# facebookresearch/vggsfm

Measured on NVIDIA H100. Metric: BA iterations/sec, higher is better.
Workload: dtype f64

## Files before the change

include/vggsfm_b200.h:

```cpp
#ifndef VGGSFM_B200_H
#define VGGSFM_B200_H

#include <stddef.h>
#include <stdint.h>

#ifdef __cplusplus
extern "C" {
#endif

#define VGG_OK 0
#define VGG_EINVAL (-1)
#define VGG_ECUDA (-2)
#define VGG_EWORKSPACE (-3)
#define VGG_ESOLVER (-4)

#define VGG_SIMPLE_PINHOLE 0
#define VGG_SIMPLE_RADIAL 1

#define VGG_INTR_CONST 0
#define VGG_INTR_PER_FRAME 1
#define VGG_INTR_SHARED 2

const char* vgg_last_error(void);
int vgg_version(void);


typedef struct vgg_ba_problem {
  int32_t S, N;
  int32_t camera_model;
  int32_t intr_mode;
  const float* uv;
  const uint8_t* mask;
  const uint8_t* param_const;
  const uint8_t* point_const;
  double* poses;
  double* intr;
  double* points;
} vgg_ba_problem;

typedef struct vgg_ba_options {
  int32_t max_num_iterations;
  int32_t max_num_consecutive_invalid_steps;
  int32_t jacobi_scaling;
  int32_t reserved;
  double function_tolerance, gradient_tolerance, parameter_tolerance;
  double initial_trust_region_radius, max_trust_region_radius, min_trust_region_radius;
  double min_relative_decrease, min_lm_diagonal, max_lm_diagonal;
} vgg_ba_options;

typedef struct vgg_ba_summary {
  int32_t iterations, successful, termination, reserved;
  double initial_cost, final_cost, final_radius;
  double device_ms;
  int64_t kernel_launches;
} vgg_ba_summary;

#define VGG_BA_NO_CONVERGENCE 0
#define VGG_BA_CONVERGENCE_GRADIENT 1
#define VGG_BA_CONVERGENCE_FUNCTION 2
#define VGG_BA_CONVERGENCE_PARAMETER 3
#define VGG_BA_MIN_TRUST_REGION 4
#define VGG_BA_FAILURE 5

typedef int (*vgg_allreduce_fn)(void* user, double* buf, size_t count, int op, void* stream);

typedef struct vgg_ba_fabric {
  double* ar_local;
  double* ar_multicast;
  size_t ar_doubles;
  int32_t world, rank;
  double* peer_base[8];
  size_t total_doubles;
} vgg_ba_fabric;

void vgg_ba_default_options(vgg_ba_options* opt);
int vgg_ba_dims(int camera_model, int intr_mode, int* dc, int* ns);
int vgg_ba_workspace_bytes(int S, int N, int camera_model, int intr_mode, size_t* bytes);

int vgg_ba_camrec_len(int camera_model, int intr_mode);
int vgg_ba_build_blocks(const vgg_ba_problem* prob, double* cost, double* camrec, double* g_p,
                        double* H_pp, double* W, double* shared, int tracks_per_warp, void* stream);

int vgg_ba_schur(const vgg_ba_problem* prob, const double* camrec, const double* g_p,
                 const double* H_pp, const double* W, const double* shared, const double* scale_p,
                 double radius, double min_diag, double max_diag, void* workspace, size_t ws_bytes,
                 double* Sraw, double* rhs, int* Dpad_out, void* stream);

int vgg_cholesky_lower(int n, int lda, double* A, void* workspace, size_t ws_bytes, int* info_host, void* stream);

int vgg_syrk_ozaki_workspace_bytes(int Kpad, int Dpad, int slices, size_t* bytes);
int vgg_syrk_ozaki(int Kpad, int Dpad, const double* Zt, double* Cmat, int slices, void* workspace, size_t ws_bytes,
                   void* stream);
int vgg_ba_solve(const vgg_ba_problem* prob, const vgg_ba_options* opt, void* workspace,
                 size_t ws_bytes, vgg_allreduce_fn allreduce, void* allreduce_user,
                 vgg_ba_summary* summary, double* trace, void* stream);
int vgg_ba_reduced_system_doubles(int S, int camera_model, int intr_mode, size_t* doubles);
int vgg_ba_fabric_doubles(int S, int camera_model, int intr_mode, size_t* doubles);
int vgg_ba_solve_fabric(const vgg_ba_problem* prob, const vgg_ba_options* opt, void* workspace,
                        size_t ws_bytes, vgg_allreduce_fn allreduce, void* allreduce_user,
                        const vgg_ba_fabric* fabric, vgg_ba_summary* summary, double* trace, void* stream);


typedef struct vgg_pose_options {
  int32_t max_num_iterations;
  int32_t max_num_consecutive_invalid_steps;
  int32_t min_inliers;
  int32_t reserved;
  double function_tolerance, gradient_tolerance, parameter_tolerance;
  double initial_trust_region_radius, max_trust_region_radius, min_trust_region_radius;
  double min_relative_decrease, min_lm_diagonal, max_lm_diagonal;
  double loss_function_scale;
  double max_reproj_error;
} vgg_pose_options;

#define VGG_POSE_SKIPPED 6
#define VGG_POSE_FEW_INLIERS 7

void vgg_pose_default_options(vgg_pose_options* opt);

int vgg_pose_refinement(int S, int P, int camera_model, const float* uv, const uint8_t* inlier,
                        const uint8_t* frame_flags, const double* points, double* poses, double* intr,
                        const vgg_pose_options* opt, uint8_t* inlier_used, double* summary_d, int32_t* summary_i,
                        void* stream);


int vgg_tri_workspace_bytes(int S, int N, int H0, int lo_num, size_t* bytes);
int vgg_triangulate_tracks(int S, int N, const double* extrinsics, const double* tracks_normalized,
                           const float* track_vis, const float* track_score, const int32_t* pairs, int H0,
                           int lo_num, double max_angular_error_deg, double min_tri_angle_deg, double* out_points,
                           int64_t* out_inlier_num, uint8_t* out_inlier_mask, void* workspace, size_t ws_bytes,
                           void* stream);

int vgg_triangulate_by_pair(int S, int N, const double* extrinsics, const double* tracks_normalized,
                            double* out_points, uint8_t* out_cheirality, double* out_angle_deg, void* workspace,
                            size_t ws_bytes, void* stream);

int vgg_filter_points3d(int S, int P, const double* points3d, const void* points2d, int points2d_is_f64,
                        const double* extrinsics, const double* intrinsics9, const double* extra_params,
                        double max_reproj_error, double min_tri_angle_deg, int check_triangle, double hard_max,
                        uint8_t* out_valid, uint8_t* out_detail, void* workspace, size_t ws_bytes, void* stream);

int vgg_project_points(int S, int P, const double* points3d, const double* extrinsics, const double* intrinsics9,
                       const double* extra_params, double* out_points2d, double* out_points_cam, void* stream);

int vgg_normalize_tracks(int S, int N, const void* tracks, const void* focal2, const void* pp2, int is_f64, void* out,
                         void* stream);

int vgg_undistort_simple_radial(int S, int N, const double* tracks_normalized, const double* extra_params,
                                int max_iterations, double max_step_norm, double rel_step_size, double* out,
                                int* iterations_run, void* workspace, size_t ws_bytes, void* stream);

int vgg_pnp_workspace_bytes(int S, int estimate_focal_length, size_t* bytes);
int vgg_absolute_pose_estimation(int S, int P, int camera_model, const float* uv, const uint8_t* mask,
                                 const uint8_t* frame_flags, const double* points, const double* intr,
                                 const double* u_samples, int num_trials, int estimate_focal_length, double max_error,
                                 double* pose_out, double* focal_out, int* num_inliers_out, uint8_t* inlier_out,
                                 void* workspace, size_t ws_bytes, void* stream);


int vgg_twoview_workspace_bytes(int B, int N, int T, int lo_num, size_t* bytes);
int vgg_estimate_fundamental(int B, int N, const void* points1, const void* points2, int points_are_f64,
                             const uint8_t* valid_mask, const int32_t* samples, int T, int lo_num, double threshold,
                             int squared, int second_refine, double* fmat_out, int32_t* inlier_num_out,
                             uint8_t* inlier_mask_out, double* residuals_out, void* workspace, size_t ws_bytes,
                             void* stream);

int vgg_fundamental_inliers(int B, int N, const void* points1, const void* points2, int points_are_f64,
                            const double* fmat, double threshold, int squared, uint8_t* inlier_mask_out, void* stream);

int vgg_relative_pose_from_fundamental(int B, int N, const void* points1, const void* points2, int points_are_f64,
                                       const double* fmat, double width, double height, double* R_out, double* t_out,
                                       double* E_out, void* stream);

int vgg_msac_fundamental_workspace_bytes(int B, int N, int max_iterations, int min_iterations, size_t* bytes);
int vgg_estimate_fundamental_msac(int B, int N, const void* points1, const void* points2, int points_are_f64,
                                  const uint8_t* valid_mask, double max_error, int max_iterations, int min_iterations,
                                  unsigned long long seed, double* fmat_out, int32_t* inlier_num_out,
                                  uint8_t* inlier_mask_out, int32_t* iterations_out, void* workspace, size_t ws_bytes,
                                  void* stream);


int vgg_corr_pyramid_bytes(int BS, int C, int H, int W, int num_levels, int elem_size, size_t* pyramid_bytes,
                           size_t* scratch_bytes);
int vgg_corr_build_pyramid(int BS, int C, int H, int W, int num_levels, const float* fmaps_nchw, int elem_size,
                           void* pyramid, void* scratch, void* stream);

int vgg_corr_sample(int BS, int N, int C, int H, int W, int num_levels, int radius, const void* pyramid, int elem_size,
                    const float* targets, const float* coords, int border_padding, float* out, void* stream);

int vgg_corr_tc_supported(int C, int H, int W, int num_levels, int radius);
int vgg_corr_tc_bytes(int BS, int C, int H, int W, int num_levels, int N, size_t* tile_bytes, size_t* target_bytes);
int vgg_corr_tc_build(int BS, int C, int H, int W, int num_levels, const void* pyramid_half, void* tiles, void* stream);
int vgg_corr_tc_sample(int BS, int N, int C, int H, int W, int num_levels, int radius, const void* tiles, const float* targets,
                       const float* coords, void* target_tiles, float* out, void* stream);

int vgg_sample_features4d(int B, int C, int H, int W, int R, const float* input_nchw, const float* coords, float* out,
                          void* stream);



int vgg_depth_sparse_samples(int n_total, const int32_t* uvd_frame, const double* uvd, double depth_min,
                             double depth_max, const int64_t* map_offsets, const int32_t* map_hw, const float* disp,
                             float* x_out, double* y_out, uint8_t* keep_out, void* stream);

int vgg_depth_median(int F, const int32_t* offsets, const double* y, double divisor, double* median_out,
                     void* stream);

int vgg_depth_ransac_workspace_bytes(int F, size_t* bytes);
int vgg_depth_ransac_max_chunk(void);
int vgg_depth_ransac_begin(int F, int max_trials, void* workspace, size_t ws_bytes, void* stream);
int vgg_depth_ransac_chunk(int F, const int32_t* offsets, const float* x, const double* y, const double* threshold,
                           int R, const int32_t* frames, int T, const int32_t* samples, uint8_t* running_out,
                           void* workspace, size_t ws_bytes, void* stream);
int vgg_depth_ransac_finish(int F, const int32_t* offsets, const float* x, const double* y, const double* threshold,
                            float* scale_out, float* shift_out, int32_t* n_trials_out, int32_t* n_inliers_out,
                            uint8_t* inlier_mask_out, void* workspace, size_t ws_bytes, void* stream);

int vgg_depth_tile_pixels(void);
int vgg_depth_apply(int F, int64_t n_tiles, const int64_t* map_offsets, const int64_t* tile_offsets,
                    const float* scale, const float* shift, float* disp, float* depth_out, int32_t* tile_counts,
                    void* stream);

int vgg_depth_unproject(int F, int64_t n_tiles, const int64_t* map_offsets, const int32_t* map_hw,
                        const int64_t* tile_offsets, const int64_t* tile_base, const float* depth, const uint8_t* rgb,
                        const int32_t* cam_model, const double* cam_params, const double* world_from_cam,
                        double* out, void* stream);

#ifdef __cplusplus
}
#endif
#endif
```

vggsfm_b200/_lib.py:

```python
from __future__ import annotations

import ctypes
import os

_HERE = os.path.dirname(os.path.abspath(__file__))
LIB_PATH = os.path.join(_HERE, "libvggsfm_b200.so")

EXPORTS = [
    "vgg_last_error", "vgg_version",
    "vgg_ba_default_options", "vgg_ba_dims", "vgg_ba_workspace_bytes", "vgg_ba_camrec_len",
    "vgg_ba_build_blocks", "vgg_ba_schur", "vgg_cholesky_lower", "vgg_ba_solve",
    "vgg_ba_reduced_system_doubles", "vgg_ba_fabric_doubles", "vgg_ba_solve_fabric",
    "vgg_pose_default_options", "vgg_pose_refinement", "vgg_pnp_workspace_bytes", "vgg_absolute_pose_estimation", "vgg_syrk_ozaki_workspace_bytes", "vgg_syrk_ozaki",
    "vgg_tri_workspace_bytes", "vgg_triangulate_tracks", "vgg_triangulate_by_pair", "vgg_filter_points3d",
    "vgg_project_points", "vgg_normalize_tracks", "vgg_undistort_simple_radial",
    "vgg_corr_pyramid_bytes", "vgg_corr_build_pyramid", "vgg_corr_sample", "vgg_sample_features4d",
    "vgg_corr_tc_supported", "vgg_corr_tc_bytes", "vgg_corr_tc_build", "vgg_corr_tc_sample",
    "vgg_twoview_workspace_bytes", "vgg_estimate_fundamental", "vgg_relative_pose_from_fundamental",
    "vgg_fundamental_inliers", "vgg_msac_fundamental_workspace_bytes", "vgg_estimate_fundamental_msac",
    "vgg_depth_sparse_samples", "vgg_depth_median", "vgg_depth_ransac_workspace_bytes", "vgg_depth_ransac_max_chunk",
    "vgg_depth_ransac_begin", "vgg_depth_ransac_chunk", "vgg_depth_ransac_finish", "vgg_depth_tile_pixels",
    "vgg_depth_apply", "vgg_depth_unproject",
]


DEV_EXPORTS = ["vgg_dev_blocks_timing", "vgg_dev_blocks_last_ms", "vgg_dev_chol128_probe", "vgg_dev_syrk_f64", "vgg_dev_syrk_f64_band", "vgg_dev_syrk_ozaki_band", "vgg_dev_trsv_probe", "vgg_dev_cholesky_band",
               "vgg_dev_last_band_hint", "vgg_dev_msac_trace", "vgg_dev_relative_pose_counts"]


class BAProblem(ctypes.Structure):
    _fields_ = [
        ("S", ctypes.c_int32), ("N", ctypes.c_int32),
        ("camera_model", ctypes.c_int32), ("intr_mode", ctypes.c_int32),
        ("uv", ctypes.c_void_p), ("mask", ctypes.c_void_p),
        ("param_const", ctypes.c_void_p), ("point_const", ctypes.c_void_p),
        ("poses", ctypes.c_void_p), ("intr", ctypes.c_void_p), ("points", ctypes.c_void_p),
    ]


class BAOptions(ctypes.Structure):
    _fields_ = [
        ("max_num_iterations", ctypes.c_int32),
        ("max_num_consecutive_invalid_steps", ctypes.c_int32),
        ("jacobi_scaling", ctypes.c_int32),
        ("reserved", ctypes.c_int32),
        ("function_tolerance", ctypes.c_double),
        ("gradient_tolerance", ctypes.c_double),
        ("parameter_tolerance", ctypes.c_double),
        ("initial_trust_region_radius", ctypes.c_double),
        ("max_trust_region_radius", ctypes.c_double),
        ("min_trust_region_radius", ctypes.c_double),
        ("min_relative_decrease", ctypes.c_double),
        ("min_lm_diagonal", ctypes.c_double),
        ("max_lm_diagonal", ctypes.c_double),
    ]


class BASummary(ctypes.Structure):
    _fields_ = [
        ("iterations", ctypes.c_int32), ("successful", ctypes.c_int32),
        ("termination", ctypes.c_int32), ("reserved", ctypes.c_int32),
        ("initial_cost", ctypes.c_double), ("final_cost", ctypes.c_double),
        ("final_radius", ctypes.c_double), ("device_ms", ctypes.c_double),
        ("kernel_launches", ctypes.c_int64),
    ]


class BAFabric(ctypes.Structure):
    _fields_ = [("ar_local", ctypes.c_void_p), ("ar_multicast", ctypes.c_void_p), ("ar_doubles", ctypes.c_size_t),
                ("world", ctypes.c_int32), ("rank", ctypes.c_int32), ("peer_base", ctypes.c_void_p * 8),
                ("total_doubles", ctypes.c_size_t)]


class PoseOptions(ctypes.Structure):
    _fields_ = [
        ("max_num_iterations", ctypes.c_int32),
        ("max_num_consecutive_invalid_steps", ctypes.c_int32),
        ("min_inliers", ctypes.c_int32),
        ("reserved", ctypes.c_int32),
        ("function_tolerance", ctypes.c_double),
        ("gradient_tolerance", ctypes.c_double),
        ("parameter_tolerance", ctypes.c_double),
        ("initial_trust_region_radius", ctypes.c_double),
        ("max_trust_region_radius", ctypes.c_double),
        ("min_trust_region_radius", ctypes.c_double),
        ("min_relative_decrease", ctypes.c_double),
        ("min_lm_diagonal", ctypes.c_double),
        ("max_lm_diagonal", ctypes.c_double),
        ("loss_function_scale", ctypes.c_double),
        ("max_reproj_error", ctypes.c_double),
    ]


ALLREDUCE_FN = ctypes.CFUNCTYPE(ctypes.c_int, ctypes.c_void_p, ctypes.c_void_p, ctypes.c_size_t,
                                ctypes.c_int, ctypes.c_void_p)

_lib = None


class NativeLibraryMissing(RuntimeError):
    pass


def lib() -> ctypes.CDLL:
    global _lib
    if _lib is not None:
        return _lib
    if not os.path.exists(LIB_PATH):
        raise NativeLibraryMissing(
            f"{LIB_PATH} not found: build it with `python -c 'import __graft_entry__ as g; g.build()'` "
            "or `make`. vggsfm_b200 has no CPU/PyTorch fallback.")
    L = ctypes.CDLL(LIB_PATH, mode=ctypes.RTLD_GLOBAL)
    L.vgg_last_error.restype = ctypes.c_char_p
    L.vgg_version.restype = ctypes.c_int
    L.vgg_ba_default_options.argtypes = [ctypes.POINTER(BAOptions)]
    L.vgg_ba_default_options.restype = None
    L.vgg_ba_dims.argtypes = [ctypes.c_int, ctypes.c_int, ctypes.POINTER(ctypes.c_int), ctypes.POINTER(ctypes.c_int)]
    L.vgg_ba_workspace_bytes.argtypes = [ctypes.c_int, ctypes.c_int, ctypes.c_int, ctypes.c_int,
                                         ctypes.POINTER(ctypes.c_size_t)]
    L.vgg_ba_camrec_len.argtypes = [ctypes.c_int, ctypes.c_int]
    L.vgg_ba_build_blocks.argtypes = [ctypes.POINTER(BAProblem)] + [ctypes.c_void_p] * 6 + [ctypes.c_int, ctypes.c_void_p]
    L.vgg_ba_schur.argtypes = ([ctypes.POINTER(BAProblem)] + [ctypes.c_void_p] * 6 +
                               [ctypes.c_double] * 3 + [ctypes.c_void_p, ctypes.c_size_t, ctypes.c_void_p,
                                                        ctypes.c_void_p, ctypes.POINTER(ctypes.c_int), ctypes.c_void_p])
    L.vgg_ba_solve.argtypes = [ctypes.POINTER(BAProblem), ctypes.POINTER(BAOptions), ctypes.c_void_p, ctypes.c_size_t,
                               ALLREDUCE_FN, ctypes.c_void_p, ctypes.POINTER(BASummary), ctypes.c_void_p,
                               ctypes.c_void_p]
    vp, ci, cd, cs = ctypes.c_void_p, ctypes.c_int, ctypes.c_double, ctypes.c_size_t
    L.vgg_ba_reduced_system_doubles.argtypes = [ci, ci, ci, ctypes.POINTER(cs)]
    L.vgg_ba_fabric_doubles.argtypes = [ci, ci, ci, ctypes.POINTER(cs)]
    L.vgg_ba_solve_fabric.argtypes = [ctypes.POINTER(BAProblem), ctypes.POINTER(BAOptions), vp, cs, ALLREDUCE_FN, vp,
                                      ctypes.POINTER(BAFabric), ctypes.POINTER(BASummary), vp, vp]
    L.vgg_pose_default_options.argtypes = [ctypes.POINTER(PoseOptions)]
    L.vgg_pose_default_options.restype = None
    L.vgg_pose_refinement.argtypes = [ci, ci, ci, vp, vp, vp, vp, vp, vp, ctypes.POINTER(PoseOptions), vp, vp, vp, vp]
    L.vgg_pnp_workspace_bytes.argtypes = [ci, ci, ctypes.POINTER(cs)]
    L.vgg_absolute_pose_estimation.argtypes = [ci, ci, ci, vp, vp, vp, vp, vp, vp, ci, ci, cd, vp, vp, vp, vp, vp, cs, vp]
    L.vgg_syrk_ozaki_workspace_bytes.argtypes = [ci, ci, ci, ctypes.POINTER(cs)]
    L.vgg_dev_blocks_timing.argtypes = [ci]
    L.vgg_dev_blocks_last_ms.argtypes = [ctypes.POINTER(cd)]
    L.vgg_dev_chol128_probe.argtypes = [ci, vp, vp, vp]
    L.vgg_dev_syrk_f64.argtypes = [ci, ci, vp, vp, vp]
    L.vgg_dev_syrk_f64_band.argtypes = L.vgg_dev_syrk_f64.argtypes + [vp, ci]
    L.vgg_dev_trsv_probe.argtypes = [ci, ci, vp, vp, cs, vp, vp]
    L.vgg_dev_last_band_hint.argtypes = [vp, vp, vp, vp, vp]
    L.vgg_syrk_ozaki.argtypes = [ci, ci, vp, vp, ci, vp, cs, vp]
    L.vgg_dev_syrk_ozaki_band.argtypes = L.vgg_syrk_ozaki.argtypes + [vp, ci]
    L.vgg_cholesky_lower.argtypes = [ci, ci, vp, vp, cs, ctypes.POINTER(ci), vp]
    L.vgg_dev_cholesky_band.argtypes = L.vgg_cholesky_lower.argtypes + [vp, ci, ci]
    L.vgg_tri_workspace_bytes.argtypes = [ci, ci, ci, ci, ctypes.POINTER(cs)]
    L.vgg_triangulate_tracks.argtypes = [ci, ci, vp, vp, vp, vp, vp, ci, ci, cd, cd, vp, vp, vp, vp, cs, vp]
    L.vgg_triangulate_by_pair.argtypes = [ci, ci, vp, vp, vp, vp, vp, vp, cs, vp]
    L.vgg_filter_points3d.argtypes = [ci, ci, vp, vp, ci, vp, vp, vp, cd, cd, ci, cd, vp, vp, vp, cs, vp]
    L.vgg_project_points.argtypes = [ci, ci, vp, vp, vp, vp, vp, vp, vp]
    L.vgg_normalize_tracks.argtypes = [ci, ci, vp, vp, vp, ci, vp, vp]
    L.vgg_undistort_simple_radial.argtypes = [ci, ci, vp, vp, ci, cd, cd, vp, ctypes.POINTER(ci), vp, cs, vp]
    L.vgg_corr_pyramid_bytes.argtypes = [ci, ci, ci, ci, ci, ci, ctypes.POINTER(cs), ctypes.POINTER(cs)]
    L.vgg_corr_build_pyramid.argtypes = [ci, ci, ci, ci, ci, vp, ci, vp, vp, vp]
    L.vgg_sample_features4d.argtypes = [ci, ci, ci, ci, ci, vp, vp, vp, vp]
    L.vgg_corr_sample.argtypes = [ci, ci, ci, ci, ci, ci, ci, vp, ci, vp, vp, ci, vp, vp]
    L.vgg_corr_tc_supported.argtypes = [ci, ci, ci, ci, ci]
    L.vgg_corr_tc_bytes.argtypes = [ci, ci, ci, ci, ci, ci, ctypes.POINTER(cs), ctypes.POINTER(cs)]
    L.vgg_corr_tc_build.argtypes = [ci, ci, ci, ci, ci, vp, vp, vp]
    L.vgg_corr_tc_sample.argtypes = [ci, ci, ci, ci, ci, ci, ci, vp, vp, vp, vp, vp, vp]
    L.vgg_twoview_workspace_bytes.argtypes = [ci, ci, ci, ci, ctypes.POINTER(cs)]
    L.vgg_estimate_fundamental.argtypes = [ci, ci, vp, vp, ci, vp, vp, ci, ci, cd, ci, ci, vp, vp, vp, vp, vp, cs, vp]
    L.vgg_fundamental_inliers.argtypes = [ci, ci, vp, vp, ci, vp, cd, ci, vp, vp]
    L.vgg_relative_pose_from_fundamental.argtypes = [ci, ci, vp, vp, ci, vp, cd, cd, vp, vp, vp, vp]
    L.vgg_dev_relative_pose_counts.argtypes = [ci, ci, vp, vp, ci, vp, cd, cd, vp, vp, vp, vp, vp]
    cu64 = ctypes.c_ulonglong
    L.vgg_msac_fundamental_workspace_bytes.argtypes = [ci, ci, ci, ci, ctypes.POINTER(cs)]
    L.vgg_estimate_fundamental_msac.argtypes = [ci, ci, vp, vp, ci, vp, cd, ci, ci, cu64, vp, vp, vp, vp, vp, cs, vp]
    L.vgg_dev_msac_trace.argtypes = [ci, ci, ci, ci, vp, ci, vp, vp, vp]
    i64 = ctypes.c_int64
    L.vgg_depth_sparse_samples.argtypes = [ci, vp, vp, cd, cd, vp, vp, vp, vp, vp, vp, vp]
    L.vgg_depth_median.argtypes = [ci, vp, vp, cd, vp, vp]
    L.vgg_depth_ransac_workspace_bytes.argtypes = [ci, ctypes.POINTER(cs)]
    L.vgg_depth_ransac_max_chunk.argtypes = []
    L.vgg_depth_ransac_begin.argtypes = [ci, ci, vp, cs, vp]
    L.vgg_depth_ransac_chunk.argtypes = [ci, vp, vp, vp, vp, ci, vp, ci, vp, vp, vp, cs, vp]
    L.vgg_depth_ransac_finish.argtypes = [ci, vp, vp, vp, vp, vp, vp, vp, vp, vp, vp, cs, vp]
    L.vgg_depth_tile_pixels.argtypes = []
    L.vgg_depth_apply.argtypes = [ci, i64, vp, vp, vp, vp, vp, vp, vp, vp]
    L.vgg_depth_unproject.argtypes = [ci, i64, vp, vp, vp, vp, vp, vp, vp, vp, vp, vp, vp]
    _lib = L
    return L


def check(rc: int, what: str) -> None:
    if rc != 0:
        raise RuntimeError(f"{what} failed (rc={rc}): {lib().vgg_last_error().decode(errors='replace')}")
```

vggsfm_b200/bundle_adjustment.py:

```python
from __future__ import annotations

import ctypes
import dataclasses
from typing import Optional

import torch

from . import _lib
from ._lib import BAOptions, BAProblem, BASummary

SIMPLE_PINHOLE = 0
SIMPLE_RADIAL = 1
INTR_CONST = 0
INTR_PER_FRAME = 1
INTR_SHARED = 2

TERMINATION = {0: "NO_CONVERGENCE", 1: "CONVERGENCE_GRADIENT", 2: "CONVERGENCE_FUNCTION",
               3: "CONVERGENCE_PARAMETER", 4: "MIN_TRUST_REGION_RADIUS", 5: "FAILURE_INVALID_STEPS"}


def camera_model_id(camera_type: str) -> int:
    if camera_type == "SIMPLE_PINHOLE":
        return SIMPLE_PINHOLE
    if camera_type == "SIMPLE_RADIAL":
        return SIMPLE_RADIAL
    raise ValueError(f"Camera type {camera_type} is not supported yet")


def dims(model: int, mode: int):
    dc, ns = ctypes.c_int(), ctypes.c_int()
    _lib.check(_lib.lib().vgg_ba_dims(model, mode, ctypes.byref(dc), ctypes.byref(ns)), "vgg_ba_dims")
    return dc.value, ns.value


def default_options() -> BAOptions:
    o = BAOptions()
    _lib.lib().vgg_ba_default_options(ctypes.byref(o))
    return o


def prepare_ba_options() -> BAOptions:
    o = default_options()
    o.function_tolerance *= 10
    o.gradient_tolerance *= 10
    o.parameter_tolerance *= 10
    o.max_num_iterations = 50
    return o


def default_param_const(S: int, model: int, mode: int, device, refine_focal_length=True, refine_extra_params=True,
                        gauge=True, const_pose: Optional[torch.Tensor] = None) -> torch.Tensor:
    dc, ns = dims(model, mode)
    c = torch.zeros(S * dc + ns, dtype=torch.uint8)
    if gauge:
        c[0:6] = 1
        if S > 1:
            c[dc + 3] = 1
    if const_pose is not None:
        for s in torch.nonzero(const_pose.cpu()).flatten().tolist():
            c[s * dc:s * dc + 6] = 1
    ni = 1 if model == SIMPLE_PINHOLE else 2
    for j, fl in enumerate([refine_focal_length, refine_extra_params][:ni]):
        if not fl:
            if mode == INTR_PER_FRAME:
                c[torch.arange(S) * dc + 6 + j] = 1
            elif mode == INTR_SHARED:
                c[S * dc + j] = 1
    return c.to(device)


_ws_cache: dict = {}


def workspace(S: int, N: int, model: int, mode: int, device) -> torch.Tensor:
    key = (S, N, model, mode, str(device))
    ws = _ws_cache.get(key)
    if ws is None:
        nbytes = ctypes.c_size_t()
        with torch.cuda.device(device):
            _lib.check(_lib.lib().vgg_ba_workspace_bytes(S, N, model, mode, ctypes.byref(nbytes)),
                       "vgg_ba_workspace_bytes")
        if len(_ws_cache) > 4:
            _ws_cache.clear()
        ws = torch.empty(nbytes.value, dtype=torch.uint8, device=device)
        _ws_cache[key] = ws
    return ws


def _problem(uv, mask, poses, intr, points, model, mode, param_const, point_const):
    S, N = mask.shape
    assert uv.dtype == torch.float32 and uv.is_contiguous() and uv.shape == (S, N, 2)
    assert mask.dtype == torch.uint8 and mask.is_contiguous()
    for t in (poses, intr, points):
        assert t.dtype == torch.float64 and t.is_contiguous() and t.is_cuda
    assert poses.shape == (S, 3, 4) and intr.shape == (S, 4) and points.shape == (N, 3)
    p = BAProblem()
    p.S, p.N, p.camera_model, p.intr_mode = S, N, model, mode
    p.uv, p.mask = uv.data_ptr(), mask.data_ptr()
    p.param_const = param_const.data_ptr() if param_const is not None else None
    p.point_const = point_const.data_ptr() if point_const is not None else None
    p.poses, p.intr, p.points = poses.data_ptr(), intr.data_ptr(), points.data_ptr()
    return p


def build_blocks(uv, mask, poses, intr, points, model, mode, point_const=None, tracks_per_warp=0):
    L = _lib.lib()
    S, N = mask.shape
    dc, ns = dims(model, mode)
    KR = L.vgg_ba_camrec_len(model, mode)
    dev = uv.device
    al = lambda n: (n + 31) // 32 * 32
    offs, tot = {}, 0
    for name, n in (("cost", 8), ("shared", 8), ("camrec", S * KR), ("g_p", N * 3), ("H_pp", N * 6)):
        offs[name] = (tot, n)
        tot += al(n)
    flat = torch.empty(tot, dtype=torch.float64, device=dev)
    view = lambda name, shape: flat[offs[name][0]:offs[name][0] + offs[name][1]].view(*shape)
    out = {
        "cost": view("cost", (8,))[:1],
        "camrec": view("camrec", (S, KR)),
        "g_p": view("g_p", (N, 3)),
        "H_pp": view("H_pp", (N, 6)),
        "W": torch.empty(N, (S * dc + ns + 1) // 2 * 2, 3, dtype=torch.float64, device=dev),
        "shared": view("shared", (8,)),
    }
    p = _problem(uv, mask, poses, intr, points, model, mode, None, point_const)
    with torch.cuda.device(dev):
        st = torch.cuda.current_stream().cuda_stream
        _lib.check(L.vgg_ba_build_blocks(ctypes.byref(p), out["cost"].data_ptr(), out["camrec"].data_ptr(),
                                         out["g_p"].data_ptr(), out["H_pp"].data_ptr(), out["W"].data_ptr(),
                                         out["shared"].data_ptr(), tracks_per_warp, st), "vgg_ba_build_blocks")
    return out


def schur(uv, mask, poses, intr, points, model, mode, blocks, scale_p, radius, min_diag=1e-6, max_diag=1e32,
          point_const=None):
    L = _lib.lib()
    S, N = mask.shape
    dc, ns = dims(model, mode)
    D = S * dc + ns
    Dpad = (D + 2 + 127) // 128 * 128
    dev = uv.device
    ws = workspace(S, N, model, mode, dev)
    Sraw = torch.empty(D, Dpad, dtype=torch.float64, device=dev)
    rhs = torch.empty(Dpad, dtype=torch.float64, device=dev)
    p = _problem(uv, mask, poses, intr, points, model, mode, None, point_const)
    dpad = ctypes.c_int()
    with torch.cuda.device(dev):
        st = torch.cuda.current_stream().cuda_stream
        _lib.check(L.vgg_ba_schur(ctypes.byref(p), blocks["camrec"].data_ptr(), blocks["g_p"].data_ptr(),
                                  blocks["H_pp"].data_ptr(), blocks["W"].data_ptr(), blocks["shared"].data_ptr(),
                                  scale_p.data_ptr(), radius, min_diag, max_diag, ws.data_ptr(), ws.numel(),
                                  Sraw.data_ptr(), rhs.data_ptr(), ctypes.byref(dpad), st), "vgg_ba_schur")
    assert dpad.value == Dpad
    return Sraw, rhs[:D]


@dataclasses.dataclass
class Summary:
    iterations: int
    successful: int
    termination: str
    initial_cost: float
    final_cost: float
    final_radius: float
    device_ms: float
    kernel_launches: int
    trace: Optional[torch.Tensor] = None
    alive: Optional[torch.Tensor] = None
    mask: Optional[torch.Tensor] = None


def lm_solve(uv, mask, poses, intr, points, model, mode, param_const=None, point_const=None,
             options: Optional[BAOptions] = None, allreduce=None, want_trace=False) -> Summary:
    L = _lib.lib()
    S, N = mask.shape
    dev = uv.device
    if param_const is None:
        param_const = default_param_const(S, model, mode, dev)
    opt = options or default_options()
    ws = workspace(S, N, model, mode, dev)
    p = _problem(uv, mask, poses, intr, points, model, mode, param_const, point_const)
    summ = BASummary()
    trace = torch.zeros(max(1, opt.max_num_iterations), 8, dtype=torch.float64) if want_trace else None
    cb = allreduce.bind(ws) if allreduce is not None else _lib.ALLREDUCE_FN()
    fabric = getattr(allreduce, "fabric", None)
    with torch.cuda.device(dev):
        st = torch.cuda.current_stream().cuda_stream
        if fabric is not None:
            fs = fabric.struct()
            rc = L.vgg_ba_solve_fabric(ctypes.byref(p), ctypes.byref(opt), ws.data_ptr(), ws.numel(), cb, None,
                                       ctypes.byref(fs), ctypes.byref(summ),
                                       trace.data_ptr() if trace is not None else None, st)
        else:
            rc = L.vgg_ba_solve(ctypes.byref(p), ctypes.byref(opt), ws.data_ptr(), ws.numel(), cb, None,
                                ctypes.byref(summ), trace.data_ptr() if trace is not None else None, st)
    _lib.check(rc, "vgg_ba_solve")
    return Summary(summ.iterations, summ.successful, TERMINATION.get(summ.termination, "?"), summ.initial_cost,
                   summ.final_cost, summ.final_radius, summ.device_ms, summ.kernel_launches,
                   trace[:summ.iterations] if trace is not None else None)



def filter_negative_depth(poses, points, mask):
    eps = torch.finfo(torch.float64).eps
    depth = torch.einsum("sj,nj->sn", poses[:, 2, :3], points) + poses[:, 2, 3][:, None]
    bad = mask & ~(depth >= eps)
    length = mask.sum(dim=0)
    nbad = bad.sum(dim=0)
    alive = (nbad == 0) | ((length - nbad) >= 2)
    mask = mask & ~bad & alive[None]
    return mask, alive


def normalize(poses, points, extent=10.0, p0=0.1, p1=0.9, alive=None):
    S = poses.shape[0]
    if S < 2:
        return poses, points
    R = poses[:, :, :3]
    t = poses[:, :, 3]
    centers = -torch.einsum("sji,sj->si", R, t)
    c32 = torch.sort(centers.to(torch.float32), dim=0).values
    P0 = int(p0 * (S - 1)) if S > 3 else 0
    P1 = int(p1 * (S - 1)) if S > 3 else S - 1
    bmin = c32[P0].double()
    bmax = c32[P1].double()
    mean = c32[P0:P1 + 1].double().sum(dim=0) / (P1 - P0 + 1)
    old_extent = torch.linalg.norm(bmax - bmin)
    scale = torch.where(old_extent < torch.finfo(torch.float64).eps, torch.ones_like(old_extent), extent / old_extent)
    tr = -scale * mean
    new_points = scale * points + tr
    if alive is not None:
        new_points = torch.where(alive[:, None], new_points, points)
    new_poses = poses.clone()
    new_poses[:, :, 3] = scale * t - torch.einsum("sij,j->si", R, tr)
    return new_poses, new_points


def pad_tracks(n: int, multiple: int = 16) -> int:
    return (n + multiple - 1) // multiple * multiple


def bundle_adjustment(points3d, extrinsics, intrinsics, extra_params, tracks, masks, shared_camera=False,
                      camera_type="SIMPLE_PINHOLE", options: Optional[BAOptions] = None, max_points3D_val=3000.0,
                      allreduce=None, want_trace=False, refine_focal_length=True, refine_extra_params=True,
                      const_pose=None, const_points=None, gauge=True, do_normalize=True, filter_reconstruction=True,
                      drop_negative_depth=True):
    model = camera_model_id(camera_type)
    dev = tracks.device
    if not tracks.is_cuda:
        raise RuntimeError("vggsfm_b200.bundle_adjustment needs CUDA tensors (no CPU fallback)")
    masks = masks.bool()
    valid_idx = torch.nonzero(masks.sum(dim=0) >= 2).flatten()
    pts = points3d.double()[valid_idx].contiguous()
    P = pts.shape[0]
    m = masks[:, valid_idx]
    m = m & (pts < max_points3D_val).all(dim=1)[None]
    poses = extrinsics.double().contiguous().clone()
    S = poses.shape[0]
    intr = torch.zeros(S, 4, dtype=torch.float64, device=dev)
    intr[:, 0] = intrinsics[:, 0, 0]
    intr[:, 1] = intrinsics[:, 0, 2]
    intr[:, 2] = intrinsics[:, 1, 2]
    if model == SIMPLE_RADIAL:
        intr[:, 3] = extra_params[:, 0]
    if shared_camera:
        mode = INTR_SHARED
        intr[:] = intr[0].clone()
    else:
        mode = INTR_PER_FRAME
    if not (refine_focal_length or refine_extra_params):
        mode = INTR_CONST
    if drop_negative_depth:
        m, alive = filter_negative_depth(poses, pts, m)
    else:
        alive = torch.ones(P, dtype=torch.bool, device=dev)
    point_const = ~m.any(dim=0)
    if const_points is not None:
        point_const = point_const | const_points[valid_idx]
    Pp = pad_tracks(max(P, 1))
    uv = torch.zeros(S, Pp, 2, dtype=torch.float32, device=dev)
    uv[:, :P] = tracks[:, valid_idx].float()
    mk = torch.zeros(S, Pp, dtype=torch.uint8, device=dev)
    mk[:, :P] = m.to(torch.uint8)
    X = torch.zeros(Pp, 3, dtype=torch.float64, device=dev)
    X[:P] = pts
    X[P:, 2] = 1.0
    pc = torch.ones(Pp, dtype=torch.uint8, device=dev)
    pc[:P] = point_const.to(torch.uint8)
    param_const = default_param_const(S, model, mode, dev, refine_focal_length, refine_extra_params, gauge, const_pose)
    summary = lm_solve(uv, mk, poses, intr, X, model, mode, param_const, pc, options, allreduce, want_trace)
    pts = X[:P]
    if do_normalize:
        poses, pts = normalize(poses, pts, 10.0, 0.1, 0.9, alive)
        if filter_reconstruction:
            poses, pts = normalize(poses, pts, 5.0, 0.1, 0.9, alive)
    pts = torch.where(alive[:, None], pts, torch.zeros_like(pts))
    summary.alive, summary.mask = alive, m
    K = torch.zeros(S, 3, 3, dtype=torch.float64, device=dev)
    K[:, 0, 0] = intr[:, 0]
    K[:, 1, 1] = intr[:, 0]
    K[:, 0, 2] = intr[:, 1]
    K[:, 1, 2] = intr[:, 2]
    K[:, 2, 2] = 1.0
    extra_out = intr[:, 3:4].clone() if model == SIMPLE_RADIAL else None
    return pts, poses, K, extra_out, valid_idx, summary


run_ba = bundle_adjustment



from .reconstruction import Reconstruction


def _reconstruction(pts, extr, K, extra, tracks, masks, image_size, camera_type, shared_camera, summary, alive=None):
    return Reconstruction.from_batch_matrix(pts, extr, K, tracks, masks, image_size, shared_camera=shared_camera,
                                            camera_type=camera_type, extra_params=extra, summary=summary, alive=alive)


def _revert_negative_focal(extr_new, K_new, extra_new, extr_old, K_old, extra_old):
    bad = K_new[:, 0, 0] < 0
    if bad.any():
        extr_new[bad] = extr_old[bad].to(extr_new.dtype)
        K_new[bad] = K_old[bad].to(K_new.dtype)
        if extra_new is not None:
            extra_new[bad] = extra_old[bad].to(extra_new.dtype)
    return extr_new, K_new, extra_new


def global_BA(triangulated_points, valid_tracks, pred_tracks, inlier_mask, extrinsics, intrinsics, extra_params,
              image_size, shared_camera=False, camera_type="SIMPLE_PINHOLE", allreduce=None):
    BA_points = triangulated_points[valid_tracks]
    BA_tracks = pred_tracks[:, valid_tracks]
    BA_inlier_masks = inlier_mask[valid_tracks].transpose(0, 1)
    pts, extr, K, extra, valid_idx, summary = bundle_adjustment(
        BA_points, extrinsics, intrinsics, extra_params, BA_tracks, BA_inlier_masks, shared_camera=shared_camera,
        camera_type=camera_type, options=prepare_ba_options(), allreduce=allreduce)
    extr, K, extra = _revert_negative_focal(extr, K, extra, extrinsics, intrinsics, extra_params)
    rec = _reconstruction(pts, extr, K, extra, BA_tracks[:, valid_idx], summary.mask, image_size, camera_type,
                          shared_camera, summary, summary.alive)
    return pts, extr, K, extra, rec


def init_BA(extrinsics, intrinsics, extra_params, tracks, points_3d_pair, inlier, image_size, shared_camera=False,
            init_max_reproj_error=0.5, camera_type="SIMPLE_PINHOLE"):
    from . import triangulation as tri
    init_idx = int(torch.argmax(inlier.sum(dim=-1)).item())
    init_indices = [0, init_idx + 1]
    toBA_extrinsics = extrinsics[init_indices]
    toBA_intrinsics = intrinsics[init_indices]
    toBA_extra = extra_params[init_indices] if extra_params is not None else None
    toBA_masks = inlier[init_idx].unsqueeze(0)
    toBA_masks = torch.cat([torch.ones_like(toBA_masks), toBA_masks], dim=0)
    valid_track = toBA_masks.sum(dim=0) >= 2
    toBA_masks = toBA_masks[:, valid_track]
    toBA_points = points_3d_pair[init_idx][valid_track]
    toBA_tracks = tracks[init_indices][:, valid_track]
    pts, extr, K, extra, valid_idx, summary = bundle_adjustment(
        toBA_points, toBA_extrinsics, toBA_intrinsics, toBA_extra, toBA_tracks, toBA_masks, shared_camera=shared_camera,
        camera_type=camera_type, options=prepare_ba_options(), filter_reconstruction=False)
    rec = _reconstruction(pts, extr, K, extra, toBA_tracks[:, valid_idx], summary.mask, image_size, camera_type,
                          shared_camera, summary, summary.alive)
    ok, _ = tri.filter_all_points3D(pts, toBA_tracks, extr, K, extra, check_triangle=False,
                                    max_reproj_error=init_max_reproj_error)
    points3D_opt = pts[ok]
    filtered = valid_track.clone()
    filtered[valid_track] = ok
    extrinsics[init_indices] = extr.to(extrinsics.dtype)
    intrinsics[init_indices] = K.to(intrinsics.dtype)
    if extra_params is not None:
        extra_params[init_indices] = extra.to(extra_params.dtype)
    return points3D_opt, extrinsics, intrinsics, extra_params, filtered, rec, init_idx


def get_valid_frame_mask(intrinsics, extrinsics, extra_params, scale):
    valid = (intrinsics[:, 0, 0] >= 0.1 * scale) & (intrinsics[:, 0, 0] <= 30 * scale)
    if extra_params is not None:
        if extra_params.dim() == 1:
            extra_params = extra_params[:, None]
        valid = valid & (extra_params.abs() <= 1.0).all(dim=-1)
    return valid & (extrinsics[:, :, 3].abs() <= 30).all(-1)


def iterative_global_BA(pred_tracks, intrinsics, extrinsics, pred_vis, pred_score, valid_tracks, points3D_opt,
                        image_size, shared_camera=False, min_valid_track_length=2, max_reproj_error=1,
                        ba_options=None, lastBA=False, camera_type="SIMPLE_PINHOLE", extra_params=None,
                        allreduce=None):
    from . import triangulation as tri
    tn = tri.cam_from_img(pred_tracks, intrinsics, extra_params)
    best_points, best_num, best_mask = tri.triangulate_tracks(extrinsics, tn, track_vis=pred_vis, track_score=pred_score,
                                                             max_ransac_iters=128)
    best_points[valid_tracks] = points3D_opt.to(best_points.dtype)
    _, filtered = tri.filter_all_points3D(best_points, pred_tracks, extrinsics, intrinsics, extra_params=extra_params,
                                          max_reproj_error=max_reproj_error, return_detail=True)
    valid_tracks = filtered.sum(dim=0) >= min_valid_track_length
    BA_points = best_points[valid_tracks]
    BA_tracks = pred_tracks[:, valid_tracks]
    BA_inlier_masks = filtered[:, valid_tracks]
    pts, extr, K, extra, valid_idx, summary = bundle_adjustment(
        BA_points, extrinsics, intrinsics, extra_params, BA_tracks, BA_inlier_masks, shared_camera=shared_camera,
        camera_type=camera_type, options=ba_options or default_options(), allreduce=allreduce)
    rec = _reconstruction(pts, extr, K, extra, BA_tracks[:, valid_idx], summary.mask, image_size, camera_type,
                          shared_camera, summary, summary.alive)
    if valid_idx.numel() != BA_points.shape[0]:
        full = torch.zeros(BA_points.shape[0], 3, dtype=pts.dtype, device=pts.device)
        full[valid_idx] = pts
        pts = full
    extr, K, extra = _revert_negative_focal(extr, K, extra, extrinsics, intrinsics, extra_params)
    _, filtered = tri.filter_all_points3D(pts, pred_tracks[:, valid_tracks], extr, K, extra_params=extra,
                                          max_reproj_error=max_reproj_error, return_detail=True)
    valid_after = filtered.sum(dim=0) >= min_valid_track_length
    valid_tmp = valid_tracks.clone()
    valid_tmp[valid_tracks] = valid_after
    valid_tracks = valid_tmp
    pts = pts[valid_after]
    BA_inlier_masks = filtered[:, valid_after]
    if lastBA:
        e2, p2 = normalize(extr, pts, 5.0, 0.1, 0.9)
        rec = _reconstruction(p2, e2, K, extra, pred_tracks[:, valid_tracks], BA_inlier_masks, image_size, camera_type,
                              shared_camera, summary)
    return pts, extr, K, extra, valid_tracks, BA_inlier_masks, rec
```

vggsfm_b200/csrc/ba_blocks.cu:

```cuda
#include <stdlib.h>
#include <utility>
#include "common.cuh"
#include "dev_probes.h"

namespace vgg {

static bool g_blocks_timing = false;
static cudaEvent_t g_blocks_ev[2] = {nullptr, nullptr};

constexpr int BW = 4;
constexpr int BT = BW * 32;
constexpr int TB = 4;
constexpr int XT = 32;
constexpr int PVS = 33;

template <int MODEL, int MODE>
struct BlkCfg {
  static constexpr int NI = (MODEL == VGG_SIMPLE_PINHOLE) ? 1 : 2;
  static constexpr int DC = (MODE == VGG_INTR_PER_FRAME) ? 6 + NI : 6;
  static constexpr int NS = (MODE == VGG_INTR_SHARED) ? NI : 0;
  static constexpr int NPACK = DC * (DC + 1) / 2;
  static constexpr int KR = DC + NPACK + 6 * NS;
  static constexpr int NP = 9 + 3 * NS;
};

__host__ __device__ constexpr int pack_row(int dc, int p) {
  int i = 0;
  while (p >= dc - i) { p -= dc - i; ++i; }
  return i;
}
__host__ __device__ constexpr int pack_col(int dc, int p) {
  int i = 0;
  while (p >= dc - i) { p -= dc - i; ++i; }
  return i + p;
}

template <int DC, int NS, int K, int KR>
__device__ __forceinline__ void cam_accumulate_one(double (&acc)[KR], const double* jc0, const double* jc1, double rx,
                                                   double ry) {
  constexpr int NPACK = DC * (DC + 1) / 2;
  if constexpr (K < DC) {
    acc[K] = fma(jc0[K], rx, fma(jc1[K], ry, acc[K]));
  } else if constexpr (K < DC + NPACK) {
    constexpr int i = pack_row(DC, K - DC), j = pack_col(DC, K - DC);
    acc[K] = fma(jc0[i], jc0[j], fma(jc1[i], jc1[j], acc[K]));
  } else {
    constexpr int q = K - DC - NPACK;
    constexpr int i = q / (NS > 0 ? NS : 1), j = q % (NS > 0 ? NS : 1);
    acc[K] = fma(jc0[i], jc0[6 + j], fma(jc1[i], jc1[6 + j], acc[K]));
  }
}
template <int DC, int NS, int KR, int... K>
__device__ __forceinline__ void cam_accumulate(double (&acc)[KR], const double* jc0, const double* jc1, double rx,
                                               double ry, std::integer_sequence<int, K...>) {
  (cam_accumulate_one<DC, NS, K, KR>(acc, jc0, jc1, rx, ry), ...);
}

template <int MODEL>
__device__ __forceinline__ void obs_math(const double* pw, int lane, const double* xt, float ox, float oy, bool valid,
                                         double* jc0, double* jc1, double* jx0, double* jx1, double& rx, double& ry) {
  const double2 xa = *reinterpret_cast<const double2*>(xt);
  const double2 xb = *reinterpret_cast<const double2*>(xt + 2);
  const double X0 = xa.x, X1 = xa.y, X2 = xb.x;
  const double m = valid ? 1.0 : 0.0;
  const double mp = (xb.y != 0.0) ? 0.0 : m;
  const double R00 = pw[0 * 32 + lane], R01 = pw[1 * 32 + lane], R02 = pw[2 * 32 + lane], t0_ = pw[3 * 32 + lane];
  const double R10 = pw[4 * 32 + lane], R11 = pw[5 * 32 + lane], R12 = pw[6 * 32 + lane], t1_ = pw[7 * 32 + lane];
  const double R20 = pw[8 * 32 + lane], R21 = pw[9 * 32 + lane], R22 = pw[10 * 32 + lane], t2_ = pw[11 * 32 + lane];
  const double fo = pw[12 * 32 + lane], cx = pw[13 * 32 + lane], cy = pw[14 * 32 + lane];
  const double kk = (MODEL == VGG_SIMPLE_RADIAL) ? pw[15 * 32 + lane] : 0.0;
  const double a1 = R00 * X0 + R01 * X1 + R02 * X2;
  const double a2 = R10 * X0 + R11 * X1 + R12 * X2;
  const double a3 = R20 * X0 + R21 * X1 + R22 * X2;
  const double px = a1 + t0_, py = a2 + t1_;
  const double pz = valid ? (a3 + t2_) : 1.0;
  const double iz = 1.0 / pz;
  const double u = px * iz, w_ = py * iz;
  const double r2 = u * u + w_ * w_;
  const double d = 1.0 + kk * r2;
  rx = valid ? (fo * d * u + cx - (double)ox) : 0.0;
  ry = valid ? (fo * d * w_ + cy - (double)oy) : 0.0;
  double a00, a01, a11;
  if (MODEL == VGG_SIMPLE_RADIAL) {
    a00 = fo * (d + 2.0 * kk * u * u);
    a01 = fo * (2.0 * kk * u * w_);
    a11 = fo * (d + 2.0 * kk * w_ * w_);
  } else {
    a00 = fo; a01 = 0.0; a11 = fo;
  }
  const double izm = iz * m;
  const double j00 = a00 * izm, j01 = a01 * izm, j02 = -(a00 * u + a01 * w_) * izm;
  const double j10 = a01 * izm, j11 = a11 * izm, j12 = -(a01 * u + a11 * w_) * izm;
  const double b1 = 2.0 * a1, b2 = 2.0 * a2, b3 = 2.0 * a3;
  jc0[0] = b2 * j02 - b3 * j01;  jc1[0] = b2 * j12 - b3 * j11;
  jc0[1] = b3 * j00 - b1 * j02;  jc1[1] = b3 * j10 - b1 * j12;
  jc0[2] = b1 * j01 - b2 * j00;  jc1[2] = b1 * j11 - b2 * j10;
  jc0[3] = j00; jc0[4] = j01; jc0[5] = j02;
  jc1[3] = j10; jc1[4] = j11; jc1[5] = j12;
  jc0[6] = m * d * u;            jc1[6] = m * d * w_;
  jc0[7] = m * fo * u * r2;      jc1[7] = m * fo * w_ * r2;
  const double mq = (xb.y != 0.0) ? 0.0 : 1.0;
  jx0[0] = mq * (j00 * R00 + j01 * R10 + j02 * R20);
  jx0[1] = mq * (j00 * R01 + j01 * R11 + j02 * R21);
  jx0[2] = mq * (j00 * R02 + j01 * R12 + j02 * R22);
  jx1[0] = mq * (j10 * R00 + j11 * R10 + j12 * R20);
  jx1[1] = mq * (j10 * R01 + j11 * R11 + j12 * R21);
  jx1[2] = mq * (j10 * R02 + j11 * R12 + j12 * R22);
  (void)mp;
}

template <int DC, int NS, int WB>
__device__ __forceinline__ void emit_blocks(double* wt, double* pvw, int lane, const double* jc0, const double* jc1,
                                            const double* jx0, const double* jx1, double rx, double ry) {
  double wb[WB];
#pragma unroll
  for (int i = 0; i < DC; ++i)
#pragma unroll
    for (int c = 0; c < 3; ++c) wb[i * 3 + c] = jc0[i] * jx0[c] + jc1[i] * jx1[c];
  if ((WB & 1) == 0) {
#pragma unroll
    for (int e = 0; e < WB; e += 2) *reinterpret_cast<double2*>(wt + e) = make_double2(wb[e], wb[e + 1]);
  } else {
#pragma unroll
    for (int e = 0; e < WB; ++e) wt[e] = wb[e];
  }
  pvw[0 * PVS + lane] = jx0[0] * rx + jx1[0] * ry;
  pvw[1 * PVS + lane] = jx0[1] * rx + jx1[1] * ry;
  pvw[2 * PVS + lane] = jx0[2] * rx + jx1[2] * ry;
  pvw[3 * PVS + lane] = jx0[0] * jx0[0] + jx1[0] * jx1[0];
  pvw[4 * PVS + lane] = jx0[0] * jx0[1] + jx1[0] * jx1[1];
  pvw[5 * PVS + lane] = jx0[0] * jx0[2] + jx1[0] * jx1[2];
  pvw[6 * PVS + lane] = jx0[1] * jx0[1] + jx1[1] * jx1[1];
  pvw[7 * PVS + lane] = jx0[1] * jx0[2] + jx1[1] * jx1[2];
  pvw[8 * PVS + lane] = jx0[2] * jx0[2] + jx1[2] * jx1[2];
#pragma unroll
  for (int j = 0; j < NS; ++j)
#pragma unroll
    for (int c = 0; c < 3; ++c) pvw[(9 + j * 3 + c) * PVS + lane] = jc0[6 + j] * jx0[c] + jc1[6 + j] * jx1[c];
}

__host__ __device__ inline size_t w_pitch(int D) { return (size_t)(D + (D & 1)); }

template <int MODEL, int MODE, bool USE_TMA>
__global__ void __launch_bounds__(BT, USE_TMA ? 2 : 3) ba_blocks_kernel(
    int S, int N, int tracks_per_warp, const float* __restrict__ uv, const uint8_t* __restrict__ mask,
    const double* __restrict__ poses, const double* __restrict__ intr, const double* __restrict__ points,
    const uint8_t* __restrict__ point_const, double* __restrict__ cost, double* __restrict__ camrec,
    double* __restrict__ g_p, double* __restrict__ H_pp, double* __restrict__ W, double* __restrict__ shared_out,
    const int* __restrict__ fg_tracks) {
  using C = BlkCfg<MODEL, MODE>;
  constexpr int DC = C::DC, NS = C::NS, KR = C::KR, NP = C::NP;
  constexpr int WB = DC * 3;
  extern __shared__ __align__(128) unsigned char smem_raw[];
  double* sm_pose = reinterpret_cast<double*>(smem_raw);
  double* sm_x = sm_pose + BW * 16 * 32;
  double* sm_pv = sm_x + BW * XT * 4;
  double* sm_w = sm_pv + BW * 32 * PVS;
  float* sm_obs = reinterpret_cast<float*>(sm_w + (size_t)BW * 2 * 32 * WB);
  const int tid = threadIdx.x, lane = tid & 31, warp = tid >> 5;
  const int D = S * DC + NS;
  const size_t pitch = w_pitch(D);
  const int ngroups = (S + 31) / 32;
  const int wid = blockIdx.x * BW + warp;
  const int g = wid % ngroups;
  const int chunk = wid / ngroups;
  const int t_begin = (int)min((long long)N, (long long)chunk * tracks_per_warp);
  const int t_end = min(N, t_begin + tracks_per_warp);
  if (fg_tracks && (t_end <= fg_tracks[2 * g] || t_begin >= fg_tracks[2 * g + 1])) return;
  const int s = g * 32 + lane;
  const bool frame_ok = s < S;
  const int nf = min(32, S - g * 32);
  double* pw = sm_pose + warp * 16 * 32;
  double* xw = sm_x + warp * XT * 4;
  double* pvw = sm_pv + warp * 32 * PVS;
  float* ow = sm_obs + (size_t)warp * 2 * 32 * 12 + lane * 12;
  double* wbuf = sm_w + (size_t)warp * 2 * 32 * WB;

#pragma unroll
  for (int i = 0; i < 12; ++i) pw[i * 32 + lane] = frame_ok ? poses[(size_t)s * 12 + i] : 0.0;
#pragma unroll
  for (int i = 0; i < 4; ++i) pw[(12 + i) * 32 + lane] = frame_ok ? intr[(size_t)s * 4 + i] : 0.0;
  __syncwarp();

  double acc[KR];
#pragma unroll
  for (int i = 0; i < KR; ++i) acc[i] = 0.0;
  double cost_acc = 0.0, gs0 = 0.0, gs1 = 0.0, hss0 = 0.0, hss1 = 0.0, hss2 = 0.0;

  const bool vec_ok = (N & 3) == 0;
  auto fetch = [&](int t0, int stage) {
    float* slot = ow + stage * 32 * 12;
    if (frame_ok && t0 < t_end) {
      const size_t o = (size_t)s * N + t0;
      if (vec_ok && t0 + TB <= t_end) {
        cp_async16(slot, uv + o * 2);
        cp_async16(slot + 4, uv + o * 2 + 4);
        cp_async4(slot + 8, mask + o);
      } else {
        uint32_t m = 0;
        for (int k = 0; k < TB; ++k) {
          const bool in = t0 + k < t_end;
          slot[2 * k] = in ? uv[(o + k) * 2] : 0.f;
          slot[2 * k + 1] = in ? uv[(o + k) * 2 + 1] : 0.f;
          if (in) m |= (uint32_t)(mask[o + k] != 0) << (8 * k);
        }
        reinterpret_cast<uint32_t*>(slot)[8] = m;
      }
    } else {
      *reinterpret_cast<float4*>(slot) = make_float4(0.f, 0.f, 0.f, 0.f);
      *reinterpret_cast<float4*>(slot + 4) = make_float4(0.f, 0.f, 0.f, 0.f);
      reinterpret_cast<uint32_t*>(slot)[8] = 0u;
    }
    cp_async_commit();
  };
  fetch(t_begin, 0);
  int batch = 0;
  for (int t0 = t_begin; t0 < t_end; t0 += TB) {
    if (((t0 - t_begin) & (XT - 1)) == 0) {
      __syncwarp();
      const int nn = t0 + lane;
      double x0 = 0.0, x1 = 0.0, x2 = 1.0, cf = 1.0;
      if (nn < t_end) {
        x0 = points[(size_t)nn * 3]; x1 = points[(size_t)nn * 3 + 1]; x2 = points[(size_t)nn * 3 + 2];
        cf = (point_const && point_const[nn] != 0) ? 1.0 : 0.0;
      }
      *reinterpret_cast<double2*>(xw + lane * 4) = make_double2(x0, x1);
      *reinterpret_cast<double2*>(xw + lane * 4 + 2) = make_double2(x2, cf);
      __syncwarp();
    }
    fetch(t0 + TB, (batch + 1) & 1);
    cp_async_wait<1>();
    const float* cur = ow + (batch & 1) * 32 * 12;
    const float4 ca = *reinterpret_cast<const float4*>(cur);
    const float4 cb = *reinterpret_cast<const float4*>(cur + 4);
    const uint32_t cm = reinterpret_cast<const uint32_t*>(cur)[8];
    ++batch;
#pragma unroll 1
    for (int k = 0; k < TB; k += 2) {
      const int nA = t0 + k;
      if (nA >= t_end) break;
      const bool hasB = nA + 1 < t_end;
      double jcA0[8], jcA1[8], jxA0[3], jxA1[3], rxA, ryA;
      double jcB0[8], jcB1[8], jxB0[3], jxB1[3], rxB, ryB;
      {
        const float ox = k == 0 ? ca.x : cb.x, oy = k == 0 ? ca.y : cb.y;
        const bool valid = frame_ok && ((cm >> (8 * k)) & 0xffu) != 0;
        obs_math<MODEL>(pw, lane, xw + ((nA - t_begin) & (XT - 1)) * 4, ox, oy, valid, jcA0, jcA1, jxA0, jxA1, rxA, ryA);
      }
      {
        const float ox = k == 0 ? ca.z : cb.z, oy = k == 0 ? ca.w : cb.w;
        const bool valid = hasB && frame_ok && ((cm >> (8 * (k + 1))) & 0xffu) != 0;
        obs_math<MODEL>(pw, lane, xw + ((nA + 1 - t_begin) & (XT - 1)) * 4, ox, oy, valid, jcB0, jcB1, jxB0, jxB1, rxB, ryB);
      }
      cost_acc += 0.5 * (rxA * rxA + ryA * ryA) + 0.5 * (rxB * rxB + ryB * ryB);
      if (USE_TMA) {
        if (lane == 0) tma_store_wait_read<0>();
        __syncwarp();
      }
      double* wA = wbuf + lane * WB;
      double* wB = wbuf + 32 * WB + lane * WB;
      emit_blocks<DC, NS, WB>(wA, pvw, lane, jcA0, jcA1, jxA0, jxA1, rxA, ryA);
      emit_blocks<DC, NS, WB>(wB, pvw + 16 * PVS, lane, jcB0, jcB1, jxB0, jxB1, rxB, ryB);
      double* dstA = W + ((size_t)nA * pitch + (size_t)g * 32 * DC) * 3;
      double* dstB = dstA + pitch * 3;
      const uint32_t bytes = (uint32_t)nf * WB * 8u;
      if (USE_TMA && (bytes & 15u) == 0) {
        fence_proxy_async();
        __syncwarp();
        if (lane == 0) {
          tma_store_1d(dstA, wbuf, bytes);
          if (hasB) tma_store_1d(dstB, wbuf + 32 * WB, bytes);
          tma_store_commit();
        }
      } else {
        __syncwarp();
        for (int e = lane; e < nf * WB; e += 32) dstA[e] = wbuf[e];
        if (hasB)
          for (int e = lane; e < nf * WB; e += 32) dstB[e] = wbuf[32 * WB + e];
        __syncwarp();
      }
      cam_accumulate<DC, NS, KR>(acc, jcA0, jcA1, rxA, ryA, std::make_integer_sequence<int, KR>{});
      cam_accumulate<DC, NS, KR>(acc, jcB0, jcB1, rxB, ryB, std::make_integer_sequence<int, KR>{});
      if (NS > 0) {
        gs0 += jcA0[6] * rxA + jcA1[6] * ryA + jcB0[6] * rxB + jcB1[6] * ryB;
        hss0 += jcA0[6] * jcA0[6] + jcA1[6] * jcA1[6] + jcB0[6] * jcB0[6] + jcB1[6] * jcB1[6];
        if (NS > 1) {
          gs1 += jcA0[7] * rxA + jcA1[7] * ryA + jcB0[7] * rxB + jcB1[7] * ryB;
          hss1 += jcA0[6] * jcA0[7] + jcA1[6] * jcA1[7] + jcB0[6] * jcB0[7] + jcB1[6] * jcB1[7];
          hss2 += jcA0[7] * jcA0[7] + jcA1[7] * jcA1[7] + jcB0[7] * jcB0[7] + jcB1[7] * jcB1[7];
        }
      }
      {
        const int v = lane & 15;
        const int nT = nA + (lane >> 4);
        double r = 0.0;
        if (v < NP) {
          const double* row = pvw + ((lane >> 4) * 16 + v) * PVS;
          double r0 = 0.0, r1 = 0.0, r2s = 0.0, r3 = 0.0;
#pragma unroll
          for (int j = 0; j < 32; j += 4) { r0 += row[j]; r1 += row[j + 1]; r2s += row[j + 2]; r3 += row[j + 3]; }
          r = (r0 + r1) + (r2s + r3);
        }
        if (r != 0.0 && nT < t_end) {
          if (v < 3) atomicAdd(&g_p[(size_t)nT * 3 + v], r);
          else if (v < 9) atomicAdd(&H_pp[(size_t)nT * 6 + (v - 3)], r);
          else if (v < NP) atomicAdd(&W[((size_t)nT * pitch + (size_t)S * DC + (v - 9) / 3) * 3 + (v - 9) % 3], r);
        }
      }
      __syncwarp();
    }
  }
  if (USE_TMA && lane == 0) tma_store_wait_all<0>();

  if (frame_ok && t_begin < t_end) {
#pragma unroll
    for (int i = 0; i < KR; ++i)
      if (acc[i] != 0.0) atomicAdd(&camrec[(size_t)s * KR + i], acc[i]);
  }
  {
    double a[8] = {cost_acc, gs0, gs1, hss0, hss1, hss2, 0.0, 0.0};
    const double r = warp_reduce_scatter<8>(a, lane);
    if (lane == 0 && r != 0.0) atomicAdd(cost, r);
    else if (NS > 0 && lane >= 1 && lane < 6 && r != 0.0) atomicAdd(&shared_out[lane - 1], r);
  }
}

template <int MODEL, int MODE>
static int launch_blocks(const vgg_ba_problem* p, double* cost, double* camrec, double* g_p, double* H_pp,
                         double* W, double* shared_out, int tracks_per_warp, const int* fg_tracks, cudaStream_t stream,
                         bool outputs_zeroed) {
  using C = BlkCfg<MODEL, MODE>;
  const int S = p->S, N = p->N;
  const int D = S * C::DC + C::NS;
  const size_t pitch = w_pitch(D);
  const size_t smem = sizeof(double) * (BW * 16 * 32 + BW * XT * 4 + BW * 32 * PVS + (size_t)BW * 2 * 32 * C::DC * 3) +
                      sizeof(float) * BW * 2 * 32 * 12;
  const bool tma_ok = ((reinterpret_cast<uintptr_t>(W) & 15) == 0);
  const int ngroups = (S + 31) / 32;
  const auto kern = tma_ok ? ba_blocks_kernel<MODEL, MODE, true> : ba_blocks_kernel<MODEL, MODE, false>;
  if (tracks_per_warp <= 0 && fg_tracks) {
    tracks_per_warp = 64;
  }
  if (tracks_per_warp <= 0) {
    static int slots = 0;
    if (slots == 0) {
      int dev = 0, sms = 132, per_sm = 2;
      cudaGetDevice(&dev);
      cudaDeviceGetAttribute(&sms, cudaDevAttrMultiProcessorCount, dev);
      cudaFuncSetAttribute(ba_blocks_kernel<MODEL, MODE, true>, cudaFuncAttributeMaxDynamicSharedMemorySize, (int)smem);
      cudaOccupancyMaxActiveBlocksPerMultiprocessor(&per_sm, ba_blocks_kernel<MODEL, MODE, true>, BT, smem);
      if (per_sm < 1) per_sm = 1;
      slots = sms * per_sm;
    }
    const long wave_warps = (long)slots * BW;
    long best_tpw = N;
    for (int waves = 1; waves <= 4; ++waves) {
      long chunks = waves * wave_warps / ngroups;
      if (chunks < 1) chunks = 1;
      long tpw = (N + chunks - 1) / chunks;
      tpw = (tpw + TB - 1) / TB * TB;
      if (tpw < 32 && waves > 1) break;
      best_tpw = tpw;
      if (tpw <= 512) break;
    }
    tracks_per_warp = (int)best_tpw;
  }
  const int chunks = (N + tracks_per_warp - 1) / tracks_per_warp;
  const long nwarps = (long)chunks * ngroups;
  const unsigned grid = (unsigned)((nwarps + BW - 1) / BW);
  if (!outputs_zeroed) {
    const char* lo = reinterpret_cast<const char*>(cost);
    const char* hi = reinterpret_cast<const char*>(H_pp + (size_t)N * 6);
    const size_t payload = sizeof(double) * (1 + 8 + (size_t)S * C::KR + (size_t)N * 9);
    const bool packed = lo < reinterpret_cast<const char*>(shared_out) && shared_out < camrec && camrec < g_p && g_p < H_pp &&
                        hi > lo && (size_t)(hi - lo) <= payload + 5 * 256;
    if (packed) {
      VGG_CUDA_CHECK(cudaMemsetAsync(cost, 0, (size_t)(hi - lo), stream));
    } else {
      VGG_CUDA_CHECK(cudaMemsetAsync(cost, 0, sizeof(double), stream));
      VGG_CUDA_CHECK(cudaMemsetAsync(camrec, 0, sizeof(double) * (size_t)S * C::KR, stream));
      VGG_CUDA_CHECK(cudaMemsetAsync(g_p, 0, sizeof(double) * (size_t)N * 3, stream));
      VGG_CUDA_CHECK(cudaMemsetAsync(H_pp, 0, sizeof(double) * (size_t)N * 6, stream));
      VGG_CUDA_CHECK(cudaMemsetAsync(shared_out, 0, sizeof(double) * 8, stream));
    }
  }
  if (pitch > (size_t)S * C::DC) {
    const size_t tail = pitch - (size_t)S * C::DC;
    VGG_CUDA_CHECK(cudaMemset2DAsync(W + (size_t)S * C::DC * 3, pitch * 24, 0, tail * 24, (size_t)N, stream));
  }
  if (g_blocks_timing) VGG_CUDA_CHECK(cudaEventRecord(g_blocks_ev[0], stream));
  VGG_CUDA_CHECK(cudaFuncSetAttribute(kern, cudaFuncAttributeMaxDynamicSharedMemorySize, (int)smem));
  kern<<<grid, BT, smem, stream>>>(S, N, tracks_per_warp, p->uv, p->mask, p->poses, p->intr, p->points, p->point_const,
                                   cost, camrec, g_p, H_pp, W, shared_out, fg_tracks);
  VGG_LAUNCH_CHECK();
  if (g_blocks_timing) VGG_CUDA_CHECK(cudaEventRecord(g_blocks_ev[1], stream));
  return VGG_OK;
}

int ba_build_blocks(const vgg_ba_problem* p, double* cost, double* camrec, double* g_p, double* H_pp, double* W,
                    double* shared_out, int tracks_per_warp, const int* fg_tracks, cudaStream_t stream,
                    bool outputs_zeroed) {
  const int key = p->camera_model * 3 + p->intr_mode;
  switch (key) {
    case 0: return launch_blocks<0, 0>(p, cost, camrec, g_p, H_pp, W, shared_out, tracks_per_warp, fg_tracks, stream, outputs_zeroed);
    case 1: return launch_blocks<0, 1>(p, cost, camrec, g_p, H_pp, W, shared_out, tracks_per_warp, fg_tracks, stream, outputs_zeroed);
    case 2: return launch_blocks<0, 2>(p, cost, camrec, g_p, H_pp, W, shared_out, tracks_per_warp, fg_tracks, stream, outputs_zeroed);
    case 3: return launch_blocks<1, 0>(p, cost, camrec, g_p, H_pp, W, shared_out, tracks_per_warp, fg_tracks, stream, outputs_zeroed);
    case 4: return launch_blocks<1, 1>(p, cost, camrec, g_p, H_pp, W, shared_out, tracks_per_warp, fg_tracks, stream, outputs_zeroed);
    case 5: return launch_blocks<1, 2>(p, cost, camrec, g_p, H_pp, W, shared_out, tracks_per_warp, fg_tracks, stream, outputs_zeroed);
  }
  set_error("bad camera_model/intr_mode %d/%d", p->camera_model, p->intr_mode);
  return VGG_EINVAL;
}

}

extern "C" int vgg_dev_blocks_timing(int enable) {
  using namespace vgg;
  if (enable && !g_blocks_ev[0]) {
    VGG_CUDA_CHECK(cudaEventCreate(&g_blocks_ev[0]));
    VGG_CUDA_CHECK(cudaEventCreate(&g_blocks_ev[1]));
  }
  g_blocks_timing = enable != 0;
  return VGG_OK;
}

extern "C" int vgg_dev_blocks_last_ms(double* ms) {
  using namespace vgg;
  VGG_REQUIRE(g_blocks_ev[0] && ms, "blocks timing was never enabled");
  VGG_CUDA_CHECK(cudaEventSynchronize(g_blocks_ev[1]));
  float f = 0.f;
  VGG_CUDA_CHECK(cudaEventElapsedTime(&f, g_blocks_ev[0], g_blocks_ev[1]));
  *ms = (double)f;
  return VGG_OK;
}
```

vggsfm_b200/csrc/ba_schur.cu:

```cuda
#include <stddef.h>
#include <algorithm>
#include <vector>
#include "common.cuh"
#include "dev_probes.h"
#include "syrk_work.h"

namespace vgg {

__device__ __forceinline__ void ar_add(double* local, double* mc, double v) {
  if (mc) asm volatile("multimem.red.relaxed.sys.global.add.f64 [%0], %1;" ::"l"(mc), "d"(v) : "memory");
  else atomicAdd(local, v);
}
__device__ __forceinline__ void ar_put(double* local, double* mc, double v) {
  if (mc) asm volatile("multimem.red.relaxed.sys.global.add.f64 [%0], %1;" ::"l"(mc), "d"(v) : "memory");
  else *local = v;
}

__global__ void jacobi_scale_points_kernel(int N, const double* __restrict__ H_pp, double* __restrict__ sc_p, int enable) {
  const int n = blockIdx.x * blockDim.x + threadIdx.x;
  if (n >= N) return;
  const double* h = H_pp + (size_t)n * 6;
  sc_p[n * 3 + 0] = enable ? 1.0 / (1.0 + sqrt(h[0])) : 1.0;
  sc_p[n * 3 + 1] = enable ? 1.0 / (1.0 + sqrt(h[3])) : 1.0;
  sc_p[n * 3 + 2] = enable ? 1.0 / (1.0 + sqrt(h[5])) : 1.0;
}

__global__ void jacobi_scale_cams_kernel(int D, const double* __restrict__ hdiag, double* __restrict__ sc_c, int enable) {
  const int i = blockIdx.x * blockDim.x + threadIdx.x;
  if (i >= D) return;
  sc_c[i] = enable ? 1.0 / (1.0 + sqrt(hdiag[i])) : 1.0;
}

__global__ void point_prep_kernel(int N, const double* __restrict__ H_pp, const double* __restrict__ g_p,
                                  const double* __restrict__ sc_p, const uint8_t* __restrict__ point_const,
                                  double radius, double min_diag, double max_diag, double* __restrict__ M,
                                  double* __restrict__ q, double* __restrict__ dpp, double* __restrict__ scal) {
  const int n = blockIdx.x * blockDim.x + threadIdx.x;
  if (n >= N) return;
  double* Mo = M + (size_t)n * 9;
  if (point_const && point_const[n]) {
#pragma unroll
    for (int i = 0; i < 9; ++i) Mo[i] = 0.0;
    q[n * 3] = q[n * 3 + 1] = q[n * 3 + 2] = 0.0;
    dpp[n * 3] = dpp[n * 3 + 1] = dpp[n * 3 + 2] = 0.0;
    return;
  }
  const double* h = H_pp + (size_t)n * 6;
  const double s0 = sc_p[n * 3], s1 = sc_p[n * 3 + 1], s2 = sc_p[n * 3 + 2];
  double v00 = h[0] * s0 * s0, v01 = h[1] * s0 * s1, v02 = h[2] * s0 * s2;
  double v11 = h[3] * s1 * s1, v12 = h[4] * s1 * s2, v22 = h[5] * s2 * s2;
  const double d0 = fmin(fmax(v00, min_diag), max_diag);
  const double d1 = fmin(fmax(v11, min_diag), max_diag);
  const double d2 = fmin(fmax(v22, min_diag), max_diag);
  dpp[n * 3] = d0; dpp[n * 3 + 1] = d1; dpp[n * 3 + 2] = d2;
  v00 += d0 / radius; v11 += d1 / radius; v22 += d2 / radius;
  bool bad = !(v00 > 0.0);
  const double l00 = sqrt(v00);
  const double l10 = v01 / l00, l20 = v02 / l00;
  const double t11 = v11 - l10 * l10;
  bad = bad || !(t11 > 0.0);
  const double l11 = sqrt(t11);
  const double l21 = (v12 - l20 * l10) / l11;
  const double t22 = v22 - l20 * l20 - l21 * l21;
  bad = bad || !(t22 > 0.0);
  const double l22 = sqrt(t22);
  if (bad) {
    atomicAdd(&scal[6], 1.0);
#pragma unroll
    for (int i = 0; i < 9; ++i) Mo[i] = 0.0;
    q[n * 3] = q[n * 3 + 1] = q[n * 3 + 2] = 0.0;
    return;
  }
  const double i00 = 1.0 / l00, i11 = 1.0 / l11, i22 = 1.0 / l22;
  const double i10 = -l10 * i00 * i11;
  const double i21 = -l21 * i11 * i22;
  const double i20 = -(l20 * i00 + l21 * i10) * i22;
  const double m00 = s0 * i00, m01 = s0 * i10, m02 = s0 * i20;
  const double m11 = s1 * i11, m12 = s1 * i21;
  const double m22 = s2 * i22;
  Mo[0] = m00; Mo[1] = m01; Mo[2] = m02;
  Mo[3] = 0.0; Mo[4] = m11; Mo[5] = m12;
  Mo[6] = 0.0; Mo[7] = 0.0; Mo[8] = m22;
  const double g0 = g_p[n * 3], g1 = g_p[n * 3 + 1], g2 = g_p[n * 3 + 2];
  q[n * 3 + 0] = m00 * g0;
  q[n * 3 + 1] = m01 * g0 + m11 * g1;
  q[n * 3 + 2] = m02 * g0 + m12 * g1 + m22 * g2;
}

__global__ void assemble_hc_kernel(int S, int dc, int ns, int KR, int Dpad, const double* __restrict__ camrec,
                                   const double* __restrict__ shared_in, double* __restrict__ Sraw,
                                   double* __restrict__ rhs, double* __restrict__ hdiag, double* __restrict__ gvec,
                                   ptrdiff_t mc_off) {
  const int s = blockIdx.x;
  const int tid = threadIdx.x;
#define VGG_PUT(ptr, val) ar_put((ptr), mc_off ? (ptr) + mc_off : nullptr, (val))
  if (s < S) {
    const double* rec = camrec + (size_t)s * KR;
    const int base = s * dc;
    if (tid < dc) {
      VGG_PUT(&gvec[base + tid], rec[tid]);
      VGG_PUT(&rhs[base + tid], -rec[tid]);
    }
    if (tid < dc * dc) {
      const int i = tid / dc, j = tid % dc;
      const int a = i < j ? i : j, b = i < j ? j : i;
      const int idx = dc + a * dc - a * (a - 1) / 2 + (b - a);
      const double val = rec[idx];
      VGG_PUT(&Sraw[(size_t)(base + i) * Dpad + base + j], val);
      if (i == j) VGG_PUT(&hdiag[base + i], val);
    }
    if (tid < 6 * ns) {
      const int i = tid / ns, j = tid % ns;
      const double val = rec[dc + dc * (dc + 1) / 2 + tid];
      VGG_PUT(&Sraw[(size_t)(S * dc + j) * Dpad + base + i], val);
      VGG_PUT(&Sraw[(size_t)(base + i) * Dpad + S * dc + j], val);
    }
  } else if (ns > 0) {
    const int base = S * dc;
    if (tid < ns) {
      VGG_PUT(&gvec[base + tid], shared_in[tid]);
      VGG_PUT(&rhs[base + tid], -shared_in[tid]);
    }
    if (tid < ns * ns) {
      const int i = tid / ns, j = tid % ns;
      const int a = i < j ? i : j, b = i < j ? j : i;
      const double val = shared_in[2 + (a == 0 ? b : 2)];
      VGG_PUT(&Sraw[(size_t)(base + i) * Dpad + base + j], val);
      if (i == j) VGG_PUT(&hdiag[base + i], val);
    }
  }
#undef VGG_PUT
}

constexpr int ZB_NT = 32;
__global__ void __launch_bounds__(128) z_build_kernel(int D, int N, int Dpad, size_t pitch, const double* __restrict__ W,
                                                      const double* __restrict__ M, const double* __restrict__ q,
                                                      double* __restrict__ Zt, double* __restrict__ rhs,
                                                      ptrdiff_t mc_off, const int* __restrict__ rb_range) {
  __shared__ double sm[ZB_NT][12];
  const int row = blockIdx.x * 128 + threadIdx.x;
  const int n0 = blockIdx.y * ZB_NT;
  const int nt = min(ZB_NT, N - n0);
  if (rb_range) {
    const int kb_first = (3 * n0) >> 6, kb_last = (3 * (n0 + nt - 1) + 2) >> 6;
    if (kb_last < rb_range[2 * blockIdx.x] || kb_first >= rb_range[2 * blockIdx.x + 1]) return;
  }
  for (int e = threadIdx.x; e < nt * 12; e += 128) {
    const int t = e / 12, k = e % 12;
    sm[t][k] = k < 9 ? M[(size_t)(n0 + t) * 9 + k] : q[(size_t)(n0 + t) * 3 + (k - 9)];
  }
  __syncthreads();
  if (row >= D) return;
  double zq = 0.0;
  const double* wp = W + ((size_t)n0 * pitch + row) * 3;
#pragma unroll 4
  for (int t = 0; t < nt; ++t, wp += pitch * 3) {
    const double w0 = wp[0], w1 = wp[1], w2 = wp[2];
    const double* m = sm[t];
    const double z0 = w0 * m[0];
    const double z1 = w0 * m[1] + w1 * m[4];
    const double z2 = w0 * m[2] + w1 * m[5] + w2 * m[8];
    double* zo = Zt + (size_t)(3 * (n0 + t)) * Dpad + row;
    zo[0] = z0;
    zo[Dpad] = z1;
    zo[2 * (size_t)Dpad] = z2;
    zq += z0 * m[9] + z1 * m[10] + z2 * m[11];
  }
  if (zq != 0.0) ar_add(&rhs[row], mc_off ? &rhs[row] + mc_off : nullptr, zq);
}

constexpr int SF_BM = 128, SF_BK = 16, SF_LDS = 132, SF_STAGES = 4, SF_MMA_WARPS = 8;
constexpr int SF_THREADS = 128 + SF_MMA_WARPS * 32;
constexpr int SF_STAGE_DOUBLES = 2 * SF_BK * SF_LDS;
constexpr size_t SF_SMEM_BYTES = sizeof(double) * SF_STAGES * SF_STAGE_DOUBLES + sizeof(uint64_t) * 2 * SF_STAGES;

struct SyrkWork {
  int bi, bj, kb0, kb1;
};

__global__ void __launch_bounds__(SF_THREADS, 1)
    syrk_f64_kernel(const SyrkWork* __restrict__ work, int nwork, int Kpad, int Dpad, const double* __restrict__ Zt,
                    double* __restrict__ Cmat, ptrdiff_t mc_off, const __grid_constant__ FabricDev fd) {
  extern __shared__ __align__(16) double sf_smem[];
  uint64_t* full = reinterpret_cast<uint64_t*>(sf_smem + SF_STAGES * SF_STAGE_DOUBLES);
  uint64_t* empty = full + SF_STAGES;
  const int warp = threadIdx.x >> 5, lane = threadIdx.x & 31;
  if (threadIdx.x == 0) {
    for (int s = 0; s < SF_STAGES; ++s) {
      mbar_init(&full[s], 1);
      mbar_init(&empty[s], SF_MMA_WARPS);
    }
    mbar_fence_init();
  }
  __syncthreads();

  int stage = 0, phase = 0;
  if (warp < 4) {
    asm volatile("setmaxnreg.dec.sync.aligned.u32 40;");
    if (warp > 0) return;
    const int row = lane & (SF_BK - 1), opnd = lane / SF_BK;
    for (int w = blockIdx.x; w < nwork; w += gridDim.x) {
      const SyrkWork wk = work[w];
      const bool diag = wk.bi == wk.bj;
      const int k1 = min(Kpad, wk.kb1 * 64);
      for (int k = wk.kb0 * 64; k < k1; k += SF_BK) {
        mbar_wait(&empty[stage], phase ^ 1);
        if (lane == 0) mbar_expect_tx(&full[stage], (diag ? 1u : 2u) * SF_BK * SF_BM * (uint32_t)sizeof(double));
        __syncwarp();
        if (opnd == 0 || !diag)
          tma_load_1d(sf_smem + stage * SF_STAGE_DOUBLES + (opnd * SF_BK + row) * SF_LDS,
                      Zt + (size_t)(k + row) * Dpad + (opnd ? wk.bj : wk.bi) * SF_BM, SF_BM * sizeof(double), &full[stage]);
        if (++stage == SF_STAGES) {
          stage = 0;
          phase ^= 1;
        }
      }
    }
    return;
  }

  asm volatile("setmaxnreg.inc.sync.aligned.u32 232;");
  const int wm = (warp - 4) >> 2, wn = warp & 3;
  const int g = lane >> 2, t = lane & 3;
  for (int w = blockIdx.x; w < nwork; w += gridDim.x) {
    const SyrkWork wk = work[w];
    const bool diag = wk.bi == wk.bj;
    const int k1 = min(Kpad, wk.kb1 * 64);
    double acc[4][4][4];
#pragma unroll
    for (int mt = 0; mt < 4; ++mt)
#pragma unroll
      for (int nt = 0; nt < 4; ++nt)
#pragma unroll
        for (int h = 0; h < 4; ++h) acc[mt][nt][h] = 0.0;
    for (int k = wk.kb0 * 64; k < k1; k += SF_BK) {
      mbar_wait(&full[stage], phase);
      const double* as = sf_smem + stage * SF_STAGE_DOUBLES + t * SF_LDS + wm * 64 + g;
      const double* bs = sf_smem + stage * SF_STAGE_DOUBLES + (diag ? 0 : SF_BK * SF_LDS) + t * SF_LDS + wn * 32 + g;
      double b[4][4];
#pragma unroll
      for (int nt = 0; nt < 4; ++nt)
#pragma unroll
        for (int j = 0; j < 4; ++j) b[nt][j] = bs[4 * j * SF_LDS + nt * 8];
#pragma unroll
      for (int mt = 0; mt < 4; ++mt) {
        double a[8];
#pragma unroll
        for (int i = 0; i < 8; ++i) a[i] = as[4 * (i >> 1) * SF_LDS + mt * 16 + 8 * (i & 1)];
#pragma unroll
        for (int nt = 0; nt < 4; ++nt) dmma_m16n8k16(acc[mt][nt], a, b[nt]);
      }
      __syncwarp();
      if (lane == 0) mbar_arrive(&empty[stage]);
      if (++stage == SF_STAGES) {
        stage = 0;
        phase ^= 1;
      }
    }
#pragma unroll
    for (int mt = 0; mt < 4; ++mt)
#pragma unroll
      for (int nt = 0; nt < 4; ++nt)
#pragma unroll
        for (int h = 0; h < 4; ++h) {
          const int r = wk.bi * SF_BM + wm * 64 + mt * 16 + g + 8 * (h >> 1);
          const int col = wk.bj * SF_BM + wn * 32 + nt * 8 + 2 * t + (h & 1);
          syrk_red_upper(Cmat, Dpad, r, col, wk.bj, diag, acc[mt][nt][h], mc_off, fd);
        }
  }
}

__global__ void scale_damp_kernel(int D, int Dpad, double* __restrict__ A, const double* __restrict__ rhs,
                                  const double* __restrict__ hdiag, const double* __restrict__ sc,
                                  const uint8_t* __restrict__ pconst, double radius, double min_diag, double max_diag,
                                  double* __restrict__ bvec) {
  const int j = blockIdx.x * blockDim.x + threadIdx.x;
  const int i = blockIdx.y;
  if (j >= D || j > i) return;
  const bool ci = pconst[i] != 0, cj = pconst[j] != 0;
  double v;
  if (ci || cj) {
    v = (i == j) ? 1.0 : 0.0;
  } else {
    v = A[(size_t)i * Dpad + j] * sc[i] * sc[j];
    if (i == j) v += fmin(fmax(hdiag[i] * sc[i] * sc[i], min_diag), max_diag) / radius;
  }
  A[(size_t)i * Dpad + j] = v;
  if (i == j) {
    const double b = ci ? 0.0 : rhs[i] * sc[i];
    bvec[i] = b;
    A[(size_t)D * Dpad + i] = b;
    if (i == 0) A[(size_t)D * Dpad + D] = 1e300;
  }
}

__global__ void cam_step_kernel(int D, const double* __restrict__ dcs, size_t dcs_stride, const double* __restrict__ sc,
                                const double* __restrict__ hdiag, const double* __restrict__ gvec,
                                const uint8_t* __restrict__ pconst, double radius, double min_diag, double max_diag,
                                double* __restrict__ d_c, double* __restrict__ scal) {
  const int i = blockIdx.x * blockDim.x + threadIdx.x;
  double a = 0, b = 0, bad = 0;
  if (i < D) {
    const double x = pconst[i] ? 0.0 : dcs[(size_t)i * dcs_stride];
    const double dc = x * sc[i];
    d_c[i] = dc;
    if (!isfinite(x)) bad = 1.0;
    const double dcc = fmin(fmax(hdiag[i] * sc[i] * sc[i], min_diag), max_diag);
    a = pconst[i] ? 0.0 : (x * x * dcc / radius - dc * gvec[i]);
    b = dc * dc;
  }
  a = warp_sum(a); b = warp_sum(b); bad = warp_sum(bad);
  if ((threadIdx.x & 31) == 0) {
    atomicAdd(&scal[0], a);
    atomicAdd(&scal[1], b);
    if (bad > 0) atomicAdd(&scal[7], bad);
  }
}

__global__ void __launch_bounds__(256) backsub_kernel(int D, int N, size_t pitch, const double* __restrict__ W,
                                                      const double* __restrict__ d_c, double* __restrict__ wacc,
                                                      const int* __restrict__ kb_rows, int arrow_row) {
  const int lane = threadIdx.x & 31;
  const int n = blockIdx.x * 8 + (threadIdx.x >> 5);
  if (n >= N) return;
  const double* wp = W + (size_t)n * pitch * 3;
  double w0 = 0, w1 = 0, w2 = 0;
  auto span = [&](int r0, int r1) {
#pragma unroll 4
    for (int r = r0 + lane; r < r1; r += 32) {
      const double d = __ldg(d_c + r);
      w0 = fma(wp[(size_t)r * 3], d, w0);
      w1 = fma(wp[(size_t)r * 3 + 1], d, w1);
      w2 = fma(wp[(size_t)r * 3 + 2], d, w2);
    }
  };
  if (kb_rows) {
    const int ka = (3 * n) >> 6, kb = (3 * n + 2) >> 6;
    const int lo = min(kb_rows[2 * ka], kb_rows[2 * kb]), hi = min(max(kb_rows[2 * ka + 1], kb_rows[2 * kb + 1]), arrow_row);
    if (lo < hi) span(lo, hi);
    span(min(arrow_row, D), D);
  } else {
    span(0, D);
  }
  w0 = warp_sum(w0); w1 = warp_sum(w1); w2 = warp_sum(w2);
  if (lane == 0) {
    wacc[(size_t)n * 3] = w0;
    wacc[(size_t)n * 3 + 1] = w1;
    wacc[(size_t)n * 3 + 2] = w2;
  }
}

__global__ void point_step_kernel(int N, const double* __restrict__ M, const double* __restrict__ g_p,
                                  const double* __restrict__ wacc, const double* __restrict__ sc_p,
                                  const double* __restrict__ dpp, const double* __restrict__ X, double radius,
                                  double* __restrict__ Xc, double* __restrict__ scal) {
  const int n = blockIdx.x * blockDim.x + threadIdx.x;
  double a = 0, b = 0;
  if (n < N) {
    const double* m = M + (size_t)n * 9;
    const double g0 = g_p[n * 3], g1 = g_p[n * 3 + 1], g2 = g_p[n * 3 + 2];
    const double y0 = -(g0 + wacc[n * 3]), y1 = -(g1 + wacc[n * 3 + 1]), y2 = -(g2 + wacc[n * 3 + 2]);
    const double t0 = m[0] * y0;
    const double t1 = m[1] * y0 + m[4] * y1;
    const double t2 = m[2] * y0 + m[5] * y1 + m[8] * y2;
    const double d0 = m[0] * t0 + m[1] * t1 + m[2] * t2;
    const double d1 = m[4] * t1 + m[5] * t2;
    const double d2 = m[8] * t2;
    Xc[n * 3] = X[n * 3] + d0;
    Xc[n * 3 + 1] = X[n * 3 + 1] + d1;
    Xc[n * 3 + 2] = X[n * 3 + 2] + d2;
    const double s0 = sc_p[n * 3], s1 = sc_p[n * 3 + 1], s2 = sc_p[n * 3 + 2];
    const double e0 = d0 / s0, e1 = d1 / s1, e2 = d2 / s2;
    a = (e0 * e0 * dpp[n * 3] + e1 * e1 * dpp[n * 3 + 1] + e2 * e2 * dpp[n * 3 + 2]) / radius -
        (d0 * g0 + d1 * g1 + d2 * g2);
    b = d0 * d0 + d1 * d1 + d2 * d2;
  }
  a = warp_sum(a); b = warp_sum(b);
  if ((threadIdx.x & 31) == 0) {
    atomicAdd(&scal[2], a);
    atomicAdd(&scal[3], b);
  }
}

__global__ void cam_update_kernel(int S, int dc, int ns, int model, const double* __restrict__ d_c,
                                  const double* __restrict__ poses, const double* __restrict__ intr,
                                  double* __restrict__ poses_c, double* __restrict__ intr_c) {
  const int s = blockIdx.x * blockDim.x + threadIdx.x;
  if (s >= S) return;
  const double* d = d_c + (size_t)s * dc;
  const double p0 = 2.0 * d[0], p1 = 2.0 * d[1], p2 = 2.0 * d[2];
  const double th2 = p0 * p0 + p1 * p1 + p2 * p2;
  const double th = sqrt(th2);
  double a, b;
  if (th < 1e-12) {
    a = 1.0 - th2 / 6.0;
    b = 0.5 - th2 / 24.0;
  } else {
    a = sin(th) / th;
    b = (1.0 - cos(th)) / th2;
  }
  double E[9];
  E[0] = 1.0 + b * (-(p1 * p1 + p2 * p2)); E[1] = -a * p2 + b * p0 * p1;           E[2] = a * p1 + b * p0 * p2;
  E[3] = a * p2 + b * p0 * p1;             E[4] = 1.0 + b * (-(p0 * p0 + p2 * p2)); E[5] = -a * p0 + b * p1 * p2;
  E[6] = -a * p1 + b * p0 * p2;            E[7] = a * p0 + b * p1 * p2;            E[8] = 1.0 + b * (-(p0 * p0 + p1 * p1));
  const double* P = poses + (size_t)s * 12;
  double* Q = poses_c + (size_t)s * 12;
#pragma unroll
  for (int i = 0; i < 3; ++i)
#pragma unroll
    for (int j = 0; j < 3; ++j) Q[i * 4 + j] = E[i * 3] * P[j] + E[i * 3 + 1] * P[4 + j] + E[i * 3 + 2] * P[8 + j];
  Q[3] = P[3] + d[3];
  Q[7] = P[7] + d[4];
  Q[11] = P[11] + d[5];
  const int ni = (model == VGG_SIMPLE_PINHOLE) ? 1 : 2;
  double f = intr[s * 4], k = intr[s * 4 + 3];
  if (dc > 6) {
    f += d[6];
    if (ni > 1) k += d[7];
  } else if (ns > 0) {
    const double* dsh = d_c + (size_t)S * dc;
    f += dsh[0];
    if (ni > 1) k += dsh[1];
  }
  intr_c[s * 4] = f;
  intr_c[s * 4 + 1] = intr[s * 4 + 1];
  intr_c[s * 4 + 2] = intr[s * 4 + 2];
  intr_c[s * 4 + 3] = k;
}

__global__ void extract_gvec_kernel(int S, int dc, int ns, int KR, const double* __restrict__ camrec,
                                    const double* __restrict__ shared_in, double* __restrict__ gvec) {
  const int i = blockIdx.x * blockDim.x + threadIdx.x;
  const int D = S * dc + ns;
  if (i >= D) return;
  gvec[i] = (i < S * dc) ? camrec[(size_t)(i / dc) * KR + (i % dc)] : shared_in[i - S * dc];
}

__global__ void gradmax_kernel(int D, int N, const double* __restrict__ gvec, const uint8_t* __restrict__ pconst,
                               const double* __restrict__ g_p, const uint8_t* __restrict__ point_const,
                               double* __restrict__ scal) {
  const int i = blockIdx.x * blockDim.x + threadIdx.x;
  unsigned long long mc = 0, mp = 0;
  if (i < D && !pconst[i]) mc = (unsigned long long)__double_as_longlong(fabs(gvec[i]));
  if (i < N * 3 && !(point_const && point_const[i / 3])) mp = (unsigned long long)__double_as_longlong(fabs(g_p[i]));
#pragma unroll
  for (int off = 16; off >= 1; off >>= 1) {
    mc = max(mc, __shfl_xor_sync(0xffffffffu, mc, off));
    mp = max(mp, __shfl_xor_sync(0xffffffffu, mp, off));
  }
  if ((threadIdx.x & 31) == 0) {
    atomicMax(reinterpret_cast<unsigned long long*>(&scal[4]), mc);
    atomicMax(reinterpret_cast<unsigned long long*>(&scal[5]), mp);
  }
}

int launch_jacobi_scale_points(int N, const double* H_pp, double* sc_p, int enable, cudaStream_t st) {
  jacobi_scale_points_kernel<<<(N + 255) / 256, 256, 0, st>>>(N, H_pp, sc_p, enable);
  VGG_LAUNCH_CHECK();
  return VGG_OK;
}
int launch_jacobi_scale_cams(int D, const double* hdiag, double* sc_c, int enable, cudaStream_t st) {
  jacobi_scale_cams_kernel<<<(D + 255) / 256, 256, 0, st>>>(D, hdiag, sc_c, enable);
  VGG_LAUNCH_CHECK();
  return VGG_OK;
}
int launch_point_prep(int N, const double* H_pp, const double* g_p, const double* sc_p, const uint8_t* point_const,
                      double radius, double min_diag, double max_diag, double* M, double* q, double* dpp,
                      double* scal, cudaStream_t st) {
  point_prep_kernel<<<(N + 127) / 128, 128, 0, st>>>(N, H_pp, g_p, sc_p, point_const, radius, min_diag, max_diag, M, q,
                                                     dpp, scal);
  VGG_LAUNCH_CHECK();
  return VGG_OK;
}
int launch_assemble_hc(int S, int dc, int ns, int KR, int Dpad, const double* camrec, const double* shared_in,
                       double* Sraw, double* rhs, double* hdiag, double* gvec, ptrdiff_t mc_off, cudaStream_t st) {
  assemble_hc_kernel<<<S + (ns > 0 ? 1 : 0), 64, 0, st>>>(S, dc, ns, KR, Dpad, camrec, shared_in, Sraw, rhs, hdiag, gvec,
                                                          mc_off);
  VGG_LAUNCH_CHECK();
  return VGG_OK;
}
int launch_z_transpose(int D, int N, int Dpad, const double* W, const double* M, const double* q, double* Zt,
                       double* rhs, ptrdiff_t mc_off, const int* rb_range, cudaStream_t st) {
  const size_t pitch = (size_t)(D + (D & 1));
  dim3 grid((D + 127) / 128, (N + ZB_NT - 1) / ZB_NT);
  z_build_kernel<<<grid, 128, 0, st>>>(D, N, Dpad, pitch, W, M, q, Zt, rhs, mc_off, rb_range);
  VGG_LAUNCH_CHECK();
  return VGG_OK;
}

struct SyrkF64State {
  int dev = -1, Kpad = -1, Dpad = -1, sms = 0, nwork = 0;
  std::vector<int> ranges;
  SyrkWork* work_dev = nullptr;
  size_t work_cap = 0;
};
thread_local SyrkF64State g_sf;

int launch_syrk(int Kpad, int Dpad, const double* Zt, double* Cmat, ptrdiff_t mc_off, const std::vector<int>& kb_ranges,
                const FabricDev& fd, cudaStream_t st) {
  VGG_REQUIRE(Dpad % SF_BM == 0 && Kpad % SF_BK == 0, "syrk: Dpad must be a multiple of 128 and Kpad of 16");
  const int nb = Dpad / SF_BM, KB = (Kpad + 63) / 64;
  SyrkF64State& hs = g_sf;
  const std::vector<int> ranges = (int)kb_ranges.size() == 2 * nb ? kb_ranges : std::vector<int>();
  int dev = 0;
  VGG_CUDA_CHECK(cudaGetDevice(&dev));
  if (hs.dev != dev || hs.Kpad != Kpad || hs.Dpad != Dpad || hs.ranges != ranges) {
    VGG_CUDA_CHECK(cudaDeviceGetAttribute(&hs.sms, cudaDevAttrMultiProcessorCount, dev));
    VGG_CUDA_CHECK(cudaFuncSetAttribute(syrk_f64_kernel, cudaFuncAttributeMaxDynamicSharedMemorySize, (int)SF_SMEM_BYTES));
    std::vector<SyrkWork> work;
    build_work_list<SyrkWork>({1}, syrk_tile_jobs(nb, ranges), KB, hs.sms, KB, 1,
                              [](const SyrkTileJob& j, int, int k0, int k1) { return SyrkWork{j.bi, j.bj, k0, k1}; }, &work);
    VGG_CUDA_CHECK(cudaDeviceSynchronize());
    if (hs.dev != dev || work.size() > hs.work_cap) {
      if (hs.work_dev) cudaFree(hs.work_dev);
      hs.work_dev = nullptr;
      hs.work_cap = std::max<size_t>(work.size(), 1);
      VGG_CUDA_CHECK(cudaMalloc(reinterpret_cast<void**>(&hs.work_dev), sizeof(SyrkWork) * hs.work_cap));
    }
    if (!work.empty())
      VGG_CUDA_CHECK(cudaMemcpy(hs.work_dev, work.data(), sizeof(SyrkWork) * work.size(), cudaMemcpyHostToDevice));
    hs.nwork = (int)work.size();
    hs.dev = dev;
    hs.Kpad = Kpad;
    hs.Dpad = Dpad;
    hs.ranges = ranges;
  }
  if (hs.nwork == 0) return VGG_OK;
  syrk_f64_kernel<<<std::min(hs.sms, hs.nwork), SF_THREADS, SF_SMEM_BYTES, st>>>(hs.work_dev, hs.nwork, Kpad, Dpad, Zt, Cmat,
                                                                               mc_off, fd);
  VGG_LAUNCH_CHECK();
  return VGG_OK;
}
int launch_scale_damp(int D, int Dpad, double* A, const double* rhs, const double* hdiag, const double* sc,
                      const uint8_t* pconst, double radius, double min_diag, double max_diag, double* bvec,
                      cudaStream_t st) {
  dim3 grid((D + 255) / 256, D);
  scale_damp_kernel<<<grid, 256, 0, st>>>(D, Dpad, A, rhs, hdiag, sc, pconst, radius, min_diag, max_diag, bvec);
  VGG_LAUNCH_CHECK();
  return VGG_OK;
}
int launch_cam_step(int D, const double* dcs, size_t dcs_stride, const double* sc, const double* hdiag, const double* gvec,
                    const uint8_t* pconst, double radius, double min_diag, double max_diag, double* d_c, double* scal,
                    cudaStream_t st) {
  cam_step_kernel<<<(D + 255) / 256, 256, 0, st>>>(D, dcs, dcs_stride, sc, hdiag, gvec, pconst, radius, min_diag, max_diag, d_c, scal);
  VGG_LAUNCH_CHECK();
  return VGG_OK;
}
int launch_backsub(int D, int N, const double* W, const double* d_c, double* wacc, const int* kb_rows, int arrow_row,
                   cudaStream_t st) {
  const size_t pitch = (size_t)(D + (D & 1));
  backsub_kernel<<<(N + 7) / 8, 256, 0, st>>>(D, N, pitch, W, d_c, wacc, kb_rows, arrow_row);
  VGG_LAUNCH_CHECK();
  return VGG_OK;
}
int launch_point_step(int N, const double* M, const double* g_p, const double* wacc, const double* sc_p,
                      const double* dpp, const double* X, double radius, double* Xc, double* scal, cudaStream_t st) {
  point_step_kernel<<<(N + 127) / 128, 128, 0, st>>>(N, M, g_p, wacc, sc_p, dpp, X, radius, Xc, scal);
  VGG_LAUNCH_CHECK();
  return VGG_OK;
}
int launch_cam_update(int S, int dc, int ns, int model, const double* d_c, const double* poses, const double* intr,
                      double* poses_c, double* intr_c, cudaStream_t st) {
  cam_update_kernel<<<(S + 127) / 128, 128, 0, st>>>(S, dc, ns, model, d_c, poses, intr, poses_c, intr_c);
  VGG_LAUNCH_CHECK();
  return VGG_OK;
}
int launch_extract_gvec(int S, int dc, int ns, int KR, const double* camrec, const double* shared_in, double* gvec,
                        cudaStream_t st) {
  const int D = S * dc + ns;
  extract_gvec_kernel<<<(D + 255) / 256, 256, 0, st>>>(S, dc, ns, KR, camrec, shared_in, gvec);
  VGG_LAUNCH_CHECK();
  return VGG_OK;
}
int launch_gradmax(int D, int N, const double* gvec, const uint8_t* pconst, const double* g_p,
                   const uint8_t* point_const, double* scal, cudaStream_t st) {
  const int n = D > N * 3 ? D : N * 3;
  gradmax_kernel<<<(n + 255) / 256, 256, 0, st>>>(D, N, gvec, pconst, g_p, point_const, scal);
  VGG_LAUNCH_CHECK();
  return VGG_OK;
}

}

extern "C" {

int vgg_dev_syrk_f64(int Kpad, int Dpad, const double* Zt, double* Cmat, void* stream) {
  return vgg_dev_syrk_f64_band(Kpad, Dpad, Zt, Cmat, stream, nullptr, 0);
}

int vgg_dev_syrk_f64_band(int Kpad, int Dpad, const double* Zt, double* Cmat, void* stream, const int* ranges, int count) {
  using namespace vgg;
  g_launch_count = 0;
  VGG_REQUIRE(Zt && Cmat && Kpad > 0 && Dpad > 0 && (ranges || count <= 0), "bad argument");
  return launch_syrk(Kpad, Dpad, Zt, Cmat, 0, std::vector<int>(ranges, ranges + std::max(count, 0)), FabricDev{},
                     static_cast<cudaStream_t>(stream));
}

}
```

vggsfm_b200/csrc/ba_solve.cu:

```cuda
#include <cublas_v2.h>
#include <math.h>
#include <stdlib.h>
#include <string.h>
#include <map>
#include <vector>
#include "common.cuh"
#include "dev_probes.h"

namespace vgg {

static thread_local char g_err[512] = "";
thread_local long long g_launch_count = 0;
void set_error(const char* fmt, ...) {
  va_list ap;
  va_start(ap, fmt);
  vsnprintf(g_err, sizeof(g_err), fmt, ap);
  va_end(ap);
}

int ba_build_blocks(const vgg_ba_problem* p, double* cost, double* camrec, double* g_p, double* H_pp, double* W,
                    double* shared_out, int tracks_per_warp, const int* fg_tracks, cudaStream_t stream,
                    bool outputs_zeroed = false);
int launch_jacobi_scale_points(int N, const double* H_pp, double* sc_p, int enable, cudaStream_t st);
int launch_jacobi_scale_cams(int D, const double* hdiag, double* sc_c, int enable, cudaStream_t st);
int launch_point_prep(int N, const double* H_pp, const double* g_p, const double* sc_p, const uint8_t* point_const,
                      double radius, double min_diag, double max_diag, double* M, double* q, double* dpp,
                      double* scal, cudaStream_t st);
int launch_assemble_hc(int S, int dc, int ns, int KR, int Dpad, const double* camrec, const double* shared_in,
                       double* Sraw, double* rhs, double* hdiag, double* gvec, ptrdiff_t mc_off, cudaStream_t st);
int launch_z_transpose(int D, int N, int Dpad, const double* W, const double* M, const double* q, double* Zt,
                       double* rhs, ptrdiff_t mc_off, const int* rb_range, cudaStream_t st);
int launch_syrk(int Kpad, int Dpad, const double* Zt, double* Cmat, ptrdiff_t mc_off, const std::vector<int>& kb_ranges,
                const FabricDev& fd, cudaStream_t st);
int launch_scale_damp(int D, int Dpad, double* A, const double* rhs, const double* hdiag, const double* sc,
                      const uint8_t* pconst, double radius, double min_diag, double max_diag, double* bvec,
                      cudaStream_t st);
int launch_cam_step(int D, const double* dcs, size_t dcs_stride, const double* sc, const double* hdiag, const double* gvec,
                    const uint8_t* pconst, double radius, double min_diag, double max_diag, double* d_c, double* scal,
                    cudaStream_t st);
int launch_backsub(int D, int N, const double* W, const double* d_c, double* wacc, const int* kb_rows, int arrow_row,
                   cudaStream_t st);
int launch_point_step(int N, const double* M, const double* g_p, const double* wacc, const double* sc_p,
                      const double* dpp, const double* X, double radius, double* Xc, double* scal, cudaStream_t st);
int launch_cam_update(int S, int dc, int ns, int model, const double* d_c, const double* poses, const double* intr,
                      double* poses_c, double* intr_c, cudaStream_t st);
int launch_extract_gvec(int S, int dc, int ns, int KR, const double* camrec, const double* shared_in, double* gvec,
                        cudaStream_t st);
int launch_gradmax(int D, int N, const double* gvec, const uint8_t* pconst, const double* g_p,
                   const uint8_t* point_const, double* scal, cudaStream_t st);

int launch_trsv_upper(int n, int lda, const double* A, const double* y, size_t y_stride, double* x, long long* stamps,
                      cudaStream_t st);
size_t chol_workspace_doubles(int n);
int chol_lower_inplace(int n, int lda, double* A, double* Ldiag, int* info, const std::vector<int>& end_blk,
                       int arrow_blk, cudaStream_t st);
int launch_fabric_barrier(const FabricDev& fd, size_t flags_off, unsigned long long epoch, int* err, cudaStream_t st);
int launch_fabric_gather(const FabricDev& fd, int nrows, int nmat, int ncols_vec, int lda, cudaStream_t st);
int launch_fabric_allreduce(const FabricDev& fd, size_t flags_off, size_t mail_off, int mail_len, int parity,
                            unsigned long long epoch, double* vec, int count, int max_slot, int* err, cudaStream_t st);

__global__ void pack_scalars_kernel(const double* __restrict__ scal, const double* __restrict__ small,
                                    const int* __restrict__ info, double* __restrict__ out) {
  const int i = threadIdx.x;
  if (i < 8) out[i] = scal[i];
  else if (i < 16) out[i] = small[i - 8];
  else if (i < 18) out[i] = (double)info[i - 16];
  else if (i == 18) out[i] = scal[8];
  else if (i == 19) out[i] = (double)info[2];
}

__global__ void xnorm_kernel(int S, int N, int dc, int ns, int model, const uint8_t* __restrict__ pconst,
                             const uint8_t* __restrict__ point_const, const double* __restrict__ poses,
                             const double* __restrict__ intr, const double* __restrict__ pts, double* __restrict__ out) {
  double acc = 0.0;
  const int np = model == VGG_SIMPLE_RADIAL ? 4 : 3;
  for (int s = threadIdx.x; s < S; s += blockDim.x) {
    const uint8_t* c = pconst + (size_t)s * dc;
    if (!(c[0] && c[1] && c[2])) acc += 1.0;
    if (!(c[3] && c[4] && c[5])) {
      const double* P = poses + (size_t)s * 12;
      acc += P[3] * P[3] + P[7] * P[7] + P[11] * P[11];
    }
    if (dc > 6) {
      bool all_const = true;
      for (int i = 6; i < dc; ++i) all_const = all_const && c[i];
      if (!all_const)
        for (int i = 0; i < np; ++i) acc += intr[(size_t)s * 4 + i] * intr[(size_t)s * 4 + i];
    }
  }
  if (threadIdx.x == 0 && ns > 0) {
    bool all_const = true;
    for (int i = 0; i < ns; ++i) all_const = all_const && pconst[(size_t)S * dc + i];
    if (!all_const)
      for (int i = 0; i < np; ++i) acc += intr[i] * intr[i];
  }
  for (int n = threadIdx.x; n < N; n += blockDim.x) {
    if (point_const && point_const[n]) continue;
    acc += pts[3 * (size_t)n] * pts[3 * (size_t)n] + pts[3 * (size_t)n + 1] * pts[3 * (size_t)n + 1] +
           pts[3 * (size_t)n + 2] * pts[3 * (size_t)n + 2];
  }
  __shared__ double red[32];
  acc = warp_sum(acc);
  if ((threadIdx.x & 31) == 0) red[threadIdx.x >> 5] = acc;
  __syncthreads();
  if (threadIdx.x < 32) {
    double v = threadIdx.x < (blockDim.x >> 5) ? red[threadIdx.x] : 0.0;
    v = warp_sum(v);
    if (threadIdx.x == 0) out[0] = v;
  }
}

struct EventPair {
  cudaEvent_t a = nullptr, b = nullptr;
  ~EventPair() {
    if (a) cudaEventDestroy(a);
    if (b) cudaEventDestroy(b);
  }
};

static double grad_max_norm(double gc, double gp) { return isnan(gc) || isnan(gp) ? NAN : fmax(gc, gp); }

static double* pinned_scalars() {
  static thread_local double* h = nullptr;
  if (!h) {
    if (cudaHostAlloc(reinterpret_cast<void**>(&h), sizeof(double) * 32, cudaHostAllocDefault) != cudaSuccess) h = nullptr;
  }
  return h;
}

static int dims_of(int model, int mode, int* dc, int* ns, int* KR) {
  if (model != VGG_SIMPLE_PINHOLE && model != VGG_SIMPLE_RADIAL) return VGG_EINVAL;
  const int ni = model == VGG_SIMPLE_PINHOLE ? 1 : 2;
  int d, n;
  if (mode == VGG_INTR_CONST) { d = 6; n = 0; }
  else if (mode == VGG_INTR_PER_FRAME) { d = 6 + ni; n = 0; }
  else if (mode == VGG_INTR_SHARED) { d = 6; n = ni; }
  else return VGG_EINVAL;
  if (dc) *dc = d;
  if (ns) *ns = n;
  if (KR) *KR = d + d * (d + 1) / 2 + 6 * n;
  return VGG_OK;
}

struct BlockSet {
  double *cost, *camrec, *g_p, *H_pp, *W, *shared;
};
struct Layout {
  int S, N, dc, ns, KR, D, Dpad, Kpad;
  BlockSet blk[2];
  double *poses[2], *intr[2], *points[2];
  double *sc_c, *sc_p, *M, *q, *dpp, *wacc, *d_c, *bvec, *Zt;
  double *AR;
  double *small;
  double *scal;
  double *packed;
  double *chol_diag;
  int *dev_info;
  size_t bytes;
};

static int make_layout(int S, int N, int model, int mode, void* base, size_t cap, Layout* L) {
  int dc, ns, KR;
  if (dims_of(model, mode, &dc, &ns, &KR) != VGG_OK) {
    set_error("bad camera_model/intr_mode");
    return VGG_EINVAL;
  }
  L->S = S; L->N = N; L->dc = dc; L->ns = ns; L->KR = KR;
  L->D = S * dc + ns;
  L->Dpad = (int)align_up((size_t)L->D + 2, 128);
  L->Kpad = (int)align_up((size_t)3 * N, 16);
  Carver c(base, cap);
  for (int b = 0; b < 2; ++b) {
    L->blk[b].cost = c.take<double>(8);
    L->blk[b].shared = c.take<double>(8);
    L->blk[b].camrec = c.take<double>((size_t)S * KR);
    L->blk[b].g_p = c.take<double>((size_t)N * 3);
    L->blk[b].H_pp = c.take<double>((size_t)N * 6);
    L->blk[b].W = c.take<double>((size_t)(L->D + (L->D & 1)) * N * 3);
    L->poses[b] = c.take<double>((size_t)S * 12);
    L->intr[b] = c.take<double>((size_t)S * 4);
    L->points[b] = c.take<double>((size_t)N * 3);
  }
  L->sc_c = c.take<double>(L->Dpad);
  L->sc_p = c.take<double>((size_t)N * 3);
  L->M = c.take<double>((size_t)N * 9);
  L->q = c.take<double>((size_t)N * 3);
  L->dpp = c.take<double>((size_t)N * 3);
  L->wacc = c.take<double>((size_t)N * 3);
  L->d_c = c.take<double>(L->Dpad);
  L->bvec = c.take<double>(L->Dpad);
  L->Zt = c.take<double>((size_t)L->Kpad * L->Dpad);
  L->AR = c.take<double>((size_t)L->D * L->Dpad + 3 * (size_t)L->Dpad);
  L->small = c.take<double>(8 + (size_t)L->Dpad);
  L->scal = c.take<double>(16);
  L->packed = c.take<double>(32);
  L->chol_diag = c.take<double>(chol_workspace_doubles(L->D + 1));
  L->dev_info = c.take<int>(4);
  L->bytes = align_up(c.off, 256);
  if (base && c.off > cap) {
    set_error("workspace too small: need %zu bytes, have %zu", c.off, cap);
    return VGG_EWORKSPACE;
  }
  return VGG_OK;
}

static cublasHandle_t get_cublas() {
  static thread_local cublasHandle_t h = nullptr;
  if (!h) {
    if (cublasCreate(&h) != CUBLAS_STATUS_SUCCESS) h = nullptr;
  }
  return h;
}

struct FabricLayout {
  size_t arc, mail_off, flags_off, total;
  int mail_len;
};
static FabricLayout fabric_layout(int D, int Dpad) {
  FabricLayout f;
  f.arc = align_up((size_t)D * Dpad + 3 * (size_t)Dpad, 256);
  f.mail_len = Dpad + 64;
  f.mail_off = 2 * f.arc;
  f.flags_off = align_up(f.mail_off + (size_t)2 * 8 * f.mail_len, 32);
  f.total = f.flags_off + 64;
  return f;
}

struct Fabric {
  bool on = false;
  FabricDev base{};
  FabricLayout lay{};
  unsigned long long* epoch = nullptr;
  int small_parity = 0;
  int* err = nullptr;
  FabricDev at(size_t off) const {
    FabricDev f = base;
    for (int r = 0; r < f.world; ++r) f.peer[r] += off;
    return f;
  }
  int barrier(cudaStream_t st) { return launch_fabric_barrier(base, lay.flags_off, ++*epoch, err, st); }
  int allreduce(double* vec, int count, int max_slot, cudaStream_t st) {
    small_parity ^= 1;
    return launch_fabric_allreduce(base, lay.flags_off, lay.mail_off, lay.mail_len, small_parity, ++*epoch, vec, count,
                                   max_slot, err, st);
  }
};

struct BandPlan {
  int nb = 0, KB = 0, ngroups = 0, arrow_blk = 0;
  std::vector<int> kb_ranges, end_blk, kb_rows, fg_tracks;
  BandDev dev{nullptr, nullptr, nullptr, 0};
};
static thread_local BandPlan g_band_last;

__global__ void __launch_bounds__(256) frame_point_range_kernel(int S, int N, const uint8_t* __restrict__ mask,
                                                                int* __restrict__ out) {
  __shared__ int s_lo[256], s_hi[256];
  const int s = blockIdx.x;
  int lo = N, hi = -1;
  for (int n = threadIdx.x; n < N; n += 256)
    if (mask[(size_t)s * N + n]) {
      lo = min(lo, n);
      hi = max(hi, n);
    }
  s_lo[threadIdx.x] = lo;
  s_hi[threadIdx.x] = hi;
  __syncthreads();
  for (int w = 128; w > 0; w >>= 1) {
    if ((int)threadIdx.x < w) {
      s_lo[threadIdx.x] = min(s_lo[threadIdx.x], s_lo[threadIdx.x + w]);
      s_hi[threadIdx.x] = max(s_hi[threadIdx.x], s_hi[threadIdx.x + w]);
    }
    __syncthreads();
  }
  if (threadIdx.x == 0) {
    out[2 * s] = s_lo[0];
    out[2 * s + 1] = s_hi[0];
  }
}

static int compute_band_hint(const vgg_ba_problem* prob, int dc, int D, int Dpad, int Kpad, bool multi_rank, cudaStream_t st,
                             BandPlan* plan) {
  const char* env = getenv("VGG_BAND");
  const bool off = env && env[0] == '0';
  const int S = prob->S, N = prob->N, nb = Dpad / 128, KB = (Kpad + 63) / 64;
  plan->nb = nb;
  plan->KB = KB;
  plan->ngroups = (S + 31) / 32;
  if (off || nb < 6 || N < 1024) return VGG_OK;
  static thread_local int* dev = nullptr;
  static thread_local int cap = 0;
  if (cap < 2 * S) {
    if (dev) cudaFree(dev);
    VGG_CUDA_CHECK(cudaMalloc(reinterpret_cast<void**>(&dev), sizeof(int) * 2 * (size_t)S));
    cap = 2 * S;
  }
  frame_point_range_kernel<<<S, 256, 0, st>>>(S, N, prob->mask, dev);
  VGG_LAUNCH_CHECK();
  std::vector<int> fr(2 * (size_t)S);
  VGG_CUDA_CHECK(cudaMemcpyAsync(fr.data(), dev, sizeof(int) * fr.size(), cudaMemcpyDeviceToHost, st));
  VGG_CUDA_CHECK(cudaStreamSynchronize(st));
  std::vector<int> rg(2 * (size_t)nb);
  for (int rb = 0; rb < nb; ++rb) {
    const int d0 = rb * 128, d1 = std::min(D, d0 + 128) - 1;
    int lo = KB, hi = 0;
    if (d1 >= d0) {
      if (d1 >= S * dc) {
        lo = 0;
        hi = KB;
      } else {
        for (int f = d0 / dc; f <= d1 / dc; ++f) {
          if (fr[2 * f + 1] < 0) continue;
          lo = std::min(lo, 3 * fr[2 * f] / 64);
          hi = std::max(hi, (3 * fr[2 * f + 1] + 2) / 64 + 1);
        }
      }
    }
    if (hi <= lo) lo = hi = 0;
    rg[2 * rb] = lo;
    rg[2 * rb + 1] = std::min(hi, KB);
  }
  double kept = 0.0, all = 0.0;
  for (int bi = 0; bi < nb; ++bi)
    for (int bj = 0; bj <= bi; ++bj) {
      all += KB;
      kept += std::max(0, std::min(rg[2 * bi + 1], rg[2 * bj + 1]) - std::max(rg[2 * bi], rg[2 * bj]));
    }
  if (kept < 0.7 * all) {
    plan->kb_ranges = rg;
    const int arrow = (S * dc) / 128;
    if (arrow >= 4 && !multi_rank) {
      std::vector<int> end(nb);
      int prev = 0;
      for (int b = 0; b < nb; ++b) {
        int e = b;
        if (b < arrow) {
          for (int i = b + 1; i < arrow; ++i)
            if (std::min(rg[2 * i + 1], rg[2 * b + 1]) > std::max(rg[2 * i], rg[2 * b])) e = i;
          e = std::max(e + 1, std::min(b + 2, arrow));
          e = std::max(e, prev);
          e = std::min(e, arrow);
        } else {
          e = nb;
        }
        end[b] = e;
        prev = e;
      }
      plan->end_blk = end;
      plan->arrow_blk = arrow;
      const int ngroups = (S + 31) / 32;
      std::vector<int> tab(2 * (size_t)(nb + KB + ngroups), 0);
      int* t_rb = tab.data();
      int* t_kb = t_rb + 2 * nb;
      int* t_fg = t_kb + 2 * KB;
      for (int i = 0; i < 2 * nb; ++i) t_rb[i] = rg[i];
      for (int kb = 0; kb < KB; ++kb) {
        int first = -1, last = -1;
        for (int rb = 0; rb < arrow; ++rb)
          if (rg[2 * rb] <= kb && kb < rg[2 * rb + 1]) {
            if (first < 0) first = rb;
            last = rb;
          }
        t_kb[2 * kb] = first < 0 ? 0 : first * 128;
        t_kb[2 * kb + 1] = first < 0 ? 0 : (last + 1) * 128;
      }
      for (int g = 0; g < ngroups; ++g) {
        int lo = N, hi = 0;
        for (int f = 32 * g; f < std::min(S, 32 * g + 32); ++f) {
          if (fr[2 * f + 1] < 0) continue;
          lo = std::min(lo, fr[2 * f]);
          hi = std::max(hi, fr[2 * f + 1] + 1);
        }
        t_fg[2 * g] = hi > lo ? lo : 0;
        t_fg[2 * g + 1] = hi > lo ? hi : 0;
      }
      static thread_local int* tdev = nullptr;
      static thread_local size_t tcap = 0;
      if (tcap < tab.size()) {
        if (tdev) cudaFree(tdev);
        VGG_CUDA_CHECK(cudaMalloc(reinterpret_cast<void**>(&tdev), sizeof(int) * tab.size()));
        tcap = tab.size();
      }
      VGG_CUDA_CHECK(cudaMemcpyAsync(tdev, tab.data(), sizeof(int) * tab.size(), cudaMemcpyHostToDevice, st));
      VGG_CUDA_CHECK(cudaStreamSynchronize(st));
      plan->dev = BandDev{tdev, tdev + 2 * nb, tdev + 2 * (nb + KB), arrow * 128};
      plan->kb_rows.assign(t_kb, t_kb + 2 * KB);
      plan->fg_tracks.assign(t_fg, t_fg + 2 * ngroups);
    }
  }
  return VGG_OK;
}

static int schur_build(const Layout& L, const BlockSet& b, const BandPlan& band, const FabricDev& fd,
                       const uint8_t* point_const, double radius, double min_diag, double max_diag, cudaStream_t st,
                       ptrdiff_t mc_off = 0, Fabric* fab = nullptr) {
  int rc;
  double* Sraw = L.AR;
  double* rhs = L.AR + (size_t)L.D * L.Dpad;
  double* hdiag = rhs + L.Dpad;
  double* gvec = hdiag + L.Dpad;
  if ((rc = launch_point_prep(L.N, b.H_pp, b.g_p, L.sc_p, point_const, radius, min_diag, max_diag, L.M, L.q, L.dpp,
                              L.scal, st)))
    return rc;
  VGG_CUDA_CHECK(cudaMemsetAsync(L.AR, 0, sizeof(double) * ((size_t)L.D * L.Dpad + 3 * (size_t)L.Dpad), st));
  if (fab && (rc = fab->barrier(st))) return rc;
  if ((rc = launch_assemble_hc(L.S, L.dc, L.ns, L.KR, L.Dpad, b.camrec, b.shared, Sraw, rhs, hdiag, gvec, mc_off, st))) return rc;
  if ((rc = launch_z_transpose(L.D, L.N, L.Dpad, b.W, L.M, L.q, L.Zt, rhs, mc_off, band.dev.rb_range, st))) return rc;
  if ((rc = launch_syrk(L.Kpad, L.Dpad, L.Zt, Sraw, mc_off, band.kb_ranges, fd, st))) return rc;
  if (fab && (rc = fab->barrier(st))) return rc;
  return VGG_OK;
}

}

using namespace vgg;

extern "C" {

const char* vgg_last_error(void) { return g_err; }
int vgg_version(void) { return 100; }

void vgg_ba_default_options(vgg_ba_options* o) {
  memset(o, 0, sizeof(*o));
  o->max_num_iterations = 100;
  o->max_num_consecutive_invalid_steps = 10;
  o->jacobi_scaling = 1;
  o->function_tolerance = 0.0;
  o->gradient_tolerance = 1e-4;
  o->parameter_tolerance = 0.0;
  o->initial_trust_region_radius = 1e4;
  o->max_trust_region_radius = 1e16;
  o->min_trust_region_radius = 1e-32;
  o->min_relative_decrease = 1e-3;
  o->min_lm_diagonal = 1e-6;
  o->max_lm_diagonal = 1e32;
}

int vgg_ba_dims(int camera_model, int intr_mode, int* dc, int* ns) {
  return dims_of(camera_model, intr_mode, dc, ns, nullptr);
}

int vgg_ba_camrec_len(int camera_model, int intr_mode) {
  int KR = 0;
  if (dims_of(camera_model, intr_mode, nullptr, nullptr, &KR) != VGG_OK) return VGG_EINVAL;
  return KR;
}

int vgg_ba_workspace_bytes(int S, int N, int camera_model, int intr_mode, size_t* bytes) {
  VGG_REQUIRE(S > 0 && N > 0 && bytes, "S, N must be positive");
  Layout L;
  const int rc = make_layout(S, N, camera_model, intr_mode, nullptr, 0, &L);
  if (rc) return rc;
  *bytes = L.bytes;
  return VGG_OK;
}

int vgg_ba_build_blocks(const vgg_ba_problem* prob, double* cost, double* camrec, double* g_p, double* H_pp, double* W,
                        double* shared_out, int tracks_per_warp, void* stream) {
  VGG_REQUIRE(prob && cost && camrec && g_p && H_pp && W && shared_out, "null pointer");
  VGG_REQUIRE(tracks_per_warp >= 0 && tracks_per_warp % 4 == 0, "tracks_per_warp must be 0 (choose) or a multiple of 4");
  g_launch_count = 0;
  return ba_build_blocks(prob, cost, camrec, g_p, H_pp, W, shared_out, tracks_per_warp, nullptr, (cudaStream_t)stream);
}

int vgg_ba_schur(const vgg_ba_problem* prob, const double* camrec, const double* g_p, const double* H_pp,
                 const double* W, const double* shared_in, const double* scale_p, double radius, double min_diag,
                 double max_diag, void* workspace, size_t ws_bytes, double* Sraw, double* rhs, int* Dpad_out,
                 void* stream) {
  VGG_REQUIRE(prob && workspace && Sraw && rhs, "null pointer");
  cudaStream_t st = (cudaStream_t)stream;
  g_launch_count = 0;
  Layout L;
  int rc = make_layout(prob->S, prob->N, prob->camera_model, prob->intr_mode, workspace, ws_bytes, &L);
  if (rc) return rc;
  BlockSet b;
  b.cost = nullptr;
  b.camrec = const_cast<double*>(camrec);
  b.g_p = const_cast<double*>(g_p);
  b.H_pp = const_cast<double*>(H_pp);
  b.W = const_cast<double*>(W);
  b.shared = const_cast<double*>(shared_in);
  VGG_CUDA_CHECK(cudaMemcpyAsync(L.sc_p, scale_p, sizeof(double) * (size_t)L.N * 3, cudaMemcpyDeviceToDevice, st));
  VGG_CUDA_CHECK(cudaMemsetAsync(L.Zt, 0, sizeof(double) * (size_t)L.Kpad * L.Dpad, st));
  VGG_CUDA_CHECK(cudaMemsetAsync(L.scal, 0, sizeof(double) * 16, st));
  rc = schur_build(L, b, BandPlan{}, FabricDev{}, prob->point_const, radius, min_diag, max_diag, st);
  if (rc) return rc;
  VGG_CUDA_CHECK(cudaMemcpyAsync(Sraw, L.AR, sizeof(double) * (size_t)L.D * L.Dpad, cudaMemcpyDeviceToDevice, st));
  VGG_CUDA_CHECK(cudaMemcpyAsync(rhs, L.AR + (size_t)L.D * L.Dpad, sizeof(double) * L.Dpad, cudaMemcpyDeviceToDevice, st));
  if (Dpad_out) *Dpad_out = L.Dpad;
  return VGG_OK;
}

int vgg_cholesky_lower(int n, int lda, double* A, void* workspace, size_t ws_bytes, int* info_host, void* stream) {
  return vgg_dev_cholesky_band(n, lda, A, workspace, ws_bytes, info_host, stream, nullptr, 0, 0);
}

int vgg_dev_cholesky_band(int n, int lda, double* A, void* workspace, size_t ws_bytes, int* info_host, void* stream,
                          const int* end_blk, int count, int arrow_blk) {
  VGG_REQUIRE(A && workspace && n > 0 && lda >= n && (end_blk || count <= 0), "bad arguments");
  cudaStream_t st = (cudaStream_t)stream;
  g_launch_count = 0;
  const size_t need = sizeof(double) * chol_workspace_doubles(n) + 256;
  if (ws_bytes < need) {
    set_error("cholesky workspace too small: need %zu bytes", need);
    return VGG_EWORKSPACE;
  }
  int* info = reinterpret_cast<int*>(workspace);
  double* diag = reinterpret_cast<double*>(reinterpret_cast<char*>(workspace) + 256);
  int rc = chol_lower_inplace(n, lda, A, diag, info, std::vector<int>(end_blk, end_blk + std::max(count, 0)),
                              count > 0 ? arrow_blk : 0, st);
  if (rc) return rc;
  if (info_host) {
    VGG_CUDA_CHECK(cudaMemcpyAsync(info_host, info, sizeof(int), cudaMemcpyDeviceToHost, st));
    VGG_CUDA_CHECK(cudaStreamSynchronize(st));
  }
  return VGG_OK;
}

int vgg_ba_reduced_system_doubles(int S, int camera_model, int intr_mode, size_t* doubles) {
  int dc, ns;
  if (!doubles || dims_of(camera_model, intr_mode, &dc, &ns, nullptr) != VGG_OK) {
    set_error("bad camera_model/intr_mode");
    return VGG_EINVAL;
  }
  const size_t D = (size_t)S * dc + ns, Dpad = align_up(D + 2, 128);
  *doubles = D * Dpad + 3 * Dpad;
  return VGG_OK;
}

int vgg_ba_fabric_doubles(int S, int camera_model, int intr_mode, size_t* doubles) {
  int dc, ns;
  if (!doubles || dims_of(camera_model, intr_mode, &dc, &ns, nullptr) != VGG_OK) {
    set_error("bad camera_model/intr_mode");
    return VGG_EINVAL;
  }
  const int D = S * dc + ns;
  *doubles = fabric_layout(D, (int)align_up((size_t)D + 2, 128)).total;
  return VGG_OK;
}

int vgg_ba_solve(const vgg_ba_problem* prob, const vgg_ba_options* opt_in, void* workspace, size_t ws_bytes,
                 vgg_allreduce_fn allreduce, void* ar_user, vgg_ba_summary* summary, double* trace, void* stream) {
  return vgg_ba_solve_fabric(prob, opt_in, workspace, ws_bytes, allreduce, ar_user, nullptr, summary, trace, stream);
}

int vgg_ba_solve_fabric(const vgg_ba_problem* prob, const vgg_ba_options* opt_in, void* workspace, size_t ws_bytes,
                        vgg_allreduce_fn allreduce, void* ar_user, const vgg_ba_fabric* fabric, vgg_ba_summary* summary,
                        double* trace, void* stream) {
  VGG_REQUIRE(prob && workspace && summary, "null pointer");
  VGG_REQUIRE(prob->uv && prob->mask && prob->param_const && prob->poses && prob->intr && prob->points, "null problem array");
  cudaStream_t st = (cudaStream_t)stream;
  g_launch_count = 0;
  vgg_ba_options opt;
  if (opt_in) opt = *opt_in;
  else vgg_ba_default_options(&opt);
  const int S = prob->S, N = prob->N;
  int dc, ns;
  if (dims_of(prob->camera_model, prob->intr_mode, &dc, &ns, nullptr) != VGG_OK) {
    set_error("bad camera_model/intr_mode");
    return VGG_EINVAL;
  }
  const int D = S * dc + ns;
  Layout L;
  int rc = make_layout(S, N, prob->camera_model, prob->intr_mode, workspace, ws_bytes, &L);
  if (rc) return rc;
  const size_t ar_count = (size_t)D * L.Dpad + 3 * (size_t)L.Dpad;
  ptrdiff_t mc_off = 0;
  Fabric fab;
  static thread_local std::map<const double*, unsigned long long> fabric_epochs;
  if (fabric && fabric->ar_local && fabric->ar_multicast) {
    VGG_REQUIRE(fabric->ar_doubles >= ar_count, "fabric buffer too small (vgg_ba_reduced_system_doubles)");
    const FabricLayout lay = fabric_layout(D, L.Dpad);
    VGG_REQUIRE(fabric->world > 1 && fabric->world <= 8 && fabric->peer_base[0] && fabric->total_doubles >= lay.total,
                "fabric needs its peer table: world in 2..8, peer_base set, total_doubles >= vgg_ba_fabric_doubles");
    L.AR = fabric->ar_local;
    mc_off = fabric->ar_multicast - fabric->ar_local;
    fab.on = true;
    fab.lay = lay;
    fab.base.world = fabric->world;
    fab.base.rank = fabric->rank;
    for (int r = 0; r < fabric->world; ++r) fab.base.peer[r] = fabric->peer_base[r];
    fab.epoch = &fabric_epochs[fabric->peer_base[fabric->rank]];
    fab.err = L.dev_info + 2;
  }
  BandPlan band;
  if ((rc = compute_band_hint(prob, dc, D, L.Dpad, L.Kpad, allreduce != nullptr || fabric != nullptr, st, &band))) return rc;
  g_band_last = band;
  if (band.dev.fg_tracks) {
    const size_t w_doubles = (size_t)N * (size_t)(D + (D & 1)) * 3;
    VGG_CUDA_CHECK(cudaMemsetAsync(L.blk[0].W, 0, sizeof(double) * w_doubles, st));
    VGG_CUDA_CHECK(cudaMemsetAsync(L.blk[1].W, 0, sizeof(double) * w_doubles, st));
  }
  double* Sraw = L.AR;
  double* rhs = L.AR + (size_t)D * L.Dpad;
  double* hdiag = rhs + L.Dpad;
  double* gvec = hdiag + L.Dpad;
  auto reduce_small = [&](double* vec, size_t count, int op) -> int {
    if (fab.on) return fab.allreduce(vec, (int)count, op == 1 ? 0 : -1, st);
    if (allreduce) return allreduce(ar_user, vec, count, op, st);
    return VGG_OK;
  };

  EventPair evs;
  VGG_CUDA_CHECK(cudaEventCreate(&evs.a));
  VGG_CUDA_CHECK(cudaEventCreate(&evs.b));
  const cudaEvent_t ev0 = evs.a, ev1 = evs.b;
  VGG_CUDA_CHECK(cudaEventRecord(ev0, st));

  int cur = 0;
  VGG_CUDA_CHECK(cudaMemcpyAsync(L.poses[0], prob->poses, sizeof(double) * (size_t)S * 12, cudaMemcpyDeviceToDevice, st));
  VGG_CUDA_CHECK(cudaMemcpyAsync(L.intr[0], prob->intr, sizeof(double) * (size_t)S * 4, cudaMemcpyDeviceToDevice, st));
  VGG_CUDA_CHECK(cudaMemcpyAsync(L.points[0], prob->points, sizeof(double) * (size_t)N * 3, cudaMemcpyDeviceToDevice, st));
  VGG_CUDA_CHECK(cudaMemsetAsync(L.Zt, 0, sizeof(double) * (size_t)L.Kpad * L.Dpad, st));
  VGG_CUDA_CHECK(cudaMemsetAsync(L.d_c, 0, sizeof(double) * L.Dpad, st));

  auto eval = [&](int which) -> int {
    vgg_ba_problem p = *prob;
    p.poses = L.poses[which];
    p.intr = L.intr[which];
    p.points = L.points[which];
    const BlockSet& b = L.blk[which];
    const size_t acc_bytes = reinterpret_cast<char*>(b.H_pp + (size_t)N * 6) - reinterpret_cast<char*>(b.cost);
    VGG_CUDA_CHECK(cudaMemsetAsync(b.cost, 0, acc_bytes, st));
    return ba_build_blocks(&p, b.cost, b.camrec, b.g_p, b.H_pp, b.W, b.shared, 0, band.dev.fg_tracks, st, true);
  };
  double* h_scal = pinned_scalars();
  if (!h_scal) {
    set_error("cudaHostAlloc for the scalar read-back failed");
    return VGG_ECUDA;
  }
  VGG_CUDA_CHECK(cudaMemsetAsync(L.dev_info, 0, sizeof(int) * 4, st));
  auto read_scalars = [&]() -> int {
    pack_scalars_kernel<<<1, 32, 0, st>>>(L.scal, L.small, L.dev_info, L.packed);
    VGG_LAUNCH_CHECK();
    VGG_CUDA_CHECK(cudaMemcpyAsync(h_scal, L.packed, sizeof(double) * 24, cudaMemcpyDeviceToHost, st));
    VGG_CUDA_CHECK(cudaStreamSynchronize(st));
    return VGG_OK;
  };
  auto cost_and_gradient = [&](int which, double* cost_out, double* gmax_out) -> int {
    const BlockSet& b = L.blk[which];
    int r;
    VGG_CUDA_CHECK(cudaMemsetAsync(L.small, 0, sizeof(double) * (8 + (size_t)L.Dpad), st));
    VGG_CUDA_CHECK(cudaMemcpyAsync(L.small, b.cost, sizeof(double), cudaMemcpyDeviceToDevice, st));
    if ((r = launch_extract_gvec(S, dc, ns, L.KR, b.camrec, b.shared, L.small + 8, st))) return r;
    if ((r = reduce_small(L.small, 8 + (size_t)L.Dpad, 0))) return r;
    VGG_CUDA_CHECK(cudaMemsetAsync(L.scal + 4, 0, sizeof(double) * 2, st));
    if ((r = launch_gradmax(D, N, L.small + 8, prob->param_const, b.g_p, prob->point_const, L.scal, st))) return r;
    if ((r = reduce_small(L.scal + 5, 1, 1))) return r;
    if ((r = read_scalars())) return r;
    if (h_scal[19] != 0.0) {
      set_error("fabric barrier timed out: a peer rank did not arrive");
      return VGG_ECUDA;
    }
    *cost_out = h_scal[8];
    *gmax_out = grad_max_norm(h_scal[4], h_scal[5]);
    return VGG_OK;
  };

  if ((rc = eval(cur))) return rc;
  if ((rc = launch_jacobi_scale_points(N, L.blk[cur].H_pp, L.sc_p, opt.jacobi_scaling, st))) return rc;
  double cost = 0, gmax = 0;
  if ((rc = cost_and_gradient(cur, &cost, &gmax))) return rc;

  memset(summary, 0, sizeof(*summary));
  summary->initial_cost = cost;
  summary->termination = VGG_BA_NO_CONVERGENCE;
  double radius = opt.initial_trust_region_radius;
  double decrease_factor = 2.0;
  int it = 0, invalid_steps = 0;
  bool have_scale_c = false;
  bool done = gmax <= opt.gradient_tolerance;
  if (done) summary->termination = VGG_BA_CONVERGENCE_GRADIENT;

  while (!done) {
    if (it >= opt.max_num_iterations) break;
    if (radius < opt.min_trust_region_radius) {
      summary->termination = VGG_BA_MIN_TRUST_REGION;
      break;
    }
    ++it;
    const int cand = cur ^ 1;
    VGG_CUDA_CHECK(cudaMemsetAsync(L.scal, 0, sizeof(double) * 16, st));
    FabricDev fd{};
    if (fab.on) {
      const size_t off = (size_t)(it & 1) * fab.lay.arc;
      L.AR = fabric->ar_local + off;
      Sraw = L.AR;
      rhs = L.AR + (size_t)D * L.Dpad;
      hdiag = rhs + L.Dpad;
      gvec = hdiag + L.Dpad;
      fd = fab.at(off);
    }
    if ((rc = schur_build(L, L.blk[cur], band, fd, prob->point_const, radius, opt.min_lm_diagonal, opt.max_lm_diagonal, st,
                          mc_off, fab.on ? &fab : nullptr)))
      return rc;
    if (fab.on && (rc = launch_fabric_gather(fd, D + 3, D + 1, D, L.Dpad, st))) return rc;
    if (allreduce && !mc_off && (rc = allreduce(ar_user, L.AR, ar_count, 0, st))) return rc;
    if (!have_scale_c) {
      if ((rc = launch_jacobi_scale_cams(D, hdiag, L.sc_c, opt.jacobi_scaling, st))) return rc;
      have_scale_c = true;
    }
    if ((rc = launch_scale_damp(D, L.Dpad, Sraw, rhs, hdiag, L.sc_c, prob->param_const, radius, opt.min_lm_diagonal,
                                opt.max_lm_diagonal, L.bvec, st)))
      return rc;
    if ((rc = chol_lower_inplace(D + 1, L.Dpad, Sraw, L.chol_diag, L.dev_info, band.end_blk, band.arrow_blk, st))) return rc;
    const double* dcs = L.bvec;
    size_t dcs_stride = 1;
    {
      VGG_CUDA_CHECK(cudaMemsetAsync(L.dev_info + 1, 0, sizeof(int), st));
      if (D > 7000) {
        cublasHandle_t cb = get_cublas();
        if (!cb || cublasSetStream(cb, st) != CUBLAS_STATUS_SUCCESS) {
          set_error("cublasCreate / cublasSetStream failed");
          return VGG_ESOLVER;
        }
        if (cublasDtrsv(cb, CUBLAS_FILL_MODE_LOWER, CUBLAS_OP_T, CUBLAS_DIAG_NON_UNIT, D, Sraw, L.Dpad, Sraw + D, L.Dpad) !=
            CUBLAS_STATUS_SUCCESS) {
          set_error("cublasDtrsv failed to launch");
          return VGG_ESOLVER;
        }
        g_launch_count += 1;
        dcs = Sraw + D;
        dcs_stride = (size_t)L.Dpad;
      } else {
        if ((rc = launch_trsv_upper(D, L.Dpad, Sraw, Sraw + D, (size_t)L.Dpad, L.bvec, nullptr, st))) return rc;
      }
    }
    if ((rc = launch_cam_step(D, dcs, dcs_stride, L.sc_c, hdiag, gvec, prob->param_const, radius, opt.min_lm_diagonal,
                              opt.max_lm_diagonal, L.d_c, L.scal, st)))
      return rc;
    if ((rc = launch_backsub(D, N, L.blk[cur].W, L.d_c, L.wacc, band.dev.kb_rows, band.dev.arrow_row, st))) return rc;
    if ((rc = launch_point_step(N, L.M, L.blk[cur].g_p, L.wacc, L.sc_p, L.dpp, L.points[cur], radius, L.points[cand],
                                L.scal, st)))
      return rc;
    if ((rc = launch_cam_update(S, dc, ns, prob->camera_model, L.d_c, L.poses[cur], L.intr[cur], L.poses[cand],
                                L.intr[cand], st)))
      return rc;
    if ((rc = eval(cand))) return rc;
    VGG_CUDA_CHECK(cudaMemsetAsync(L.small, 0, sizeof(double) * (8 + (size_t)L.Dpad), st));
    VGG_CUDA_CHECK(cudaMemcpyAsync(L.small, L.blk[cand].cost, sizeof(double), cudaMemcpyDeviceToDevice, st));
    VGG_CUDA_CHECK(cudaMemcpyAsync(L.small + 1, L.scal + 2, sizeof(double) * 2, cudaMemcpyDeviceToDevice, st));
    VGG_CUDA_CHECK(cudaMemcpyAsync(L.small + 3, L.scal + 6, sizeof(double), cudaMemcpyDeviceToDevice, st));
    if ((rc = launch_extract_gvec(S, dc, ns, L.KR, L.blk[cand].camrec, L.blk[cand].shared, L.small + 8, st))) return rc;
    if (fab.on) {
      if ((rc = launch_gradmax(D, N, L.small + 8, prob->param_const, L.blk[cand].g_p, prob->point_const, L.scal, st))) return rc;
      VGG_CUDA_CHECK(cudaMemcpyAsync(L.small + 4, L.scal + 5, sizeof(double), cudaMemcpyDeviceToDevice, st));
      if ((rc = fab.allreduce(L.small, 8 + L.Dpad, 4, st))) return rc;
      VGG_CUDA_CHECK(cudaMemsetAsync(L.scal + 4, 0, sizeof(double) * 2, st));
      if ((rc = launch_gradmax(D, N, L.small + 8, prob->param_const, L.blk[cand].g_p, prob->point_const, L.scal, st))) return rc;
      VGG_CUDA_CHECK(cudaMemcpyAsync(L.scal + 5, L.small + 4, sizeof(double), cudaMemcpyDeviceToDevice, st));
    } else {
      if (allreduce && (rc = allreduce(ar_user, L.small, 8 + (size_t)L.Dpad, 0, st))) return rc;
      if ((rc = launch_gradmax(D, N, L.small + 8, prob->param_const, L.blk[cand].g_p, prob->point_const, L.scal, st))) return rc;
      if (allreduce && (rc = allreduce(ar_user, L.scal + 5, 1, 1, st))) return rc;
    }
    if (opt.parameter_tolerance > 0.0) {
      xnorm_kernel<<<1, 1024, 0, st>>>(S, N, dc, ns, prob->camera_model, prob->param_const, prob->point_const,
                                        L.poses[cur], L.intr[cur], L.points[cur], L.scal + 8);
      VGG_LAUNCH_CHECK();
    }
    if ((rc = read_scalars())) return rc;
    const int h_info[2] = {(int)h_scal[16], (int)h_scal[17]};

    const double c_cost = h_scal[8];
    const double quad = h_scal[0] + h_scal[9];
    const double step_norm = sqrt(h_scal[1] + h_scal[10]);
    const double model_change = 0.5 * quad;
    if (h_scal[19] != 0.0) {
      set_error("fabric barrier timed out: a peer rank did not arrive");
      return VGG_ECUDA;
    }
    const bool solver_bad = h_info[0] != 0 || h_info[1] != 0 || h_scal[7] > 0 || h_scal[11] > 0;
    double* tr = trace ? trace + (size_t)(it - 1) * 8 : nullptr;
    if (tr) {
      tr[0] = it; tr[1] = cost; tr[2] = c_cost; tr[3] = model_change; tr[4] = 0; tr[5] = radius; tr[6] = step_norm; tr[7] = 0;
    }
    if (solver_bad || !(model_change > 0.0) || !isfinite(c_cost)) {
      ++invalid_steps;
      if (tr) tr[7] = 2;
      if (invalid_steps >= opt.max_num_consecutive_invalid_steps) {
        summary->termination = VGG_BA_FAILURE;
        break;
      }
      radius *= 0.5;
      continue;
    }
    invalid_steps = 0;
    const double cost_change = cost - c_cost;
    const double rho = cost_change / model_change;
    if (tr) tr[4] = rho;
    const double x_norm = opt.parameter_tolerance > 0.0 ? sqrt(h_scal[18]) : 0.0;
    if (step_norm <= opt.parameter_tolerance * (x_norm + opt.parameter_tolerance)) {
      summary->termination = VGG_BA_CONVERGENCE_PARAMETER;
      break;
    }
    const bool success = rho > opt.min_relative_decrease;
    if (fabs(cost_change) <= opt.function_tolerance * cost) {
      summary->termination = VGG_BA_CONVERGENCE_FUNCTION;
      break;
    }
    if (success) {
      cur = cand;
      cost = c_cost;
      summary->successful++;
      if (tr) tr[7] = 1;
      radius = fmin(opt.max_trust_region_radius, radius / fmax(1.0 / 3.0, 1.0 - pow(2.0 * rho - 1.0, 3.0)));
      decrease_factor = 2.0;
      gmax = grad_max_norm(h_scal[4], h_scal[5]);
      if (gmax <= opt.gradient_tolerance) {
        summary->termination = VGG_BA_CONVERGENCE_GRADIENT;
        break;
      }
    } else {
      radius = radius / decrease_factor;
      decrease_factor *= 2.0;
    }
  }

  VGG_CUDA_CHECK(cudaMemcpyAsync(prob->poses, L.poses[cur], sizeof(double) * (size_t)S * 12, cudaMemcpyDeviceToDevice, st));
  VGG_CUDA_CHECK(cudaMemcpyAsync(prob->intr, L.intr[cur], sizeof(double) * (size_t)S * 4, cudaMemcpyDeviceToDevice, st));
  VGG_CUDA_CHECK(cudaMemcpyAsync(prob->points, L.points[cur], sizeof(double) * (size_t)N * 3, cudaMemcpyDeviceToDevice, st));
  VGG_CUDA_CHECK(cudaEventRecord(ev1, st));
  VGG_CUDA_CHECK(cudaEventSynchronize(ev1));
  float ms = 0;
  VGG_CUDA_CHECK(cudaEventElapsedTime(&ms, ev0, ev1));
  summary->iterations = it;
  summary->final_cost = cost;
  summary->final_radius = radius;
  summary->device_ms = ms;
  summary->kernel_launches = g_launch_count;
  return VGG_OK;
}

int vgg_dev_last_band_hint(int* meta, int* rb_range, int* end_blk, int* kb_rows, int* fg_tracks) {
  VGG_REQUIRE(meta, "null pointer");
  const BandPlan& r = g_band_last;
  const int m[8] = {!r.kb_ranges.empty(), !r.end_blk.empty(), !r.fg_tracks.empty(), r.nb, r.KB, r.ngroups, r.arrow_blk, 0};
  memcpy(meta, m, sizeof(m));
  auto put = [](int* dst, const std::vector<int>& v) {
    if (dst && !v.empty()) memcpy(dst, v.data(), sizeof(int) * v.size());
  };
  put(rb_range, r.kb_ranges);
  put(end_blk, r.end_blk);
  put(kb_rows, r.kb_rows);
  put(fg_tracks, r.fg_tracks);
  return VGG_OK;
}

}
```

vggsfm_b200/csrc/common.cuh:

```cuda
#pragma once
#include <cuda_runtime.h>
#include <stdint.h>
#include <stdio.h>
#include <stdarg.h>
#include "../../include/vggsfm_b200.h"

namespace vgg {

void set_error(const char* fmt, ...);
extern thread_local long long g_launch_count;

#define VGG_CUDA_CHECK(expr)                                                              \
  do {                                                                                    \
    cudaError_t _e = (expr);                                                              \
    if (_e != cudaSuccess) {                                                              \
      vgg::set_error("%s:%d: %s -> %s", __FILE__, __LINE__, #expr, cudaGetErrorString(_e)); \
      return VGG_ECUDA;                                                                   \
    }                                                                                     \
  } while (0)

#define VGG_LAUNCH_CHECK()                 \
  do {                                     \
    vgg::g_launch_count++;                 \
    VGG_CUDA_CHECK(cudaGetLastError());    \
  } while (0)

#define VGG_REQUIRE(cond, msg)                                   \
  do {                                                           \
    if (!(cond)) {                                               \
      vgg::set_error("%s:%d: %s", __FILE__, __LINE__, msg);      \
      return VGG_EINVAL;                                         \
    }                                                            \
  } while (0)

__host__ __device__ constexpr inline size_t align_up(size_t x, size_t a) { return (x + a - 1) / a * a; }

struct Carver {
  char* base;
  size_t off = 0, cap;
  Carver(void* p, size_t c) : base(static_cast<char*>(p)), cap(c) {}
  template <typename T>
  T* take(size_t n) {
    off = align_up(off, 256);
    T* r = reinterpret_cast<T*>(base + off);
    off += n * sizeof(T);
    return r;
  }
  bool ok() const { return base == nullptr || off <= cap; }
};

struct BandDev {
  const int* rb_range;
  const int* kb_rows;
  const int* fg_tracks;
  int arrow_row;
};

struct FabricDev {
  int world, rank;
  double* peer[8];
};

#ifdef __CUDACC__
__device__ __forceinline__ uint32_t smem_u32(const void* p) {
  return static_cast<uint32_t>(__cvta_generic_to_shared(p));
}
__device__ __forceinline__ void mbar_init(uint64_t* bar, uint32_t count) {
  asm volatile("mbarrier.init.shared::cta.b64 [%0], %1;" ::"r"(smem_u32(bar)), "r"(count));
}
__device__ __forceinline__ void mbar_fence_init() {
  asm volatile("fence.mbarrier_init.release.cluster;" ::: "memory");
}
__device__ __forceinline__ void mbar_expect_tx(uint64_t* bar, uint32_t bytes) {
  asm volatile("mbarrier.arrive.expect_tx.shared::cta.b64 _, [%0], %1;" ::"r"(smem_u32(bar)), "r"(bytes)
               : "memory");
}
__device__ __forceinline__ void mbar_arrive(uint64_t* bar) {
  asm volatile("mbarrier.arrive.shared::cta.b64 _, [%0];" ::"r"(smem_u32(bar)) : "memory");
}
__device__ __forceinline__ void mbar_wait(uint64_t* bar, uint32_t parity) {
  asm volatile(
      "{\n"
      ".reg .pred p;\n"
      "WAIT_LOOP:\n"
      "mbarrier.try_wait.parity.shared::cta.b64 p, [%0], %1;\n"
      "@p bra DONE;\n"
      "bra WAIT_LOOP;\n"
      "DONE:\n"
      "}\n" ::"r"(smem_u32(bar)),
      "r"(parity)
      : "memory");
}
__device__ __forceinline__ void tma_load_1d(void* smem_dst, const void* gmem_src, uint32_t bytes, uint64_t* bar) {
  asm volatile(
      "cp.async.bulk.shared::cluster.global.mbarrier::complete_tx::bytes [%0], [%1], %2, [%3];" ::"r"(
          smem_u32(smem_dst)),
      "l"(gmem_src), "r"(bytes), "r"(smem_u32(bar))
      : "memory");
}
__device__ __forceinline__ void tma_store_1d(void* gmem_dst, const void* smem_src, uint32_t bytes) {
  asm volatile("cp.async.bulk.global.shared::cta.bulk_group [%0], [%1], %2;" ::"l"(gmem_dst),
               "r"(smem_u32(smem_src)), "r"(bytes)
               : "memory");
}
__device__ __forceinline__ void tma_store_commit() { asm volatile("cp.async.bulk.commit_group;" ::: "memory"); }
template <int N>
__device__ __forceinline__ void tma_store_wait_read() {
  asm volatile("cp.async.bulk.wait_group.read %0;" ::"n"(N) : "memory");
}
template <int N>
__device__ __forceinline__ void tma_store_wait_all() {
  asm volatile("cp.async.bulk.wait_group %0;" ::"n"(N) : "memory");
}
__device__ __forceinline__ void fence_proxy_async() { asm volatile("fence.proxy.async.shared::cta;" ::: "memory"); }

__device__ __forceinline__ uint64_t wgmma_desc_sw64(uint32_t saddr) {
  return (uint64_t)((saddr >> 4) & 0x3FFF) | (1ull << 16) | ((uint64_t)(512 >> 4) << 32) | (2ull << 62);
}
__device__ __forceinline__ void wgmma_fence() { asm volatile("wgmma.fence.sync.aligned;" ::: "memory"); }
__device__ __forceinline__ void wgmma_commit() { asm volatile("wgmma.commit_group.sync.aligned;" ::: "memory"); }
__device__ __forceinline__ void wgmma_wait_all() { asm volatile("wgmma.wait_group.sync.aligned 0;" ::: "memory"); }

__device__ __forceinline__ void cp_async16(void* smem_dst, const void* gmem_src) {
  asm volatile("cp.async.cg.shared.global [%0], [%1], 16;" ::"r"(smem_u32(smem_dst)), "l"(gmem_src) : "memory");
}
__device__ __forceinline__ void cp_async4(void* smem_dst, const void* gmem_src) {
  asm volatile("cp.async.ca.shared.global [%0], [%1], 4;" ::"r"(smem_u32(smem_dst)), "l"(gmem_src) : "memory");
}
__device__ __forceinline__ void cp_async_commit() { asm volatile("cp.async.commit_group;" ::: "memory"); }
template <int N>
__device__ __forceinline__ void cp_async_wait() {
  asm volatile("cp.async.wait_group %0;" ::"n"(N) : "memory");
}

__device__ __forceinline__ void dmma_m16n8k16(double (&d)[4], const double (&a)[8], const double (&b)[4]) {
  asm volatile(
      "mma.sync.aligned.m16n8k16.row.col.f64.f64.f64.f64 {%0,%1,%2,%3}, {%4,%5,%6,%7,%8,%9,%10,%11}, {%12,%13,%14,%15}, "
      "{%0,%1,%2,%3};"
      : "+d"(d[0]), "+d"(d[1]), "+d"(d[2]), "+d"(d[3])
      : "d"(a[0]), "d"(a[1]), "d"(a[2]), "d"(a[3]), "d"(a[4]), "d"(a[5]), "d"(a[6]), "d"(a[7]), "d"(b[0]), "d"(b[1]),
        "d"(b[2]), "d"(b[3]));
}

template <int KP>
__device__ __forceinline__ double warp_reduce_scatter(double (&v)[KP], int lane) {
#pragma unroll
  for (int off = KP / 2; off >= 1; off >>= 1) {
    const bool up = (lane & off) != 0;
#pragma unroll
    for (int i = 0; i < off; ++i) {
      const double mine = up ? v[i + off] : v[i];
      const double send = up ? v[i] : v[i + off];
      v[i] = mine + __shfl_xor_sync(0xffffffffu, send, off);
    }
  }
  double r = v[0];
#pragma unroll
  for (int off = KP; off < 32; off <<= 1) r += __shfl_xor_sync(0xffffffffu, r, off);
  return r;
}

__device__ __forceinline__ double warp_sum(double r) {
#pragma unroll
  for (int off = 16; off >= 1; off >>= 1) r += __shfl_xor_sync(0xffffffffu, r, off);
  return r;
}
__device__ __forceinline__ double warp_max(double r) {
#pragma unroll
  for (int off = 16; off >= 1; off >>= 1) r = fmax(r, __shfl_xor_sync(0xffffffffu, r, off));
  return r;
}

__device__ __forceinline__ void syrk_red_upper(double* Cmat, int Dpad, int r, int col, int bj, bool diag, double v,
                                               ptrdiff_t mc_off, const FabricDev& fd) {
  if (v == 0.0 || (diag && col < r)) return;
  const size_t off = (size_t)col * Dpad + r;
  if (fd.world > 1) {
    asm volatile("red.relaxed.sys.global.add.f64 [%0], %1;" ::"l"(fd.peer[bj % fd.world] + off), "d"(-v) : "memory");
  } else if (mc_off) {
    asm volatile("multimem.red.relaxed.sys.global.add.f64 [%0], %1;" ::"l"(Cmat + off + mc_off), "d"(-v) : "memory");
  } else {
    atomicAdd(Cmat + off, -v);
  }
}
#endif

}
```

Measured before the change: 341.0.

## Recompute camera-point Jacobian blocks on the fly instead of materializing W

The block builder no longer writes the dense per-point W (camera-by-point cross Jacobian) buffer. The Z-transpose and back-substitution stages now recompute the needed Jacobian entries directly from poses, intrinsics, points and observations through a shared obs_math header. This removes a large global write and read of W each iteration, plus its memsets and workspace. In exchange, the projection and Jacobian math runs again in the Z build and back-substitution kernels.

```diff
diff --git a/include/vggsfm_b200.h b/include/vggsfm_b200.h
--- a/include/vggsfm_b200.h
+++ b/include/vggsfm_b200.h
@@ -82,7 +82,7 @@
                         double* H_pp, double* W, double* shared, int tracks_per_warp, void* stream);
 
 int vgg_ba_schur(const vgg_ba_problem* prob, const double* camrec, const double* g_p,
-                 const double* H_pp, const double* W, const double* shared, const double* scale_p,
+                 const double* H_pp, const double* shared, const double* scale_p,
                  double radius, double min_diag, double max_diag, void* workspace, size_t ws_bytes,
                  double* Sraw, double* rhs, int* Dpad_out, void* stream);
 
diff --git a/vggsfm_b200/_lib.py b/vggsfm_b200/_lib.py
--- a/vggsfm_b200/_lib.py
+++ b/vggsfm_b200/_lib.py
@@ -120,7 +120,7 @@
                                          ctypes.POINTER(ctypes.c_size_t)]
     L.vgg_ba_camrec_len.argtypes = [ctypes.c_int, ctypes.c_int]
     L.vgg_ba_build_blocks.argtypes = [ctypes.POINTER(BAProblem)] + [ctypes.c_void_p] * 6 + [ctypes.c_int, ctypes.c_void_p]
-    L.vgg_ba_schur.argtypes = ([ctypes.POINTER(BAProblem)] + [ctypes.c_void_p] * 6 +
+    L.vgg_ba_schur.argtypes = ([ctypes.POINTER(BAProblem)] + [ctypes.c_void_p] * 5 +
                                [ctypes.c_double] * 3 + [ctypes.c_void_p, ctypes.c_size_t, ctypes.c_void_p,
                                                         ctypes.c_void_p, ctypes.POINTER(ctypes.c_int), ctypes.c_void_p])
     L.vgg_ba_solve.argtypes = [ctypes.POINTER(BAProblem), ctypes.POINTER(BAOptions), ctypes.c_void_p, ctypes.c_size_t,
diff --git a/vggsfm_b200/bundle_adjustment.py b/vggsfm_b200/bundle_adjustment.py
--- a/vggsfm_b200/bundle_adjustment.py
+++ b/vggsfm_b200/bundle_adjustment.py
@@ -149,7 +149,7 @@
     with torch.cuda.device(dev):
         st = torch.cuda.current_stream().cuda_stream
         _lib.check(L.vgg_ba_schur(ctypes.byref(p), blocks["camrec"].data_ptr(), blocks["g_p"].data_ptr(),
-                                  blocks["H_pp"].data_ptr(), blocks["W"].data_ptr(), blocks["shared"].data_ptr(),
+                                  blocks["H_pp"].data_ptr(), blocks["shared"].data_ptr(),
                                   scale_p.data_ptr(), radius, min_diag, max_diag, ws.data_ptr(), ws.numel(),
                                   Sraw.data_ptr(), rhs.data_ptr(), ctypes.byref(dpad), st), "vgg_ba_schur")
     assert dpad.value == Dpad
diff --git a/vggsfm_b200/csrc/ba_blocks.cu b/vggsfm_b200/csrc/ba_blocks.cu
--- a/vggsfm_b200/csrc/ba_blocks.cu
+++ b/vggsfm_b200/csrc/ba_blocks.cu
@@ -1,5 +1,6 @@
 #include <stdlib.h>
 #include <utility>
+#include "ba_obs.h"
 #include "common.cuh"
 #include "dev_probes.h"
 
@@ -13,16 +14,6 @@
 constexpr int TB = 4;
 constexpr int XT = 32;
 constexpr int PVS = 33;
-
-template <int MODEL, int MODE>
-struct BlkCfg {
-  static constexpr int NI = (MODEL == VGG_SIMPLE_PINHOLE) ? 1 : 2;
-  static constexpr int DC = (MODE == VGG_INTR_PER_FRAME) ? 6 + NI : 6;
-  static constexpr int NS = (MODE == VGG_INTR_SHARED) ? NI : 0;
-  static constexpr int NPACK = DC * (DC + 1) / 2;
-  static constexpr int KR = DC + NPACK + 6 * NS;
-  static constexpr int NP = 9 + 3 * NS;
-};
 
 __host__ __device__ constexpr int pack_row(int dc, int p) {
   int i = 0;
@@ -56,73 +47,22 @@
   (cam_accumulate_one<DC, NS, K, KR>(acc, jc0, jc1, rx, ry), ...);
 }
 
-template <int MODEL>
-__device__ __forceinline__ void obs_math(const double* pw, int lane, const double* xt, float ox, float oy, bool valid,
-                                         double* jc0, double* jc1, double* jx0, double* jx1, double& rx, double& ry) {
-  const double2 xa = *reinterpret_cast<const double2*>(xt);
-  const double2 xb = *reinterpret_cast<const double2*>(xt + 2);
-  const double X0 = xa.x, X1 = xa.y, X2 = xb.x;
-  const double m = valid ? 1.0 : 0.0;
-  const double mp = (xb.y != 0.0) ? 0.0 : m;
-  const double R00 = pw[0 * 32 + lane], R01 = pw[1 * 32 + lane], R02 = pw[2 * 32 + lane], t0_ = pw[3 * 32 + lane];
-  const double R10 = pw[4 * 32 + lane], R11 = pw[5 * 32 + lane], R12 = pw[6 * 32 + lane], t1_ = pw[7 * 32 + lane];
-  const double R20 = pw[8 * 32 + lane], R21 = pw[9 * 32 + lane], R22 = pw[10 * 32 + lane], t2_ = pw[11 * 32 + lane];
-  const double fo = pw[12 * 32 + lane], cx = pw[13 * 32 + lane], cy = pw[14 * 32 + lane];
-  const double kk = (MODEL == VGG_SIMPLE_RADIAL) ? pw[15 * 32 + lane] : 0.0;
-  const double a1 = R00 * X0 + R01 * X1 + R02 * X2;
-  const double a2 = R10 * X0 + R11 * X1 + R12 * X2;
-  const double a3 = R20 * X0 + R21 * X1 + R22 * X2;
-  const double px = a1 + t0_, py = a2 + t1_;
-  const double pz = valid ? (a3 + t2_) : 1.0;
-  const double iz = 1.0 / pz;
-  const double u = px * iz, w_ = py * iz;
-  const double r2 = u * u + w_ * w_;
-  const double d = 1.0 + kk * r2;
-  rx = valid ? (fo * d * u + cx - (double)ox) : 0.0;
-  ry = valid ? (fo * d * w_ + cy - (double)oy) : 0.0;
-  double a00, a01, a11;
-  if (MODEL == VGG_SIMPLE_RADIAL) {
-    a00 = fo * (d + 2.0 * kk * u * u);
-    a01 = fo * (2.0 * kk * u * w_);
-    a11 = fo * (d + 2.0 * kk * w_ * w_);
-  } else {
-    a00 = fo; a01 = 0.0; a11 = fo;
-  }
-  const double izm = iz * m;
-  const double j00 = a00 * izm, j01 = a01 * izm, j02 = -(a00 * u + a01 * w_) * izm;
-  const double j10 = a01 * izm, j11 = a11 * izm, j12 = -(a01 * u + a11 * w_) * izm;
-  const double b1 = 2.0 * a1, b2 = 2.0 * a2, b3 = 2.0 * a3;
-  jc0[0] = b2 * j02 - b3 * j01;  jc1[0] = b2 * j12 - b3 * j11;
-  jc0[1] = b3 * j00 - b1 * j02;  jc1[1] = b3 * j10 - b1 * j12;
-  jc0[2] = b1 * j01 - b2 * j00;  jc1[2] = b1 * j11 - b2 * j10;
-  jc0[3] = j00; jc0[4] = j01; jc0[5] = j02;
-  jc1[3] = j10; jc1[4] = j11; jc1[5] = j12;
-  jc0[6] = m * d * u;            jc1[6] = m * d * w_;
-  jc0[7] = m * fo * u * r2;      jc1[7] = m * fo * w_ * r2;
-  const double mq = (xb.y != 0.0) ? 0.0 : 1.0;
-  jx0[0] = mq * (j00 * R00 + j01 * R10 + j02 * R20);
-  jx0[1] = mq * (j00 * R01 + j01 * R11 + j02 * R21);
-  jx0[2] = mq * (j00 * R02 + j01 * R12 + j02 * R22);
-  jx1[0] = mq * (j10 * R00 + j11 * R10 + j12 * R20);
-  jx1[1] = mq * (j10 * R01 + j11 * R11 + j12 * R21);
-  jx1[2] = mq * (j10 * R02 + j11 * R12 + j12 * R22);
-  (void)mp;
-}
-
-template <int DC, int NS, int WB>
+template <int DC, int NS, int WB, bool WRITE_W>
 __device__ __forceinline__ void emit_blocks(double* wt, double* pvw, int lane, const double* jc0, const double* jc1,
                                             const double* jx0, const double* jx1, double rx, double ry) {
-  double wb[WB];
-#pragma unroll
-  for (int i = 0; i < DC; ++i)
-#pragma unroll
-    for (int c = 0; c < 3; ++c) wb[i * 3 + c] = jc0[i] * jx0[c] + jc1[i] * jx1[c];
-  if ((WB & 1) == 0) {
-#pragma unroll
-    for (int e = 0; e < WB; e += 2) *reinterpret_cast<double2*>(wt + e) = make_double2(wb[e], wb[e + 1]);
-  } else {
-#pragma unroll
-    for (int e = 0; e < WB; ++e) wt[e] = wb[e];
+  if (WRITE_W) {
+    double wb[WB];
+#pragma unroll
+    for (int i = 0; i < DC; ++i)
+#pragma unroll
+      for (int c = 0; c < 3; ++c) wb[i * 3 + c] = w_entry(jc0, jc1, jx0, jx1, i, c);
+    if ((WB & 1) == 0) {
+#pragma unroll
+      for (int e = 0; e < WB; e += 2) *reinterpret_cast<double2*>(wt + e) = make_double2(wb[e], wb[e + 1]);
+    } else {
+#pragma unroll
+      for (int e = 0; e < WB; ++e) wt[e] = wb[e];
+    }
   }
   pvw[0 * PVS + lane] = jx0[0] * rx + jx1[0] * ry;
   pvw[1 * PVS + lane] = jx0[1] * rx + jx1[1] * ry;
@@ -133,30 +73,34 @@
   pvw[6 * PVS + lane] = jx0[1] * jx0[1] + jx1[1] * jx1[1];
   pvw[7 * PVS + lane] = jx0[1] * jx0[2] + jx1[1] * jx1[2];
   pvw[8 * PVS + lane] = jx0[2] * jx0[2] + jx1[2] * jx1[2];
-#pragma unroll
-  for (int j = 0; j < NS; ++j)
-#pragma unroll
-    for (int c = 0; c < 3; ++c) pvw[(9 + j * 3 + c) * PVS + lane] = jc0[6 + j] * jx0[c] + jc1[6 + j] * jx1[c];
+  if (WRITE_W) {
+#pragma unroll
+    for (int j = 0; j < NS; ++j)
+#pragma unroll
+      for (int c = 0; c < 3; ++c) pvw[(9 + j * 3 + c) * PVS + lane] = w_entry(jc0, jc1, jx0, jx1, 6 + j, c);
+  }
 }
 
 __host__ __device__ inline size_t w_pitch(int D) { return (size_t)(D + (D & 1)); }
 
-template <int MODEL, int MODE, bool USE_TMA>
-__global__ void __launch_bounds__(BT, USE_TMA ? 2 : 3) ba_blocks_kernel(
+constexpr int BLK_NOW_CTAS = 2;
+template <int MODEL, int MODE, bool WRITE_W, bool USE_TMA>
+__global__ void __launch_bounds__(BT, WRITE_W ? (USE_TMA ? 2 : 3) : BLK_NOW_CTAS) ba_blocks_kernel(
     int S, int N, int tracks_per_warp, const float* __restrict__ uv, const uint8_t* __restrict__ mask,
     const double* __restrict__ poses, const double* __restrict__ intr, const double* __restrict__ points,
     const uint8_t* __restrict__ point_const, double* __restrict__ cost, double* __restrict__ camrec,
     double* __restrict__ g_p, double* __restrict__ H_pp, double* __restrict__ W, double* __restrict__ shared_out,
     const int* __restrict__ fg_tracks) {
   using C = BlkCfg<MODEL, MODE>;
-  constexpr int DC = C::DC, NS = C::NS, KR = C::KR, NP = C::NP;
+  constexpr int DC = C::DC, NS = C::NS, KR = C::KR;
+  constexpr int NP = WRITE_W ? 9 + 3 * NS : 9;
   constexpr int WB = DC * 3;
   extern __shared__ __align__(128) unsigned char smem_raw[];
   double* sm_pose = reinterpret_cast<double*>(smem_raw);
   double* sm_x = sm_pose + BW * 16 * 32;
   double* sm_pv = sm_x + BW * XT * 4;
   double* sm_w = sm_pv + BW * 32 * PVS;
-  float* sm_obs = reinterpret_cast<float*>(sm_w + (size_t)BW * 2 * 32 * WB);
+  float* sm_obs = reinterpret_cast<float*>(sm_w + (WRITE_W ? (size_t)BW * 2 * 32 * WB : 0));
   const int tid = threadIdx.x, lane = tid & 31, warp = tid >> 5;
   const int D = S * DC + NS;
   const size_t pitch = w_pitch(D);
@@ -245,26 +189,32 @@
       {
         const float ox = k == 0 ? ca.x : cb.x, oy = k == 0 ? ca.y : cb.y;
         const bool valid = frame_ok && ((cm >> (8 * k)) & 0xffu) != 0;
-        obs_math<MODEL>(pw, lane, xw + ((nA - t_begin) & (XT - 1)) * 4, ox, oy, valid, jcA0, jcA1, jxA0, jxA1, rxA, ryA);
+        const double* xt = xw + ((nA - t_begin) & (XT - 1)) * 4;
+        const double2 xa = *reinterpret_cast<const double2*>(xt), xb = *reinterpret_cast<const double2*>(xt + 2);
+        obs_math<MODEL>(pw + lane, 32, xa.x, xa.y, xb.x, xb.y != 0.0, ox, oy, valid, jcA0, jcA1, jxA0, jxA1, rxA, ryA);
       }
       {
         const float ox = k == 0 ? ca.z : cb.z, oy = k == 0 ? ca.w : cb.w;
         const bool valid = hasB && frame_ok && ((cm >> (8 * (k + 1))) & 0xffu) != 0;
-        obs_math<MODEL>(pw, lane, xw + ((nA + 1 - t_begin) & (XT - 1)) * 4, ox, oy, valid, jcB0, jcB1, jxB0, jxB1, rxB, ryB);
+        const double* xt = xw + ((nA + 1 - t_begin) & (XT - 1)) * 4;
+        const double2 xa = *reinterpret_cast<const double2*>(xt), xb = *reinterpret_cast<const double2*>(xt + 2);
+        obs_math<MODEL>(pw + lane, 32, xa.x, xa.y, xb.x, xb.y != 0.0, ox, oy, valid, jcB0, jcB1, jxB0, jxB1, rxB, ryB);
       }
       cost_acc += 0.5 * (rxA * rxA + ryA * ryA) + 0.5 * (rxB * rxB + ryB * ryB);
-      if (USE_TMA) {
+      if (WRITE_W && USE_TMA) {
         if (lane == 0) tma_store_wait_read<0>();
         __syncwarp();
       }
       double* wA = wbuf + lane * WB;
       double* wB = wbuf + 32 * WB + lane * WB;
-      emit_blocks<DC, NS, WB>(wA, pvw, lane, jcA0, jcA1, jxA0, jxA1, rxA, ryA);
-      emit_blocks<DC, NS, WB>(wB, pvw + 16 * PVS, lane, jcB0, jcB1, jxB0, jxB1, rxB, ryB);
+      emit_blocks<DC, NS, WB, WRITE_W>(wA, pvw, lane, jcA0, jcA1, jxA0, jxA1, rxA, ryA);
+      emit_blocks<DC, NS, WB, WRITE_W>(wB, pvw + 16 * PVS, lane, jcB0, jcB1, jxB0, jxB1, rxB, ryB);
       double* dstA = W + ((size_t)nA * pitch + (size_t)g * 32 * DC) * 3;
       double* dstB = dstA + pitch * 3;
       const uint32_t bytes = (uint32_t)nf * WB * 8u;
-      if (USE_TMA && (bytes & 15u) == 0) {
+      if (!WRITE_W) {
+        __syncwarp();
+      } else if (USE_TMA && (bytes & 15u) == 0) {
         fence_proxy_async();
         __syncwarp();
         if (lane == 0) {
@@ -310,7 +260,7 @@
       __syncwarp();
     }
   }
-  if (USE_TMA && lane == 0) tma_store_wait_all<0>();
+  if (WRITE_W && USE_TMA && lane == 0) tma_store_wait_all<0>();
 
   if (frame_ok && t_begin < t_end) {
 #pragma unroll
@@ -333,22 +283,28 @@
   const int S = p->S, N = p->N;
   const int D = S * C::DC + C::NS;
   const size_t pitch = w_pitch(D);
-  const size_t smem = sizeof(double) * (BW * 16 * 32 + BW * XT * 4 + BW * 32 * PVS + (size_t)BW * 2 * 32 * C::DC * 3) +
+  const bool write_w = W != nullptr;
+  const size_t smem = sizeof(double) * (BW * 16 * 32 + BW * XT * 4 + BW * 32 * PVS +
+                                        (write_w ? (size_t)BW * 2 * 32 * C::DC * 3 : 0)) +
                       sizeof(float) * BW * 2 * 32 * 12;
   const bool tma_ok = ((reinterpret_cast<uintptr_t>(W) & 15) == 0);
   const int ngroups = (S + 31) / 32;
-  const auto kern = tma_ok ? ba_blocks_kernel<MODEL, MODE, true> : ba_blocks_kernel<MODEL, MODE, false>;
+  const auto kern = !write_w ? ba_blocks_kernel<MODEL, MODE, false, false>
+                    : tma_ok ? ba_blocks_kernel<MODEL, MODE, true, true>
+                             : ba_blocks_kernel<MODEL, MODE, true, false>;
   if (tracks_per_warp <= 0 && fg_tracks) {
     tracks_per_warp = 64;
   }
   if (tracks_per_warp <= 0) {
-    static int slots = 0;
+    static int slots_of[2] = {0, 0};
+    int& slots = slots_of[write_w];
     if (slots == 0) {
       int dev = 0, sms = 132, per_sm = 2;
       cudaGetDevice(&dev);
       cudaDeviceGetAttribute(&sms, cudaDevAttrMultiProcessorCount, dev);
-      cudaFuncSetAttribute(ba_blocks_kernel<MODEL, MODE, true>, cudaFuncAttributeMaxDynamicSharedMemorySize, (int)smem);
-      cudaOccupancyMaxActiveBlocksPerMultiprocessor(&per_sm, ba_blocks_kernel<MODEL, MODE, true>, BT, smem);
+      const auto qk = write_w ? ba_blocks_kernel<MODEL, MODE, true, true> : kern;
+      cudaFuncSetAttribute(qk, cudaFuncAttributeMaxDynamicSharedMemorySize, (int)smem);
+      cudaOccupancyMaxActiveBlocksPerMultiprocessor(&per_sm, qk, BT, smem);
       if (per_sm < 1) per_sm = 1;
       slots = sms * per_sm;
     }
@@ -384,7 +340,7 @@
       VGG_CUDA_CHECK(cudaMemsetAsync(shared_out, 0, sizeof(double) * 8, stream));
     }
   }
-  if (pitch > (size_t)S * C::DC) {
+  if (write_w && pitch > (size_t)S * C::DC) {
     const size_t tail = pitch - (size_t)S * C::DC;
     VGG_CUDA_CHECK(cudaMemset2DAsync(W + (size_t)S * C::DC * 3, pitch * 24, 0, tail * 24, (size_t)N, stream));
   }
diff --git a/vggsfm_b200/csrc/ba_obs.h b/vggsfm_b200/csrc/ba_obs.h
--- /dev/null
+++ b/vggsfm_b200/csrc/ba_obs.h
@@ -0,0 +1,69 @@
+#pragma once
+#include "common.cuh"
+
+namespace vgg {
+
+template <int MODEL, int MODE>
+struct BlkCfg {
+  static constexpr int NI = (MODEL == VGG_SIMPLE_PINHOLE) ? 1 : 2;
+  static constexpr int DC = (MODE == VGG_INTR_PER_FRAME) ? 6 + NI : 6;
+  static constexpr int NS = (MODE == VGG_INTR_SHARED) ? NI : 0;
+  static constexpr int NPACK = DC * (DC + 1) / 2;
+  static constexpr int KR = DC + NPACK + 6 * NS;
+};
+
+template <int MODEL>
+__device__ __forceinline__ void obs_math(const double* cam, int cs, double X0, double X1, double X2, bool pc, float ox,
+                                         float oy, bool valid, double* jc0, double* jc1, double* jx0, double* jx1,
+                                         double& rx, double& ry) {
+  const double m = valid ? 1.0 : 0.0;
+  const double R00 = cam[0 * cs], R01 = cam[1 * cs], R02 = cam[2 * cs], t0_ = cam[3 * cs];
+  const double R10 = cam[4 * cs], R11 = cam[5 * cs], R12 = cam[6 * cs], t1_ = cam[7 * cs];
+  const double R20 = cam[8 * cs], R21 = cam[9 * cs], R22 = cam[10 * cs], t2_ = cam[11 * cs];
+  const double fo = cam[12 * cs], cx = cam[13 * cs], cy = cam[14 * cs];
+  const double kk = (MODEL == VGG_SIMPLE_RADIAL) ? cam[15 * cs] : 0.0;
+  const double a1 = R00 * X0 + R01 * X1 + R02 * X2;
+  const double a2 = R10 * X0 + R11 * X1 + R12 * X2;
+  const double a3 = R20 * X0 + R21 * X1 + R22 * X2;
+  const double px = a1 + t0_, py = a2 + t1_;
+  const double pz = valid ? (a3 + t2_) : 1.0;
+  const double iz = 1.0 / pz;
+  const double u = px * iz, w_ = py * iz;
+  const double r2 = u * u + w_ * w_;
+  const double d = 1.0 + kk * r2;
+  rx = valid ? (fo * d * u + cx - (double)ox) : 0.0;
+  ry = valid ? (fo * d * w_ + cy - (double)oy) : 0.0;
+  double a00, a01, a11;
+  if (MODEL == VGG_SIMPLE_RADIAL) {
+    a00 = fo * (d + 2.0 * kk * u * u);
+    a01 = fo * (2.0 * kk * u * w_);
+    a11 = fo * (d + 2.0 * kk * w_ * w_);
+  } else {
+    a00 = fo; a01 = 0.0; a11 = fo;
+  }
+  const double izm = iz * m;
+  const double j00 = a00 * izm, j01 = a01 * izm, j02 = -(a00 * u + a01 * w_) * izm;
+  const double j10 = a01 * izm, j11 = a11 * izm, j12 = -(a01 * u + a11 * w_) * izm;
+  const double b1 = 2.0 * a1, b2 = 2.0 * a2, b3 = 2.0 * a3;
+  jc0[0] = b2 * j02 - b3 * j01;  jc1[0] = b2 * j12 - b3 * j11;
+  jc0[1] = b3 * j00 - b1 * j02;  jc1[1] = b3 * j10 - b1 * j12;
+  jc0[2] = b1 * j01 - b2 * j00;  jc1[2] = b1 * j11 - b2 * j10;
+  jc0[3] = j00; jc0[4] = j01; jc0[5] = j02;
+  jc1[3] = j10; jc1[4] = j11; jc1[5] = j12;
+  jc0[6] = m * d * u;            jc1[6] = m * d * w_;
+  jc0[7] = m * fo * u * r2;      jc1[7] = m * fo * w_ * r2;
+  const double mq = pc ? 0.0 : 1.0;
+  jx0[0] = mq * (j00 * R00 + j01 * R10 + j02 * R20);
+  jx0[1] = mq * (j00 * R01 + j01 * R11 + j02 * R21);
+  jx0[2] = mq * (j00 * R02 + j01 * R12 + j02 * R22);
+  jx1[0] = mq * (j10 * R00 + j11 * R10 + j12 * R20);
+  jx1[1] = mq * (j10 * R01 + j11 * R11 + j12 * R21);
+  jx1[2] = mq * (j10 * R02 + j11 * R12 + j12 * R22);
+}
+
+__device__ __forceinline__ double w_entry(const double* jc0, const double* jc1, const double* jx0, const double* jx1,
+                                          int i, int c) {
+  return jc0[i] * jx0[c] + jc1[i] * jx1[c];
+}
+
+}
diff --git a/vggsfm_b200/csrc/ba_schur.cu b/vggsfm_b200/csrc/ba_schur.cu
--- a/vggsfm_b200/csrc/ba_schur.cu
+++ b/vggsfm_b200/csrc/ba_schur.cu
@@ -1,6 +1,7 @@
 #include <stddef.h>
 #include <algorithm>
 #include <vector>
+#include "ba_obs.h"
 #include "common.cuh"
 #include "dev_probes.h"
 #include "syrk_work.h"
@@ -132,41 +133,126 @@
 #undef VGG_PUT
 }
 
-constexpr int ZB_NT = 32;
-__global__ void __launch_bounds__(128) z_build_kernel(int D, int N, int Dpad, size_t pitch, const double* __restrict__ W,
-                                                      const double* __restrict__ M, const double* __restrict__ q,
-                                                      double* __restrict__ Zt, double* __restrict__ rhs,
-                                                      ptrdiff_t mc_off, const int* __restrict__ rb_range) {
-  __shared__ double sm[ZB_NT][12];
-  const int row = blockIdx.x * 128 + threadIdx.x;
-  const int n0 = blockIdx.y * ZB_NT;
-  const int nt = min(ZB_NT, N - n0);
-  if (rb_range) {
-    const int kb_first = (3 * n0) >> 6, kb_last = (3 * (n0 + nt - 1) + 2) >> 6;
-    if (kb_last < rb_range[2 * blockIdx.x] || kb_first >= rb_range[2 * blockIdx.x + 1]) return;
-  }
-  for (int e = threadIdx.x; e < nt * 12; e += 128) {
-    const int t = e / 12, k = e % 12;
-    sm[t][k] = k < 9 ? M[(size_t)(n0 + t) * 9 + k] : q[(size_t)(n0 + t) * 3 + (k - 9)];
-  }
+constexpr int ZB_NT = 8;
+constexpr int ZB_W = 4;
+template <int MODEL, int MODE>
+__global__ void __launch_bounds__(ZB_W * 32) z_build_kernel(
+    int S, int N, int Dpad, const float* __restrict__ uv, const uint8_t* __restrict__ mask,
+    const double* __restrict__ poses, const double* __restrict__ intr, const double* __restrict__ points,
+    const uint8_t* __restrict__ point_const, const double* __restrict__ M, const double* __restrict__ q,
+    double* __restrict__ Zt, double* __restrict__ rhs, ptrdiff_t mc_off, const int* __restrict__ fg_tracks) {
+  using C = BlkCfg<MODEL, MODE>;
+  constexpr int DC = C::DC, NS = C::NS;
+  constexpr int ZR = 32 * DC;
+  __shared__ __align__(16) double s_cam[ZB_W][16 * 32];
+  __shared__ __align__(16) double s_z[ZB_W][3 * ZR];
+  __shared__ double s_pt[ZB_NT][16];
+  __shared__ double s_ws[ZB_W][ZB_NT][3 * (NS > 0 ? NS : 1)];
+  const int lane = threadIdx.x & 31, warp = threadIdx.x >> 5;
+  const int n0 = blockIdx.x * ZB_NT, nt = min(ZB_NT, N - n0);
+  const int ngroups = (S + 31) / 32;
+  for (int e = threadIdx.x; e < ZB_NT * 16; e += blockDim.x) {
+    const int t = e >> 4, k = e & 15, n = n0 + t;
+    double v = 0.0;
+    if (t < nt) {
+      if (k < 3) v = points[(size_t)n * 3 + k];
+      else if (k == 3) v = (point_const && point_const[n]) ? 1.0 : 0.0;
+      else if (k < 13) v = M[(size_t)n * 9 + (k - 4)];
+      else v = q[(size_t)n * 3 + (k - 13)];
+    }
+    s_pt[t][k] = v;
+  }
+  if (NS > 0)
+    for (int e = threadIdx.x; e < ZB_W * ZB_NT * 3 * NS; e += blockDim.x) (&s_ws[0][0][0])[e] = 0.0;
   __syncthreads();
-  if (row >= D) return;
-  double zq = 0.0;
-  const double* wp = W + ((size_t)n0 * pitch + row) * 3;
-#pragma unroll 4
-  for (int t = 0; t < nt; ++t, wp += pitch * 3) {
-    const double w0 = wp[0], w1 = wp[1], w2 = wp[2];
-    const double* m = sm[t];
-    const double z0 = w0 * m[0];
-    const double z1 = w0 * m[1] + w1 * m[4];
-    const double z2 = w0 * m[2] + w1 * m[5] + w2 * m[8];
-    double* zo = Zt + (size_t)(3 * (n0 + t)) * Dpad + row;
-    zo[0] = z0;
-    zo[Dpad] = z1;
-    zo[2 * (size_t)Dpad] = z2;
-    zq += z0 * m[9] + z1 * m[10] + z2 * m[11];
-  }
-  if (zq != 0.0) ar_add(&rhs[row], mc_off ? &rhs[row] + mc_off : nullptr, zq);
+  double* pw = s_cam[warp];
+  double* zs = s_z[warp];
+  const float2* uv2 = reinterpret_cast<const float2*>(uv);
+  for (int g = warp; g < ngroups; g += ZB_W) {
+    if (fg_tracks && (n0 + nt <= fg_tracks[2 * g] || n0 >= fg_tracks[2 * g + 1])) continue;
+    const int s = g * 32 + lane;
+    const bool frame_ok = s < S;
+    const int cnt = min(32, S - g * 32) * DC;
+    __syncwarp();
+#pragma unroll
+    for (int i = 0; i < 12; ++i) pw[i * 32 + lane] = frame_ok ? poses[(size_t)s * 12 + i] : 0.0;
+#pragma unroll
+    for (int i = 0; i < 4; ++i) pw[(12 + i) * 32 + lane] = frame_ok ? intr[(size_t)s * 4 + i] : 0.0;
+    __syncwarp();
+    double zq[DC];
+#pragma unroll
+    for (int i = 0; i < DC; ++i) zq[i] = 0.0;
+    for (int t = 0; t < nt; ++t) {
+      const size_t o = (size_t)s * N + n0 + t;
+      const bool valid = frame_ok && mask[o] != 0;
+      if (!__any_sync(0xffffffffu, valid)) continue;
+      const float2 ob = frame_ok ? uv2[o] : make_float2(0.f, 0.f);
+      const double* pt = s_pt[t];
+      const double* m = pt + 4;
+      double jc0[8], jc1[8], jx0[3], jx1[3], rx, ry;
+      obs_math<MODEL>(pw + lane, 32, pt[0], pt[1], pt[2], pt[3] != 0.0, ob.x, ob.y, valid, jc0, jc1, jx0, jx1, rx, ry);
+#pragma unroll
+      for (int i = 0; i < DC; ++i) {
+        const double w0 = w_entry(jc0, jc1, jx0, jx1, i, 0), w1 = w_entry(jc0, jc1, jx0, jx1, i, 1),
+                     w2 = w_entry(jc0, jc1, jx0, jx1, i, 2);
+        const double z0 = w0 * m[0];
+        const double z1 = w0 * m[1] + w1 * m[4];
+        const double z2 = w0 * m[2] + w1 * m[5] + w2 * m[8];
+        zs[lane * DC + i] = z0;
+        zs[ZR + lane * DC + i] = z1;
+        zs[2 * ZR + lane * DC + i] = z2;
+        zq[i] += z0 * m[9] + z1 * m[10] + z2 * m[11];
+      }
+      if (NS > 0) {
+        double a[8];
+#pragma unroll
+        for (int k = 0; k < 8; ++k) a[k] = k < 3 * NS ? w_entry(jc0, jc1, jx0, jx1, 6 + k / 3, k % 3) : 0.0;
+        const double r = warp_reduce_scatter<8>(a, lane);
+        if (lane < 3 * NS) s_ws[warp][t][lane] += r;
+      }
+      __syncwarp();
+      double* dst = Zt + (size_t)(3 * (n0 + t)) * Dpad + (size_t)g * ZR;
+#pragma unroll
+      for (int c = 0; c < 3; ++c, dst += Dpad) {
+        const double* src = zs + c * ZR;
+        for (int e = 2 * lane; e + 1 < cnt; e += 64)
+          *reinterpret_cast<double2*>(dst + e) = *reinterpret_cast<const double2*>(src + e);
+        if ((cnt & 1) && lane == 0) dst[cnt - 1] = src[cnt - 1];
+      }
+      __syncwarp();
+    }
+    if (frame_ok) {
+#pragma unroll
+      for (int i = 0; i < DC; ++i) {
+        double* r = &rhs[(size_t)s * DC + i];
+        if (zq[i] != 0.0) ar_add(r, mc_off ? r + mc_off : nullptr, zq[i]);
+      }
+    }
+  }
+  if (NS > 0) {
+    __syncthreads();
+    if ((int)threadIdx.x < nt * NS) {
+      const int t = threadIdx.x / NS, j = threadIdx.x % NS;
+      double w[3];
+#pragma unroll
+      for (int c = 0; c < 3; ++c) {
+        w[c] = 0.0;
+#pragma unroll
+        for (int v = 0; v < ZB_W; ++v) w[c] += s_ws[v][t][j * 3 + c];
+      }
+      const double* m = s_pt[t] + 4;
+      const double z0 = w[0] * m[0];
+      const double z1 = w[0] * m[1] + w[1] * m[4];
+      const double z2 = w[0] * m[2] + w[1] * m[5] + w[2] * m[8];
+      double* zo = Zt + (size_t)(3 * (n0 + t)) * Dpad + (size_t)S * DC + j;
+      zo[0] = z0;
+      zo[Dpad] = z1;
+      zo[2 * (size_t)Dpad] = z2;
+      const double zq = z0 * m[9] + z1 * m[10] + z2 * m[11];
+      double* r = &rhs[(size_t)S * DC + j];
+      if (zq != 0.0) ar_add(r, mc_off ? r + mc_off : nullptr, zq);
+    }
+  }
 }
 
 constexpr int SF_BM = 128, SF_BK = 16, SF_LDS = 132, SF_STAGES = 4, SF_MMA_WARPS = 8;
@@ -317,36 +403,67 @@
   }
 }
 
-__global__ void __launch_bounds__(256) backsub_kernel(int D, int N, size_t pitch, const double* __restrict__ W,
-                                                      const double* __restrict__ d_c, double* __restrict__ wacc,
-                                                      const int* __restrict__ kb_rows, int arrow_row) {
-  const int lane = threadIdx.x & 31;
-  const int n = blockIdx.x * 8 + (threadIdx.x >> 5);
-  if (n >= N) return;
-  const double* wp = W + (size_t)n * pitch * 3;
-  double w0 = 0, w1 = 0, w2 = 0;
-  auto span = [&](int r0, int r1) {
-#pragma unroll 4
-    for (int r = r0 + lane; r < r1; r += 32) {
-      const double d = __ldg(d_c + r);
-      w0 = fma(wp[(size_t)r * 3], d, w0);
-      w1 = fma(wp[(size_t)r * 3 + 1], d, w1);
-      w2 = fma(wp[(size_t)r * 3 + 2], d, w2);
-    }
-  };
-  if (kb_rows) {
-    const int ka = (3 * n) >> 6, kb = (3 * n + 2) >> 6;
-    const int lo = min(kb_rows[2 * ka], kb_rows[2 * kb]), hi = min(max(kb_rows[2 * ka + 1], kb_rows[2 * kb + 1]), arrow_row);
-    if (lo < hi) span(lo, hi);
-    span(min(arrow_row, D), D);
-  } else {
-    span(0, D);
-  }
-  w0 = warp_sum(w0); w1 = warp_sum(w1); w2 = warp_sum(w2);
-  if (lane == 0) {
-    wacc[(size_t)n * 3] = w0;
-    wacc[(size_t)n * 3 + 1] = w1;
-    wacc[(size_t)n * 3 + 2] = w2;
+constexpr int BS_W = 16;
+template <int MODEL, int MODE>
+__global__ void __launch_bounds__(BS_W * 32) backsub_kernel(
+    int S, int N, const float* __restrict__ uv, const uint8_t* __restrict__ mask, const double* __restrict__ poses,
+    const double* __restrict__ intr, const double* __restrict__ points, const uint8_t* __restrict__ point_const,
+    const double* __restrict__ d_c, double* __restrict__ wacc, const int* __restrict__ fg_tracks) {
+  using C = BlkCfg<MODEL, MODE>;
+  constexpr int DC = C::DC, NS = C::NS;
+  __shared__ double s_cam[BS_W][16];
+  __shared__ double s_acc[3][BS_W][32];
+  const int lane = threadIdx.x & 31, warp = threadIdx.x >> 5, nw = blockDim.x >> 5;
+  const int nlo = blockIdx.x * 32, nhi = min(N, nlo + 32);
+  const int n = nlo + lane;
+  const bool track_ok = n < N;
+  double X0 = 0.0, X1 = 0.0, X2 = 0.0;
+  bool pc = true;
+  if (track_ok) {
+    X0 = points[(size_t)n * 3]; X1 = points[(size_t)n * 3 + 1]; X2 = points[(size_t)n * 3 + 2];
+    pc = point_const && point_const[n] != 0;
+  }
+  double dsh[2] = {0.0, 0.0};
+#pragma unroll
+  for (int j = 0; j < NS; ++j) dsh[j] = d_c[(size_t)S * DC + j];
+  const float2* uv2 = reinterpret_cast<const float2*>(uv);
+  double* cam = s_cam[warp];
+  double w0 = 0.0, w1 = 0.0, w2 = 0.0;
+  for (int s = warp; s < S; s += nw) {
+    if (fg_tracks && (nhi <= fg_tracks[2 * (s >> 5)] || nlo >= fg_tracks[2 * (s >> 5) + 1])) continue;
+    const size_t o = (size_t)s * N + n;
+    const bool valid = track_ok && mask[o] != 0;
+    if (!__any_sync(0xffffffffu, valid)) continue;
+    const float2 ob = valid ? uv2[o] : make_float2(0.f, 0.f);
+    __syncwarp();
+    if (lane < 16) cam[lane] = lane < 12 ? poses[(size_t)s * 12 + lane] : intr[(size_t)s * 4 + (lane - 12)];
+    __syncwarp();
+    double jc0[8], jc1[8], jx0[3], jx1[3], rx, ry;
+    obs_math<MODEL>(cam, 1, X0, X1, X2, pc, ob.x, ob.y, valid, jc0, jc1, jx0, jx1, rx, ry);
+    const double* d = d_c + (size_t)s * DC;
+#pragma unroll
+    for (int i = 0; i < DC; ++i) {
+      const double di = __ldg(d + i);
+      w0 = fma(w_entry(jc0, jc1, jx0, jx1, i, 0), di, w0);
+      w1 = fma(w_entry(jc0, jc1, jx0, jx1, i, 1), di, w1);
+      w2 = fma(w_entry(jc0, jc1, jx0, jx1, i, 2), di, w2);
+    }
+#pragma unroll
+    for (int j = 0; j < NS; ++j) {
+      w0 = fma(w_entry(jc0, jc1, jx0, jx1, 6 + j, 0), dsh[j], w0);
+      w1 = fma(w_entry(jc0, jc1, jx0, jx1, 6 + j, 1), dsh[j], w1);
+      w2 = fma(w_entry(jc0, jc1, jx0, jx1, 6 + j, 2), dsh[j], w2);
+    }
+  }
+  s_acc[0][warp][lane] = w0;
+  s_acc[1][warp][lane] = w1;
+  s_acc[2][warp][lane] = w2;
+  __syncthreads();
+  for (int e = threadIdx.x; e < 96; e += blockDim.x) {
+    const int c = e >> 5, t = e & 31;
+    double r = 0.0;
+    for (int v = 0; v < nw; ++v) r += s_acc[c][v][t];
+    if (nlo + t < N) wacc[(size_t)(nlo + t) * 3 + c] = r;
   }
 }
 
@@ -479,11 +596,24 @@
   VGG_LAUNCH_CHECK();
   return VGG_OK;
 }
-int launch_z_transpose(int D, int N, int Dpad, const double* W, const double* M, const double* q, double* Zt,
-                       double* rhs, ptrdiff_t mc_off, const int* rb_range, cudaStream_t st) {
-  const size_t pitch = (size_t)(D + (D & 1));
-  dim3 grid((D + 127) / 128, (N + ZB_NT - 1) / ZB_NT);
-  z_build_kernel<<<grid, 128, 0, st>>>(D, N, Dpad, pitch, W, M, q, Zt, rhs, mc_off, rb_range);
+#define VGG_PICK_BA_KERNEL(kern, tmpl, p)                 \
+  decltype(&tmpl<0, 0>) kern = nullptr;                   \
+  switch ((p)->camera_model * 3 + (p)->intr_mode) {       \
+    case 0: kern = tmpl<0, 0>; break;                     \
+    case 1: kern = tmpl<0, 1>; break;                     \
+    case 2: kern = tmpl<0, 2>; break;                     \
+    case 3: kern = tmpl<1, 0>; break;                     \
+    case 4: kern = tmpl<1, 1>; break;                     \
+    case 5: kern = tmpl<1, 2>; break;                     \
+  }                                                       \
+  VGG_REQUIRE(kern, "bad camera_model/intr_mode")
+
+int launch_z_build(const vgg_ba_problem* p, int Dpad, const double* M, const double* q, double* Zt, double* rhs,
+                   ptrdiff_t mc_off, const int* fg_tracks, cudaStream_t st) {
+  VGG_PICK_BA_KERNEL(kern, z_build_kernel, p);
+  const int nw = std::min(ZB_W, (p->S + 31) / 32);
+  kern<<<(p->N + ZB_NT - 1) / ZB_NT, nw * 32, 0, st>>>(p->S, p->N, Dpad, p->uv, p->mask, p->poses, p->intr, p->points,
+                                                        p->point_const, M, q, Zt, rhs, mc_off, fg_tracks);
   VGG_LAUNCH_CHECK();
   return VGG_OK;
 }
@@ -546,10 +676,11 @@
   VGG_LAUNCH_CHECK();
   return VGG_OK;
 }
-int launch_backsub(int D, int N, const double* W, const double* d_c, double* wacc, const int* kb_rows, int arrow_row,
-                   cudaStream_t st) {
-  const size_t pitch = (size_t)(D + (D & 1));
-  backsub_kernel<<<(N + 7) / 8, 256, 0, st>>>(D, N, pitch, W, d_c, wacc, kb_rows, arrow_row);
+int launch_backsub(const vgg_ba_problem* p, const double* d_c, double* wacc, const int* fg_tracks, cudaStream_t st) {
+  VGG_PICK_BA_KERNEL(kern, backsub_kernel, p);
+  const int nw = std::min(BS_W, p->S);
+  kern<<<(p->N + 31) / 32, nw * 32, 0, st>>>(p->S, p->N, p->uv, p->mask, p->poses, p->intr, p->points, p->point_const,
+                                             d_c, wacc, fg_tracks);
   VGG_LAUNCH_CHECK();
   return VGG_OK;
 }
diff --git a/vggsfm_b200/csrc/ba_solve.cu b/vggsfm_b200/csrc/ba_solve.cu
--- a/vggsfm_b200/csrc/ba_solve.cu
+++ b/vggsfm_b200/csrc/ba_solve.cu
@@ -28,8 +28,8 @@
                       double* scal, cudaStream_t st);
 int launch_assemble_hc(int S, int dc, int ns, int KR, int Dpad, const double* camrec, const double* shared_in,
                        double* Sraw, double* rhs, double* hdiag, double* gvec, ptrdiff_t mc_off, cudaStream_t st);
-int launch_z_transpose(int D, int N, int Dpad, const double* W, const double* M, const double* q, double* Zt,
-                       double* rhs, ptrdiff_t mc_off, const int* rb_range, cudaStream_t st);
+int launch_z_build(const vgg_ba_problem* p, int Dpad, const double* M, const double* q, double* Zt, double* rhs,
+                   ptrdiff_t mc_off, const int* fg_tracks, cudaStream_t st);
 int launch_syrk(int Kpad, int Dpad, const double* Zt, double* Cmat, ptrdiff_t mc_off, const std::vector<int>& kb_ranges,
                 const FabricDev& fd, cudaStream_t st);
 int launch_scale_damp(int D, int Dpad, double* A, const double* rhs, const double* hdiag, const double* sc,
@@ -38,8 +38,7 @@
 int launch_cam_step(int D, const double* dcs, size_t dcs_stride, const double* sc, const double* hdiag, const double* gvec,
                     const uint8_t* pconst, double radius, double min_diag, double max_diag, double* d_c, double* scal,
                     cudaStream_t st);
-int launch_backsub(int D, int N, const double* W, const double* d_c, double* wacc, const int* kb_rows, int arrow_row,
-                   cudaStream_t st);
+int launch_backsub(const vgg_ba_problem* p, const double* d_c, double* wacc, const int* fg_tracks, cudaStream_t st);
 int launch_point_step(int N, const double* M, const double* g_p, const double* wacc, const double* sc_p,
                       const double* dpp, const double* X, double radius, double* Xc, double* scal, cudaStream_t st);
 int launch_cam_update(int S, int dc, int ns, int model, const double* d_c, const double* poses, const double* intr,
@@ -143,7 +142,7 @@
 }
 
 struct BlockSet {
-  double *cost, *camrec, *g_p, *H_pp, *W, *shared;
+  double *cost, *camrec, *g_p, *H_pp, *shared;
 };
 struct Layout {
   int S, N, dc, ns, KR, D, Dpad, Kpad;
@@ -176,7 +175,6 @@
     L->blk[b].camrec = c.take<double>((size_t)S * KR);
     L->blk[b].g_p = c.take<double>((size_t)N * 3);
     L->blk[b].H_pp = c.take<double>((size_t)N * 6);
-    L->blk[b].W = c.take<double>((size_t)(L->D + (L->D & 1)) * N * 3);
     L->poses[b] = c.take<double>((size_t)S * 12);
     L->intr[b] = c.take<double>((size_t)S * 4);
     L->points[b] = c.take<double>((size_t)N * 3);
@@ -249,7 +247,7 @@
 struct BandPlan {
   int nb = 0, KB = 0, ngroups = 0, arrow_blk = 0;
   std::vector<int> kb_ranges, end_blk, kb_rows, fg_tracks;
-  BandDev dev{nullptr, nullptr, nullptr, 0};
+  BandDev dev{nullptr};
 };
 static thread_local BandPlan g_band_last;
 
@@ -349,11 +347,7 @@
       plan->end_blk = end;
       plan->arrow_blk = arrow;
       const int ngroups = (S + 31) / 32;
-      std::vector<int> tab(2 * (size_t)(nb + KB + ngroups), 0);
-      int* t_rb = tab.data();
-      int* t_kb = t_rb + 2 * nb;
-      int* t_fg = t_kb + 2 * KB;
-      for (int i = 0; i < 2 * nb; ++i) t_rb[i] = rg[i];
+      std::vector<int> t_kb(2 * (size_t)KB, 0), t_fg(2 * (size_t)ngroups, 0);
       for (int kb = 0; kb < KB; ++kb) {
         int first = -1, last = -1;
         for (int rb = 0; rb < arrow; ++rb)
@@ -376,36 +370,36 @@
       }
       static thread_local int* tdev = nullptr;
       static thread_local size_t tcap = 0;
-      if (tcap < tab.size()) {
+      if (tcap < t_fg.size()) {
         if (tdev) cudaFree(tdev);
-        VGG_CUDA_CHECK(cudaMalloc(reinterpret_cast<void**>(&tdev), sizeof(int) * tab.size()));
-        tcap = tab.size();
+        VGG_CUDA_CHECK(cudaMalloc(reinterpret_cast<void**>(&tdev), sizeof(int) * t_fg.size()));
+        tcap = t_fg.size();
       }
-      VGG_CUDA_CHECK(cudaMemcpyAsync(tdev, tab.data(), sizeof(int) * tab.size(), cudaMemcpyHostToDevice, st));
+      VGG_CUDA_CHECK(cudaMemcpyAsync(tdev, t_fg.data(), sizeof(int) * t_fg.size(), cudaMemcpyHostToDevice, st));
       VGG_CUDA_CHECK(cudaStreamSynchronize(st));
-      plan->dev = BandDev{tdev, tdev + 2 * nb, tdev + 2 * (nb + KB), arrow * 128};
-      plan->kb_rows.assign(t_kb, t_kb + 2 * KB);
-      plan->fg_tracks.assign(t_fg, t_fg + 2 * ngroups);
-    }
-  }
-  return VGG_OK;
-}
-
-static int schur_build(const Layout& L, const BlockSet& b, const BandPlan& band, const FabricDev& fd,
-                       const uint8_t* point_const, double radius, double min_diag, double max_diag, cudaStream_t st,
+      plan->dev = BandDev{tdev};
+      plan->kb_rows = t_kb;
+      plan->fg_tracks = t_fg;
+    }
+  }
+  return VGG_OK;
+}
+
+static int schur_build(const Layout& L, const vgg_ba_problem& p, const BlockSet& b, const BandPlan& band,
+                       const FabricDev& fd, double radius, double min_diag, double max_diag, cudaStream_t st,
                        ptrdiff_t mc_off = 0, Fabric* fab = nullptr) {
   int rc;
   double* Sraw = L.AR;
   double* rhs = L.AR + (size_t)L.D * L.Dpad;
   double* hdiag = rhs + L.Dpad;
   double* gvec = hdiag + L.Dpad;
-  if ((rc = launch_point_prep(L.N, b.H_pp, b.g_p, L.sc_p, point_const, radius, min_diag, max_diag, L.M, L.q, L.dpp,
+  if ((rc = launch_point_prep(L.N, b.H_pp, b.g_p, L.sc_p, p.point_const, radius, min_diag, max_diag, L.M, L.q, L.dpp,
                               L.scal, st)))
     return rc;
   VGG_CUDA_CHECK(cudaMemsetAsync(L.AR, 0, sizeof(double) * ((size_t)L.D * L.Dpad + 3 * (size_t)L.Dpad), st));
   if (fab && (rc = fab->barrier(st))) return rc;
   if ((rc = launch_assemble_hc(L.S, L.dc, L.ns, L.KR, L.Dpad, b.camrec, b.shared, Sraw, rhs, hdiag, gvec, mc_off, st))) return rc;
-  if ((rc = launch_z_transpose(L.D, L.N, L.Dpad, b.W, L.M, L.q, L.Zt, rhs, mc_off, band.dev.rb_range, st))) return rc;
+  if ((rc = launch_z_build(&p, L.Dpad, L.M, L.q, L.Zt, rhs, mc_off, band.dev.fg_tracks, st))) return rc;
   if ((rc = launch_syrk(L.Kpad, L.Dpad, L.Zt, Sraw, mc_off, band.kb_ranges, fd, st))) return rc;
   if (fab && (rc = fab->barrier(st))) return rc;
   return VGG_OK;
@@ -464,7 +458,7 @@
 }
 
 int vgg_ba_schur(const vgg_ba_problem* prob, const double* camrec, const double* g_p, const double* H_pp,
-                 const double* W, const double* shared_in, const double* scale_p, double radius, double min_diag,
+                 const double* shared_in, const double* scale_p, double radius, double min_diag,
                  double max_diag, void* workspace, size_t ws_bytes, double* Sraw, double* rhs, int* Dpad_out,
                  void* stream) {
   VGG_REQUIRE(prob && workspace && Sraw && rhs, "null pointer");
@@ -478,12 +472,11 @@
   b.camrec = const_cast<double*>(camrec);
   b.g_p = const_cast<double*>(g_p);
   b.H_pp = const_cast<double*>(H_pp);
-  b.W = const_cast<double*>(W);
   b.shared = const_cast<double*>(shared_in);
   VGG_CUDA_CHECK(cudaMemcpyAsync(L.sc_p, scale_p, sizeof(double) * (size_t)L.N * 3, cudaMemcpyDeviceToDevice, st));
   VGG_CUDA_CHECK(cudaMemsetAsync(L.Zt, 0, sizeof(double) * (size_t)L.Kpad * L.Dpad, st));
   VGG_CUDA_CHECK(cudaMemsetAsync(L.scal, 0, sizeof(double) * 16, st));
-  rc = schur_build(L, b, BandPlan{}, FabricDev{}, prob->point_const, radius, min_diag, max_diag, st);
+  rc = schur_build(L, *prob, b, BandPlan{}, FabricDev{}, radius, min_diag, max_diag, st);
   if (rc) return rc;
   VGG_CUDA_CHECK(cudaMemcpyAsync(Sraw, L.AR, sizeof(double) * (size_t)L.D * L.Dpad, cudaMemcpyDeviceToDevice, st));
   VGG_CUDA_CHECK(cudaMemcpyAsync(rhs, L.AR + (size_t)L.D * L.Dpad, sizeof(double) * L.Dpad, cudaMemcpyDeviceToDevice, st));
@@ -586,11 +579,6 @@
   BandPlan band;
   if ((rc = compute_band_hint(prob, dc, D, L.Dpad, L.Kpad, allreduce != nullptr || fabric != nullptr, st, &band))) return rc;
   g_band_last = band;
-  if (band.dev.fg_tracks) {
-    const size_t w_doubles = (size_t)N * (size_t)(D + (D & 1)) * 3;
-    VGG_CUDA_CHECK(cudaMemsetAsync(L.blk[0].W, 0, sizeof(double) * w_doubles, st));
-    VGG_CUDA_CHECK(cudaMemsetAsync(L.blk[1].W, 0, sizeof(double) * w_doubles, st));
-  }
   double* Sraw = L.AR;
   double* rhs = L.AR + (size_t)D * L.Dpad;
   double* hdiag = rhs + L.Dpad;
@@ -614,15 +602,19 @@
   VGG_CUDA_CHECK(cudaMemsetAsync(L.Zt, 0, sizeof(double) * (size_t)L.Kpad * L.Dpad, st));
   VGG_CUDA_CHECK(cudaMemsetAsync(L.d_c, 0, sizeof(double) * L.Dpad, st));
 
-  auto eval = [&](int which) -> int {
+  auto state = [&](int which) {
     vgg_ba_problem p = *prob;
     p.poses = L.poses[which];
     p.intr = L.intr[which];
     p.points = L.points[which];
+    return p;
+  };
+  auto eval = [&](int which) -> int {
+    const vgg_ba_problem p = state(which);
     const BlockSet& b = L.blk[which];
     const size_t acc_bytes = reinterpret_cast<char*>(b.H_pp + (size_t)N * 6) - reinterpret_cast<char*>(b.cost);
     VGG_CUDA_CHECK(cudaMemsetAsync(b.cost, 0, acc_bytes, st));
-    return ba_build_blocks(&p, b.cost, b.camrec, b.g_p, b.H_pp, b.W, b.shared, 0, band.dev.fg_tracks, st, true);
+    return ba_build_blocks(&p, b.cost, b.camrec, b.g_p, b.H_pp, nullptr, b.shared, 0, band.dev.fg_tracks, st, true);
   };
   double* h_scal = pinned_scalars();
   if (!h_scal) {
@@ -691,8 +683,9 @@
       gvec = hdiag + L.Dpad;
       fd = fab.at(off);
     }
-    if ((rc = schur_build(L, L.blk[cur], band, fd, prob->point_const, radius, opt.min_lm_diagonal, opt.max_lm_diagonal, st,
-                          mc_off, fab.on ? &fab : nullptr)))
+    const vgg_ba_problem pcur = state(cur);
+    if ((rc = schur_build(L, pcur, L.blk[cur], band, fd, radius, opt.min_lm_diagonal, opt.max_lm_diagonal, st, mc_off,
+                          fab.on ? &fab : nullptr)))
       return rc;
     if (fab.on && (rc = launch_fabric_gather(fd, D + 3, D + 1, D, L.Dpad, st))) return rc;
     if (allreduce && !mc_off && (rc = allreduce(ar_user, L.AR, ar_count, 0, st))) return rc;
@@ -729,7 +722,7 @@
     if ((rc = launch_cam_step(D, dcs, dcs_stride, L.sc_c, hdiag, gvec, prob->param_const, radius, opt.min_lm_diagonal,
                               opt.max_lm_diagonal, L.d_c, L.scal, st)))
       return rc;
-    if ((rc = launch_backsub(D, N, L.blk[cur].W, L.d_c, L.wacc, band.dev.kb_rows, band.dev.arrow_row, st))) return rc;
+    if ((rc = launch_backsub(&pcur, L.d_c, L.wacc, band.dev.fg_tracks, st))) return rc;
     if ((rc = launch_point_step(N, L.M, L.blk[cur].g_p, L.wacc, L.sc_p, L.dpp, L.points[cur], radius, L.points[cand],
                                 L.scal, st)))
       return rc;
diff --git a/vggsfm_b200/csrc/common.cuh b/vggsfm_b200/csrc/common.cuh
--- a/vggsfm_b200/csrc/common.cuh
+++ b/vggsfm_b200/csrc/common.cuh
@@ -50,10 +50,7 @@
 };
 
 struct BandDev {
-  const int* rb_range;
-  const int* kb_rows;
   const int* fg_tracks;
-  int arrow_row;
 };
 
 struct FabricDev {
```

After: 361.3, median of 6. +6.0%, better.
